# Kyo-suke-S/Depth_image_captioning_pub

Hardware: AMD Instinct MI355X
Metric: images/sec (train, depth-soft, 224x224, seq-len 20) (higher is better)
Workload: dtype f32; 1 GPU; depth-soft train step, synthetic RGB-D 224x224, batch 64/GPU, seq-len 20, V=10000, ResNet-152 (random init, batch-stat BN) + depth CNN + soft-attention LSTM; global_batch=64, batch_per_gpu=64, seq_len=20, vocab=10000, parallelism=dp1, resnet_conv_mode=f16x2, cross_step_resnet_overlap=True, resnet_forwards_in_flight=3, annotation_cells=49, ranks=1, collective=none (single rank)

## Files before the change

depth_image_captioning_pub_amd/csrc/api.hip:

```cpp
#include "dic.h"
#include "conv.h"
#include "nn_kernels.h"

#include <cstdio>

using namespace dic;

namespace dic { void resnet_fuse_bn_operand(int mask); void resnet_fuse_bn_halo(int on); void resnet_fuse_res_bn(int on); void depth_encoder_l1_sparse(int on); void bn_finalize_two_level_rows(int rows); void resnet_debug_fused_tail_bn(int on); void conv1_depth_debug_blocks(int n);
                void depth_encoder_f16x2(int on); }
#ifdef DIC_EXPERIMENTS
namespace dic { void decoder_debug_persistent(int on); void decoder_persist_debug_buffer(unsigned long long* p); void decoder_persist_debug_placement(int p);
                void resnet_debug_skip_bn_apply(int on); }
#endif

extern "C" {

int dic_version(void) { return DIC_ABI_VERSION; }
size_t dic_struct_bytes(int which) {
  switch (which) {
    case 0: return sizeof(dic_conv_bn_layer);
    case 1: return sizeof(dic_decoder_weights);
    case 2: return sizeof(dic_decoder_grads);
    case 3: return sizeof(dic_depth_encoder_weights);
    case 4: return sizeof(dic_depth_encoder_grads);
    case 5: return sizeof(dic_depth_bn_state);
    case 6: return sizeof(dic_nic_weights);
    case 7: return sizeof(dic_nic_grads);
    default: return 0;
  }
}
const char* dic_last_error(void) { return last_error(); }

int dic_gemm_f32(int M, int N, int K, const float* A, long long lda, int a_colk, const float* B, long long ldb,
                 int b_colk, float* C, long long ldc, const float* bias, int act, int accumulate, int splitk,
                 float* workspace, size_t workspace_bytes, int force_tile, void* stream) {
  GemmParams p{};
  p.M = M; p.N = N; p.K = K;
  p.A = a_colk ? op_colk(A, lda) : op_rowk(A, lda);
  p.B = b_colk ? op_colk(B, ldb) : op_rowk(B, ldb);
  p.ep = ep_store(C, ldc, bias, act);
  p.ep.accumulate = accumulate;
  p.splitk = splitk; p.ws = workspace;
  p.ablate = force_tile / 1000;
  force_tile %= 1000;
  DIC_REQUIRE(force_tile == 0 || force_tile == 64 || force_tile == 128, "force_tile must be 0, 64 or 128");
  if (splitk > 1)
    DIC_REQUIRE(workspace_bytes >= gemm_splitk_ws_bytes(M, N, splitk), "dic_gemm_f32: workspace too small");
  return gemm_launch(p, (hipStream_t)stream, force_tile);
}

int dic_conv2d_fwd(const float* x, int B, int H, int W, int C, int in_nchw, const float* w_ohwi, const float* bias,
                   int CO, int KH, int KW, int stride, int pad, float* y_nhwc, float* bn_partial, int* mtiles_out,
                   int force_tile, float* tail_ws, void* stream) {
  ConvDesc d{B, H, W, C, CO, KH, KW, stride, pad, in_nchw};
  return conv_fwd(x, d, w_ohwi, bias, y_nhwc, bn_partial, mtiles_out, (hipStream_t)stream, force_tile, tail_ws);
}

int dic_debug_force_staged_gemm(int on) {
  if (gemm_bf3_force_tile(on) == 0) return 0;
  if (on >= 100 && on <= 104) { dic::resnet_fuse_bn_operand(on == 104 ? -1 : on - 100); return 0; }
  if (on == 98 || on == 99) { dic::resnet_fuse_res_bn(on - 98); return 0; }
  if (on == 108 || on == 109) { dic::resnet_fuse_bn_halo(on - 108); return 0; }
  if (on == 182 || on == 183) { dic::bn_finalize_two_level_rows(on == 182 ? 512 : 1024); return 0; }
  if (on == 180 || on == 181) { dic::depth_encoder_l1_sparse(on - 180); return 0; }
  if (on == 116 || on == 117) { dic::depth_encoder_f16x2(on - 116); return 0; }
#ifdef DIC_EXPERIMENTS
  if (on == 140 || on == 141) { dic::decoder_debug_persistent(on - 140); return 0; }
  if (on == 142 || on == 143) { dic::decoder_persist_debug_placement(on - 142); return 0; }
  if (on >= 130 && on <= 134) { dic::conv1_depth_debug_blocks(256 * (on - 130)); return 0; }
  if (on >= 150 && on <= 153) { dic::resnet_debug_fused_tail_bn(on - 150); return 0; }
  if (on >= 124 && on <= 127) { dic::resnet_debug_skip_bn_apply(on == 125 ? 3 : on == 126 ? 2 : on == 127 ? 1 : 0); return 0; }
  if (on >= 0 && on <= 13) { gemm_force_v1(on); return 0; }
#endif
  DIC_REQUIRE(false, "debug switch: unknown code %d", on);
  return 0;
}
#ifdef DIC_EXPERIMENTS
int dic_debug_decoder_stamps(unsigned long long* dev_buf) { dic::decoder_persist_debug_buffer(dev_buf); return 0; }
#endif
int dic_debug_conv1_wgrad(const float* x, int B, int H, int W, const float* dy, float* dw, float* dbias, float* ws, float* cs_ws,
                          void* stream) {
  ConvDesc d{B, H, W, 1, 128, 7, 7, 3, 0, 0};
  return conv1_depth_wgrad(x, d, dy, dw, dbias, ws, cs_ws, (hipStream_t)stream);
}
int dic_debug_conv1_fwd(const float* x, int B, int H, int W, const float* w, const float* bias, float* y, float* partial,
                        void* stream) {
  ConvDesc d{B, H, W, 1, 128, 7, 7, 3, 0, 0};
  int rows = 0;
  return conv1_depth_fwd(x, d, w, bias, y, partial, &rows, (hipStream_t)stream);
}
int dic_debug_conv_bf3(const uint16_t* const x_planes[3], int B, int H, int W, int C, const uint16_t* const w_planes[3], int CO,
                       int k, int stride, int pad, float* y, float* bn_partial, int* mtiles_out, float* tail_ws, void* stream) {
  ConvDesc d{B, H, W, C, CO, k, k, stride, pad, 0};
  return conv_fwd_bf3(x_planes, d, w_planes, y, bn_partial, mtiles_out, tail_ws, (hipStream_t)stream, nullptr, nullptr, nullptr);
}
int dic_debug_bf3_plan(int route, int fmt, int B, int H, int W, int C, int CO, int k, int stride, int pad, int flags, int splitk,
                       int tail_ws_slabs, char* name, int name_bytes, int* out) {
  DIC_REQUIRE(name && name_bytes > 0 && out, "debug_bf3_plan: bad arguments");
  const char* kernel = nullptr;
  DIC_TRY(bf3_plan_route(route, fmt, ConvDesc{B, H, W, C, CO, k, k, stride, pad, 0}, flags, splitk, tail_ws_slabs, &kernel, out));
  snprintf(name, name_bytes, "%s", kernel);
  return DIC_OK;
}
int dic_debug_conv_fmt(const uint16_t* const x_planes[3], int B, int H, int W, int C, const uint16_t* const w_planes[3], int CO,
                       int k, int stride, int pad, float* y, float* bn_partial, int* mtiles_out, float* tail_ws, int fmt, float out_scale,
                       void* stream) {
  ConvDesc d{B, H, W, C, CO, k, k, stride, pad, 0};
  return conv_fwd_bf3(x_planes, d, w_planes, y, bn_partial, mtiles_out, tail_ws, (hipStream_t)stream, nullptr, nullptr, nullptr, 0, 1024, fmt,
                      out_scale);
}
int dic_debug_conv1x1_bn_fmt(const float* raw, const float* scale, const float* shift, const float* res, int relu, float* act_out, int M,
                             int C, const uint16_t* const w_planes[3], int CO, float* y, float* bn_partial, int* mtiles_out, float* tail_ws,
                             int tail_ws_slabs, int fmt, float out_scale, void* stream) {
  return conv1x1_fwd_bf3_bn(raw, scale, shift, res, relu, act_out, M, C, w_planes, CO, y, bn_partial, mtiles_out, tail_ws, tail_ws_slabs,
                            (hipStream_t)stream, nullptr, nullptr, fmt, out_scale);
}
int dic_debug_conv3x3_bn(const float* raw, const float* scale, const float* shift, int relu, int B, int H, int W, int C,
                         const uint16_t* const w_planes[3], int CO, float* y, float* bn_partial, int* mtiles_out, float* tail_ws,
                         int tail_ws_slabs, float out_scale, uint32_t* status, void* stream) {
  ConvDesc d{B, H, W, C, CO, 3, 3, 1, 1, 0};
  return conv3x3_fwd_bf3_bn(raw, scale, shift, relu, d, w_planes, y, bn_partial, mtiles_out, tail_ws, tail_ws_slabs, (hipStream_t)stream,
                            nullptr, nullptr, 1, out_scale, status);
}
#ifdef DIC_EXPERIMENTS
int dic_debug_conv1x1_astat(const float* raw, const float* scale, const float* shift, int relu, int M, int C, const uint16_t* const w_planes[3],
                            int CO, float* y, float* bn_partial, int* mtiles_out, float out_scale, uint32_t* status, void* stream) {
  return conv1x1_astat_bn(raw, scale, shift, relu, M, C, w_planes, CO, y, bn_partial, mtiles_out, (hipStream_t)stream, out_scale, status);
}
#endif
int dic_conv_persistent_grid(int max_workgroups) {
  DIC_REQUIRE(gemm_bf3_set_persist_grid(max_workgroups) == 0, "dic_conv_persistent_grid: 1 <= max_workgroups <= 1024");
  return DIC_OK;
}
int dic_debug_conv1x1_bn(const float* raw, const float* scale, const float* shift, const float* res, int relu, float* act_out, int M,
                         int C, const uint16_t* const w_planes[3], int CO, float* y, float* bn_partial, int* mtiles_out, float* tail_ws,
                         int tail_ws_slabs, void* stream) {
  return conv1x1_fwd_bf3_bn(raw, scale, shift, res, relu, act_out, M, C, w_planes, CO, y, bn_partial, mtiles_out, tail_ws, tail_ws_slabs,
                            (hipStream_t)stream, nullptr, nullptr);
}
static int bn_buf(const float* scale, const float* shift, const float* mean, const float* invstd, BnBuf* out, const char* who) {
  DIC_REQUIRE(scale && shift && mean && invstd, "%s: a BatchNorm buffer (scale, shift, mean, invstd) is NULL", who);
  *out = BnBuf{const_cast<float*>(scale), const_cast<float*>(shift), const_cast<float*>(mean), const_cast<float*>(invstd)};
  return DIC_OK;
}
static int bn_buf_opt(const float* scale, const float* shift, const float* mean, const float* invstd, BnBuf* out, bool* have, const char* who) {
  *have = scale || shift || mean || invstd;
  *out = BnBuf{};
  return *have ? bn_buf(scale, shift, mean, invstd, out, who) : DIC_OK;
}
static int plane_list(uint16_t* const planes[3], const char* who) {
  DIC_REQUIRE(!planes || (planes[0] && planes[1]), "%s: planes[0] / planes[1] is NULL", who);
  return DIC_OK;
}
int dic_debug_bn_backward_ws_floats(int C) {
  DIC_REQUIRE(C > 0 && C % 64 == 0, "dic_debug_bn_backward_ws_floats: C=%d must be a positive multiple of 64", C);
  const size_t n = bn_backward_ws_floats(C);
  DIC_REQUIRE(n < ((size_t)1 << 31), "dic_debug_bn_backward_ws_floats: C=%d is out of range", C);
  return (int)n;
}
int dic_debug_bn_finalize(const float* partial, int mtiles, long long count, int C, const float* gamma, const float* beta,
                          float* running_mean, float* running_var, float* scale, float* shift, float* mean, float* invstd, double* red,
                          size_t red_doubles, uint32_t* status, void* stream) {
  BnBuf bn;
  DIC_TRY(bn_buf(scale, shift, mean, invstd, &bn, "dic_debug_bn_finalize"));
  DIC_REQUIRE(partial && gamma && beta, "dic_debug_bn_finalize: partial / gamma / beta is NULL");
  DIC_REQUIRE(mtiles >= 1 && count >= 1 && C >= 1, "dic_debug_bn_finalize: mtiles=%d count=%lld C=%d must be positive", mtiles, count, C);
  DIC_REQUIRE(!running_mean == !running_var, "dic_debug_bn_finalize: running_mean and running_var go together");
  DIC_REQUIRE(!red || red_doubles >= bn_finalize_ws_doubles(mtiles, C), "dic_debug_bn_finalize: red holds %zu doubles, %zu needed", red_doubles,
              bn_finalize_ws_doubles(mtiles, C));
  return bn_finalize_train(partial, mtiles, count, C, gamma, beta, running_mean, running_var, bn, red, (hipStream_t)stream, status);
}
int dic_debug_bn_finalize_eval(int C, const float* gamma, const float* beta, const float* running_mean, const float* running_var,
                               float* scale, float* shift, float* mean, float* invstd, void* stream) {
  BnBuf bn;
  DIC_TRY(bn_buf(scale, shift, mean, invstd, &bn, "dic_debug_bn_finalize_eval"));
  DIC_REQUIRE(gamma && beta && running_mean && running_var, "dic_debug_bn_finalize_eval: gamma / beta / running statistics NULL");
  DIC_REQUIRE(C >= 1, "dic_debug_bn_finalize_eval: C=%d must be positive", C);
  return bn_finalize_eval(C, gamma, beta, running_mean, running_var, bn, (hipStream_t)stream);
}
int dic_debug_bn_apply(const float* x, const float* residual, const uint16_t* const residual_planes[3], float* y, uint16_t* const planes[3],
                       long long rows, int C, const float* scale, const float* shift, const float* mean, const float* invstd, int relu,
                       const float* res_scale, const float* res_shift, const float* res_mean, const float* res_invstd, uint32_t* status,
                       void* stream) {
  BnBuf bn, rbn;
  bool have_rbn;
  DIC_TRY(bn_buf(scale, shift, mean, invstd, &bn, "dic_debug_bn_apply"));
  DIC_TRY(bn_buf_opt(res_scale, res_shift, res_mean, res_invstd, &rbn, &have_rbn, "dic_debug_bn_apply (residual)"));
  DIC_TRY(plane_list(planes, "dic_debug_bn_apply"));
  DIC_REQUIRE(x, "dic_debug_bn_apply: x is NULL");
  DIC_REQUIRE(rows >= 1 && C >= 1, "dic_debug_bn_apply: rows=%lld C=%d must be positive", rows, C);
  DIC_REQUIRE(!residual_planes || (residual_planes[0] && residual_planes[1] && residual_planes[2]), "dic_debug_bn_apply: a residual plane is NULL");
  if (!planes) {
    DIC_REQUIRE(y, "dic_debug_bn_apply: no output (y and planes NULL)");
    DIC_REQUIRE(!residual_planes && !have_rbn, "dic_debug_bn_apply: a plane residual or a residual BatchNorm needs plane output");
    DIC_REQUIRE(C % 4 == 0, "dic_debug_bn_apply: C=%d %% 4", C);
    return bn_apply(x, residual, y, rows, C, bn, relu, (hipStream_t)stream);
  }
  DIC_REQUIRE(C % 32 == 0, "dic_debug_bn_apply: C=%d %% 32 (plane output)", C);
  return bn_apply_planes(x, residual, residual_planes, y, planes, rows, C, bn, relu, (hipStream_t)stream, have_rbn ? &rbn : nullptr, status);
}
static int pool_geometry(const char* who, int B, int H, int W, int C, int k, int s, int p) {
  DIC_REQUIRE(B >= 1 && H >= 1 && W >= 1 && C >= 1, "%s: B=%d H=%d W=%d C=%d must be positive", who, B, H, W, C);
  DIC_REQUIRE(C % 4 == 0, "%s: C=%d %% 4", who, C);
  DIC_REQUIRE(k >= 1 && k <= 15 && s >= 1 && p >= 0 && 2 * p <= k, "%s: k=%d (1..15) s=%d p=%d (at most k / 2)", who, k, s, p);
  DIC_REQUIRE(H + 2 * p >= k && W + 2 * p >= k, "%s: the %dx%d window does not fit the padded %dx%d map", who, k, k, H + 2 * p, W + 2 * p);
  return DIC_OK;
}
int dic_debug_bn_relu_maxpool(const float* x, int B, int H, int W, int C, const float* scale, const float* shift, const float* mean,
                              const float* invstd, int relu, int k, int s, int p, float* y, unsigned char* idx, uint16_t* const planes[3],
                              uint32_t* status, float* xsel, void* stream) {
  BnBuf bn;
  bool have_bn;
  DIC_TRY(bn_buf_opt(scale, shift, mean, invstd, &bn, &have_bn, "dic_debug_bn_relu_maxpool"));
  DIC_TRY(plane_list(planes, "dic_debug_bn_relu_maxpool"));
  DIC_TRY(pool_geometry("dic_debug_bn_relu_maxpool", B, H, W, C, k, s, p));
  DIC_REQUIRE(x && (y || planes), "dic_debug_bn_relu_maxpool: x is NULL or there is no output");
  DIC_REQUIRE(!planes || C % 32 == 0, "dic_debug_bn_relu_maxpool: C=%d %% 32 (plane output)", C);
  return bn_relu_maxpool(x, B, H, W, C, have_bn ? &bn : nullptr, relu, k, s, p, y, idx, (hipStream_t)stream, planes, status, xsel);
}
int dic_debug_adaptive_avgpool(const float* x, int B, int H, int W, int C, const float* scale, const float* shift, const float* mean,
                               const float* invstd, int relu, int out, float* y, void* stream) {
  BnBuf bn;
  bool have_bn;
  DIC_TRY(bn_buf_opt(scale, shift, mean, invstd, &bn, &have_bn, "dic_debug_adaptive_avgpool"));
  DIC_REQUIRE(x && y, "dic_debug_adaptive_avgpool: x / y is NULL");
  DIC_REQUIRE(B >= 1 && H >= 1 && W >= 1 && C >= 1 && out >= 1, "dic_debug_adaptive_avgpool: B=%d H=%d W=%d C=%d out=%d must be positive", B, H, W, C, out);
  DIC_REQUIRE(C % 4 == 0, "dic_debug_adaptive_avgpool: C=%d %% 4", C);
  return adaptive_avgpool(x, B, H, W, C, have_bn ? &bn : nullptr, relu, out, y, (hipStream_t)stream);
}
int dic_debug_adaptive_avgpool_bwd(const float* dy, int B, int H, int W, int C, int out, float* dx, void* stream) {
  DIC_REQUIRE(dy && dx, "dic_debug_adaptive_avgpool_bwd: dy / dx is NULL");
  DIC_REQUIRE(B >= 1 && H >= 1 && W >= 1 && C >= 1 && out >= 1, "dic_debug_adaptive_avgpool_bwd: B=%d H=%d W=%d C=%d out=%d must be positive", B, H, W, C, out);
  DIC_REQUIRE(C % 4 == 0, "dic_debug_adaptive_avgpool_bwd: C=%d %% 4", C);
  return adaptive_avgpool_bwd(dy, B, H, W, C, out, dx, (hipStream_t)stream);
}
int dic_debug_maxpool_relu_bwd(const float* dpool, const unsigned char* idx, const float* x, int B, int H, int W, int C, int k,
                               const float* scale, const float* shift, const float* mean, const float* invstd, float* dy, void* stream) {
  BnBuf bn;
  DIC_TRY(bn_buf(scale, shift, mean, invstd, &bn, "dic_debug_maxpool_relu_bwd"));
  DIC_TRY(pool_geometry("dic_debug_maxpool_relu_bwd", B, H, W, C, k, k, 0));
  DIC_REQUIRE(dpool && idx && x && dy, "dic_debug_maxpool_relu_bwd: dpool / idx / x / dy is NULL");
  return maxpool_relu_bwd(dpool, idx, x, B, H, W, C, k, bn, dy, (hipStream_t)stream);
}
int dic_debug_relu_mask_bwd(float* dy, const float* x, long long rows, int C, const float* scale, const float* shift, const float* mean,
                            const float* invstd, void* stream) {
  BnBuf bn;
  DIC_TRY(bn_buf(scale, shift, mean, invstd, &bn, "dic_debug_relu_mask_bwd"));
  DIC_REQUIRE(dy && x, "dic_debug_relu_mask_bwd: dy / x is NULL");
  DIC_REQUIRE(rows >= 1 && C >= 1 && C % 4 == 0, "dic_debug_relu_mask_bwd: rows=%lld, C=%d %% 4", rows, C);
  return relu_mask_bwd(dy, x, rows, C, bn, (hipStream_t)stream);
}
static int f16_scale(const uint16_t* const planes[3], uint32_t* bound, float* slot, F16Scale* out, const char* who) {
  *out = F16Scale{bound, slot};
  DIC_REQUIRE(!(planes && !planes[2]) || (bound && slot), "%s: f16x2 planes need the scale's bound word and slot", who);
  return DIC_OK;
}
int dic_debug_bn_backward(float* dy_dx, const float* x, long long rows, int C, const float* gamma, const float* scale, const float* shift,
                          const float* mean, const float* invstd, float* dgamma, float* dbeta, float* ws, size_t ws_floats,
                          uint16_t* const dx_planes[3], uint32_t* f16_bound, float* f16_slot, void* stream) {
  BnBuf bn;
  F16Scale fs;
  DIC_TRY(bn_buf(scale, shift, mean, invstd, &bn, "dic_debug_bn_backward"));
  DIC_TRY(plane_list(dx_planes, "dic_debug_bn_backward"));
  DIC_TRY(f16_scale(dx_planes, f16_bound, f16_slot, &fs, "dic_debug_bn_backward"));
  DIC_REQUIRE(dy_dx && x && gamma && dgamma && dbeta && ws, "dic_debug_bn_backward: dy_dx / x / gamma / dgamma / dbeta / ws is NULL");
  DIC_REQUIRE(rows >= 1 && C >= 1 && C % 64 == 0, "dic_debug_bn_backward: rows=%lld, C=%d %% 64", rows, C);
  DIC_REQUIRE(ws_floats >= bn_backward_ws_floats(C), "dic_debug_bn_backward: ws holds %zu floats, %zu needed", ws_floats, bn_backward_ws_floats(C));
  return bn_backward(dy_dx, x, rows, C, gamma, bn, dgamma, dbeta, ws, (hipStream_t)stream, dx_planes, &fs);
}
int dic_debug_bn_pool_backward(const float* dpool, const unsigned char* idx, const float* x, int B, int H, int W, int C, int k,
                               const float* gamma, const float* scale, const float* shift, const float* mean, const float* invstd,
                               float* dgamma, float* dbeta, float* ws, size_t ws_floats, float* dy, uint16_t* const dy_planes[3],
                               uint32_t* f16_bound, float* f16_slot, void* stream) {
  BnBuf bn;
  F16Scale fs;
  DIC_TRY(bn_buf(scale, shift, mean, invstd, &bn, "dic_debug_bn_pool_backward"));
  DIC_TRY(plane_list(dy_planes, "dic_debug_bn_pool_backward"));
  DIC_TRY(f16_scale(dy_planes, f16_bound, f16_slot, &fs, "dic_debug_bn_pool_backward"));
  DIC_TRY(pool_geometry("dic_debug_bn_pool_backward", B, H, W, C, k, k, 0));
  DIC_REQUIRE(dpool && idx && x && gamma && dgamma && dbeta && ws && dy, "dic_debug_bn_pool_backward: dpool / idx / x / gamma / dgamma / dbeta / ws / dy is NULL");
  DIC_REQUIRE(C % 64 == 0 && 256 % (C / 4) == 0, "dic_debug_bn_pool_backward: C=%d %% 64, with C / 4 dividing 256", C);
  DIC_REQUIRE(ws_floats >= bn_backward_ws_floats(C), "dic_debug_bn_pool_backward: ws holds %zu floats, %zu needed", ws_floats, bn_backward_ws_floats(C));
  return bn_pool_backward(dpool, idx, x, B, H, W, C, k, gamma, bn, dgamma, dbeta, ws, dy, (hipStream_t)stream, dy_planes, &fs);
}
int dic_debug_colsum_rows(const float* X, long long ld, long long rows, int C, float* out, float* ws, size_t ws_floats, void* stream) {
  DIC_REQUIRE(X && out && ws, "dic_debug_colsum_rows: X / out / ws is NULL");
  DIC_REQUIRE(rows >= 1 && C >= 1 && ld >= C, "dic_debug_colsum_rows: rows=%lld C=%d ld=%lld (at least C)", rows, C, ld);
  DIC_REQUIRE(ws_floats >= (size_t)256 * C, "dic_debug_colsum_rows: ws holds %zu floats, %zu needed", ws_floats, (size_t)256 * C);
  return colsum_rows(X, ld, rows, C, out, ws, (hipStream_t)stream);
}
int dic_debug_f16_scale_reset(uint32_t* bounds, int n, void* stream) {
  DIC_REQUIRE(bounds && n >= 1 && n <= 64, "dic_debug_f16_scale_reset: bounds is NULL or n=%d is outside 1..64", n);
  return f16_scale_reset(bounds, n, (hipStream_t)stream);
}
int dic_debug_f16_scale_from_absmax(const float* x, long long n, uint32_t* bound, float* slot, void* stream) {
  DIC_REQUIRE(x && bound && slot, "dic_debug_f16_scale_from_absmax: x / bound / slot is NULL");
  DIC_REQUIRE(n >= 4 && n % 4 == 0, "dic_debug_f16_scale_from_absmax: n=%lld %% 4", n);
  return f16_scale_from_absmax(x, n, F16Scale{bound, slot}, (hipStream_t)stream);
}
int dic_debug_f16_scale_finish(uint32_t* bound, float* slot, void* stream) {
  DIC_REQUIRE(bound && slot, "dic_debug_f16_scale_finish: bound / slot is NULL");
  return f16_scale_finish(F16Scale{bound, slot}, (hipStream_t)stream);
}
static int conv_geometry(const char* who, int B, int H, int W, int C, int CO, int k, int stride, int pad) {
  DIC_REQUIRE(B >= 1 && H >= 1 && W >= 1 && C >= 1 && CO >= 1, "%s: B=%d H=%d W=%d C=%d CO=%d must be positive", who, B, H, W, C, CO);
  DIC_REQUIRE(k >= 1 && k <= 7 && stride >= 1 && pad >= 0 && pad < k, "%s: k=%d (1..7) stride=%d pad=%d (below k)", who, k, stride, pad);
  DIC_REQUIRE(H + 2 * pad >= k && W + 2 * pad >= k, "%s: the %dx%d filter does not fit the padded %dx%d map", who, k, k, H + 2 * pad, W + 2 * pad);
  const ConvDesc d{B, H, W, C, CO, k, k, stride, pad, 0};
  DIC_REQUIRE((long long)B * d.OH() * d.OW() <= 0x7fffffffll - 32 && (long long)B * H * W <= 0x7fffffffll, "%s: more than 2^31 pixels", who);
  return DIC_OK;
}
static int plane_triple(const uint16_t* const planes[3], int fmt, const char* who, const char* what) {
  DIC_REQUIRE(planes && planes[0] && planes[1] && (fmt || planes[2]), "%s: %s: a plane pointer is NULL", who, what);
  return DIC_OK;
}
int dic_debug_conv_wgrad_sizes(int B, int H, int W, int C, int CO, int k, int stride, int pad, int splitk, size_t* dyT_elems, size_t* pT_elems,
                               size_t* ws_floats) {
  DIC_TRY(conv_geometry("dic_debug_conv_wgrad_sizes", B, H, W, C, CO, k, stride, pad));
  DIC_REQUIRE(C % 32 == 0 && CO % 32 == 0, "dic_debug_conv_wgrad_sizes: C=%d and CO=%d %% 32", C, CO);
  DIC_REQUIRE(splitk >= 1 && splitk <= 16, "dic_debug_conv_wgrad_sizes: splitk=%d is outside 1..16", splitk);
  DIC_REQUIRE(dyT_elems && pT_elems && ws_floats, "dic_debug_conv_wgrad_sizes: an output pointer is NULL");
  const ConvDesc d{B, H, W, C, CO, k, k, stride, pad, 0};
  *dyT_elems = conv_wgrad_bf3_plane_elems(d, 0); *pT_elems = conv_wgrad_bf3_plane_elems(d, 1); *ws_floats = conv_wgrad_bf3_ws_floats(d, splitk);
  return DIC_OK;
}
int dic_debug_conv_wgrad(const float* x, int B, int H, int W, int C, int CO, int k, int stride, int pad, const float* dy, float* dw_ohwi,
                         int splitk, uint16_t* const dyT[3], size_t dyT_elems, uint16_t* const pT[3], size_t pT_elems, float* ws,
                         size_t ws_floats, int fmt, const float* dy_slot, void* stream) {
  const char* who = "dic_debug_conv_wgrad";
  DIC_TRY(conv_geometry(who, B, H, W, C, CO, k, stride, pad));
  DIC_REQUIRE(x && dy && dw_ohwi && ws, "%s: x / dy / dw_ohwi / ws is NULL", who);
  DIC_REQUIRE(fmt == 0 || fmt == 1, "%s: fmt=%d is neither 0 (bf16x3) nor 1 (f16x2)", who, fmt);
  DIC_REQUIRE(C % 32 == 0 && CO % 32 == 0, "%s: C=%d and CO=%d %% 32", who, C, CO);
  DIC_REQUIRE(splitk >= 1 && splitk <= 16, "%s: splitk=%d is outside 1..16", who, splitk);
  DIC_TRY(plane_triple(dyT, fmt, who, "dyT"));
  DIC_TRY(plane_triple(pT, fmt, who, "pT"));
  DIC_REQUIRE(fmt == 0 || dy_slot, "%s: the f16x2 format needs the gradient's scale slot", who);
  const ConvDesc d{B, H, W, C, CO, k, k, stride, pad, 0};
  DIC_REQUIRE(dyT_elems >= conv_wgrad_bf3_plane_elems(d, 0), "%s: dyT planes hold %zu elements, %zu needed", who, dyT_elems, conv_wgrad_bf3_plane_elems(d, 0));
  DIC_REQUIRE(pT_elems >= conv_wgrad_bf3_plane_elems(d, 1), "%s: pT planes hold %zu elements, %zu needed", who, pT_elems, conv_wgrad_bf3_plane_elems(d, 1));
  DIC_REQUIRE(ws_floats >= conv_wgrad_bf3_ws_floats(d, splitk), "%s: ws holds %zu floats, %zu needed", who, ws_floats, conv_wgrad_bf3_ws_floats(d, splitk));
  return conv_wgrad_bf3(x, d, dy, dw_ohwi, splitk, dyT, pT, ws, (hipStream_t)stream, fmt, dy_slot);
}
int dic_debug_conv_dgrad_s1(const uint16_t* const dy_planes[3], int B, int H, int W, int C, int CO, int k, int pad,
                            const uint16_t* const wflip_planes[3], float* dx, float* tail_ws, int tail_ws_slabs, int fmt, const float* alpha_dev0,
                            const float* alpha_dev1, void* stream) {
  const char* who = "dic_debug_conv_dgrad_s1";
  DIC_TRY(conv_geometry(who, B, H, W, C, CO, k, 1, pad));
  DIC_REQUIRE(fmt == 0 || fmt == 1, "%s: fmt=%d is neither 0 (bf16x3) nor 1 (f16x2)", who, fmt);
  DIC_REQUIRE(C % 32 == 0 && CO % 32 == 0, "%s: C=%d and CO=%d %% 32", who, C, CO);
  DIC_REQUIRE(k * k <= 32, "%s: k=%d: at most 32 taps", who, k);
  DIC_TRY(plane_triple(dy_planes, fmt, who, "dy_planes"));
  DIC_TRY(plane_triple(wflip_planes, fmt, who, "wflip_planes"));
  DIC_REQUIRE(dx, "%s: dx is NULL", who);
  DIC_REQUIRE(!tail_ws == (tail_ws_slabs == 0) && tail_ws_slabs >= 0 && tail_ws_slabs <= 1024, "%s: tail_ws and tail_ws_slabs=%d (0..1024) go together", who, tail_ws_slabs);
  DIC_REQUIRE(fmt == 1 || (!alpha_dev0 && !alpha_dev1), "%s: device-resident factors belong to the f16x2 format", who);
  const ConvDesc d{B, H, W, C, CO, k, k, 1, pad, 0};
  return conv_dgrad_s1_bf3(dy_planes, d, wflip_planes, dx, (hipStream_t)stream, tail_ws, tail_ws ? tail_ws_slabs : 256, fmt, alpha_dev0, alpha_dev1);
}
int dic_debug_depth_prepare_weights(const float* w2_oihw, const float* w3_oihw, uint16_t* const w2_pl[3], uint16_t* const w2f_pl[3],
                                    uint16_t* const w3_pl[3], uint16_t* const w3f_pl[3], size_t w2_plane_elems, size_t w3_plane_elems,
                                    const float* slots, void* stream) {
  const char* who = "dic_debug_depth_prepare_weights";
  const int fmt = slots ? 1 : 0;
  DIC_REQUIRE(w2_oihw && w3_oihw, "%s: w2 / w3 is NULL", who);
  DIC_TRY(plane_triple(w2_pl, fmt, who, "w2_pl"));
  DIC_TRY(plane_triple(w2f_pl, fmt, who, "w2f_pl"));
  DIC_TRY(plane_triple(w3_pl, fmt, who, "w3_pl"));
  DIC_TRY(plane_triple(w3f_pl, fmt, who, "w3f_pl"));
  DIC_REQUIRE(w2_plane_elems >= (size_t)512 * 1152 && w3_plane_elems >= (size_t)2048 * 512, "%s: planes hold %zu / %zu elements, %zu / %zu needed", who,
              w2_plane_elems, w3_plane_elems, (size_t)512 * 1152, (size_t)2048 * 512);
  return depth_prepare_weights(w2_oihw, w3_oihw, w2_pl, w2f_pl, w3_pl, w3f_pl, slots, (hipStream_t)stream);
}
int dic_debug_conv_wgrad_f32(const float* x, int B, int H, int W, int C, int in_nchw, int CO, int k, int stride, int pad, const float* dy, float* dw_ohwi,
                             int splitk, float* ws, size_t ws_floats, void* stream) {
  const char* who = "dic_debug_conv_wgrad_f32";
  DIC_TRY(conv_geometry(who, B, H, W, C, CO, k, stride, pad));
  DIC_REQUIRE(x && dy && dw_ohwi, "%s: x / dy / dw_ohwi is NULL", who);
  DIC_REQUIRE(splitk >= 1 && splitk <= 1024, "%s: splitk=%d is outside 1..1024", who, splitk);
  DIC_REQUIRE(in_nchw == 0 || in_nchw == 1, "%s: in_nchw=%d is neither 0 nor 1", who, in_nchw);
  const size_t need = gemm_splitk_ws_bytes(CO, k * k * C, splitk) / sizeof(float);
  DIC_REQUIRE(splitk == 1 || (ws && ws_floats >= need), "%s: ws holds %zu floats, %zu needed", who, ws ? ws_floats : (size_t)0, need);
  const ConvDesc d{B, H, W, C, CO, k, k, stride, pad, in_nchw};
  return conv_wgrad(x, d, dy, dw_ohwi, splitk, ws, (hipStream_t)stream);
}
static const ConvDesc layer1_desc(int B, int H, int W) { return ConvDesc{B, H, W, 1, 128, 7, 7, 3, 0, 0}; }
int dic_debug_depth_layer1_sparse_ws_floats(int B, int H, int W) {
  DIC_REQUIRE(B >= 1 && H >= 7 && W >= 7 && (long long)B * H * W <= 0x7fffffffll, "dic_debug_depth_layer1_sparse_ws_floats: B=%d H=%d W=%d", B, H, W);
  const size_t n = depth_layer1_sparse_ws_floats(layer1_desc(B, H, W));
  DIC_REQUIRE(n < ((size_t)1 << 31), "dic_debug_depth_layer1_sparse_ws_floats: B=%d H=%d W=%d is out of range", B, H, W);
  return (int)n;
}
constexpr size_t kLayer1ColsumFloats = (size_t)64 * 128 * 49;
int dic_debug_depth_layer1_bwd_sparse(const float* depth, int B, int H, int W, const float* dpool, const unsigned char* idx, const float* xsel,
                                      const float* conv_w, const float* conv_b, const float* gamma, const float* scale, const float* shift,
                                      const float* mean, const float* invstd, float* dgamma, float* dbeta, float* dW, float* db, float* bn_ws,
                                      size_t bn_ws_floats, float* ws, size_t ws_floats, float* cs_ws, size_t cs_ws_floats, void* stream) {
  const char* who = "dic_debug_depth_layer1_bwd_sparse";
  BnBuf bn;
  DIC_TRY(bn_buf(scale, shift, mean, invstd, &bn, who));
  DIC_REQUIRE(depth && dpool && idx && xsel && conv_w && conv_b && gamma, "%s: depth / dpool / idx / xsel / conv_w / conv_b / gamma is NULL", who);
  DIC_REQUIRE(dgamma && dbeta && dW && db && bn_ws && ws && cs_ws, "%s: dgamma / dbeta / dW / db / bn_ws / ws / cs_ws is NULL", who);
  DIC_REQUIRE(B >= 1 && H >= 7 && W >= 7 && (long long)B * H * W <= 0x7fffffffll, "%s: B=%d H=%d W=%d", who, B, H, W);
  const ConvDesc d = layer1_desc(B, H, W);
  if (!depth_layer1_sparse_supported(d)) return 1;
  DIC_REQUIRE(bn_ws_floats >= bn_backward_ws_floats(128), "%s: bn_ws holds %zu floats, %zu needed", who, bn_ws_floats, bn_backward_ws_floats(128));
  DIC_REQUIRE(ws_floats >= depth_layer1_sparse_ws_floats(d), "%s: ws holds %zu floats, %zu needed", who, ws_floats, depth_layer1_sparse_ws_floats(d));
  DIC_REQUIRE(cs_ws_floats >= kLayer1ColsumFloats, "%s: cs_ws holds %zu floats, %zu needed", who, cs_ws_floats, kLayer1ColsumFloats);
  return depth_layer1_backward_sparse(depth, d, dpool, idx, xsel, conv_w, conv_b, gamma, bn, dgamma, dbeta, dW, db, bn_ws, ws, cs_ws, (hipStream_t)stream);
}
int dic_debug_conv1_fwd_checked(const float* x, int B, int H, int W, const float* w, const float* bias, float* y, float* partial,
                                size_t partial_floats, int* partial_rows, void* stream) {
  const char* who = "dic_debug_conv1_fwd_checked";
  DIC_REQUIRE(x && w && bias && y, "%s: x / w / bias / y is NULL", who);
  DIC_REQUIRE(B >= 1 && H >= 7 && W >= 7 && (long long)B * H * W <= 0x7fffffffll, "%s: B=%d H=%d W=%d", who, B, H, W);
  const ConvDesc d = layer1_desc(B, H, W);
  if (!conv1_depth_supported(d)) return 1;
  DIC_REQUIRE(!partial || partial_floats >= (size_t)conv1_depth_fwd_blocks(d) * 2 * 128, "%s: partial holds %zu floats, %zu needed", who, partial_floats,
              (size_t)conv1_depth_fwd_blocks(d) * 2 * 128);
  return conv1_depth_fwd(x, d, w, bias, y, partial, partial_rows, (hipStream_t)stream);
}
int dic_debug_conv1_wgrad_checked(const float* x, int B, int H, int W, const float* dy, float* dw, float* dbias, float* ws, size_t ws_floats,
// ... 23 lines not shown
```

depth_image_captioning_pub_amd/csrc/conv.h:

```cpp
#pragma once
#include "gemm.h"

namespace dic {

struct ConvDesc {
  int B, H, W, C;
  int CO, KH, KW, stride, pad;
  int in_nchw;
  int OH() const { return (H + 2 * pad - KH) / stride + 1; }
  int OW() const { return (W + 2 * pad - KW) / stride + 1; }
  int M() const { return B * OH() * OW(); }
  int K() const { return KH * KW * C; }
  ConvGeom geom() const { return ConvGeom{H, W, C, OH(), OW(), KH, KW, stride, pad, in_nchw}; }
};

int conv_fwd(const float* x, const ConvDesc& d, const float* w_ohwi, const float* bias, float* y,
             float* bn_partial, int* mtiles_out, hipStream_t st, int force_tile = 0, float* tail_ws = nullptr);
int conv_mtiles(const ConvDesc& d, int force_tile = 0);

int conv_fwd_bf3(const unsigned short* const x_planes[3], const ConvDesc& d, const unsigned short* const w_planes[3],
                 float* y, float* bn_partial, int* mtiles_out, float* tail_ws, hipStream_t st,
                 const float* bias = nullptr, const BnFuseArgs* bn_fuse = nullptr, int* bn_fused = nullptr,
                 int act = 0 , int tail_ws_slabs = 256 ,
                 int fmt = 0 ,
                 float out_scale = 1.0f ,
                 const float* alpha_dev0 = nullptr, const float* alpha_dev1 = nullptr );
int conv1x1_fwd_bf3_bn(const float* raw, const float* scale, const float* shift, const float* res, int relu, float* act_out,
                       int M, int C, const unsigned short* const w_planes[3], int CO, float* y, float* bn_partial,
                       int* mtiles_out, float* tail_ws, int tail_ws_slabs, hipStream_t st, const BnFuseArgs* bn_fuse = nullptr,
                       int* bn_fused = nullptr, int fmt = 0, float out_scale = 1.0f,
                       unsigned* status = nullptr ,
                       const float* res_scale = nullptr, const float* res_shift = nullptr );
bool conv1x1_bf3_bn_eligible(const float* raw, int M, int C, int CO, float* tail_ws, int tail_ws_slabs, int fmt = 0);
int bf3_plan_route(int route, int fmt, const ConvDesc& d, int flags, int splitk, int tail_ws_slabs, const char** kernel, int out[6]);
int conv3x3_fwd_bf3_bn(const float* raw, const float* scale, const float* shift, int relu, const ConvDesc& d,
                       const unsigned short* const w_planes[3], float* y, float* bn_partial, int* mtiles_out, float* tail_ws,
                       int tail_ws_slabs, hipStream_t st, const BnFuseArgs* bn_fuse, int* bn_fused, int fmt, float out_scale, unsigned* status);
#ifdef DIC_EXPERIMENTS
bool conv1x1_astat_eligible(int M, int C, int CO);
int conv1x1_astat_bn(const float* raw, const float* scale, const float* shift, int relu, int M, int C, const unsigned short* const w_planes[3],
                     int CO, float* y, float* bn_partial, int* mtiles_out, hipStream_t st, float out_scale, unsigned* status = nullptr);
#endif
constexpr int kResnetTailSlabs = 1024;
size_t conv_wgrad_bf3_plane_elems(const ConvDesc& d, int which);
size_t conv_wgrad_bf3_ws_floats(const ConvDesc& d, int splitk);
int conv_wgrad_bf3(const float* x, const ConvDesc& d, const float* dy, float* dw_ohwi, int splitk,
                   unsigned short* const dyT[3], unsigned short* const pT[3], float* ws, hipStream_t st,
                   int fmt = 0, const float* dy_slot = nullptr );
size_t conv_stem_bf3_plane_elems(int B, int H, int W);
int conv_stem_pack_weights(const float* w_oihw, int CO, float* scratch_f32, unsigned short* const w_planes[3], hipStream_t st,
                           float f16_scale = 0.f );
int conv_stem_bf3(const float* imgs_nchw, int B, int H, int W, int CO, unsigned short* const x_planes[3],
                  const unsigned short* const w_planes[3], float* y, float* bn_partial, int* mtiles_out, hipStream_t st,
                  int fmt = 0, float out_scale = 1.0f, unsigned* status = nullptr );
int conv_dgrad_s1_bf3(const unsigned short* const dy_planes[3], const ConvDesc& d,
                      const unsigned short* const wflip_planes[3], float* dx, hipStream_t st, float* tail_ws = nullptr,
                      int tail_ws_slabs = 256, int fmt = 0, const float* alpha_dev0 = nullptr, const float* alpha_dev1 = nullptr);
int split_bf16x3(const float* x, long long n, unsigned short* hi, unsigned short* mid, unsigned short* lo, hipStream_t st);
int split_bf16x3_paired(const float* x, long long rows, int K, unsigned short* hi, unsigned short* mid,
                        unsigned short* lo, hipStream_t st);
int split_f16x2_paired(const float* x, long long rows, int K, float scale, unsigned short* h1, unsigned short* h2, hipStream_t st,
                       unsigned* status = nullptr );

int conv1_depth_fwd(const float* x, const ConvDesc& d, const float* w, const float* bias, float* y, float* bn_partial,
                    int* partial_rows, hipStream_t st);
int conv1_depth_fwd_blocks(const ConvDesc& d);
bool conv1_depth_supported(const ConvDesc& d);
size_t conv1_depth_wgrad_ws_floats(const ConvDesc& d);
struct BnBuf;
bool depth_layer1_sparse_supported(const ConvDesc& d);
size_t depth_layer1_sparse_ws_floats(const ConvDesc& d);
int conv1_depth_wgrad(const float* x, const ConvDesc& d, const float* dy, float* dw, float* dbias, float* ws, float* cs_ws,
                      hipStream_t st);
int depth_layer1_backward_sparse(const float* depth, const ConvDesc& d, const float* dpool, const unsigned char* idx, const float* xsel,
                                 const float* conv_w, const float* conv_b, const float* gamma, BnBuf bn, float* dgamma, float* dbeta,
                                 float* dW, float* db, float* bn_ws, float* ws, float* cs_ws, hipStream_t st);
int depth_prepare_weights(const float* w2, const float* w3, unsigned short* const w2_pl[3], unsigned short* const w2f_pl[3],
                          unsigned short* const w3_pl[3], unsigned short* const w3f_pl[3], const float* slots, hipStream_t st);
int conv_wgrad(const float* x, const ConvDesc& d, const float* dy, float* dw_ohwi, int splitk, float* ws,
               hipStream_t st);
int conv_dgrad_s1(const float* dy, const ConvDesc& d, const float* w_flip, float* dx, hipStream_t st);
int conv_flip_weights(const float* w_ohwi, const ConvDesc& d, float* w_flip, hipStream_t st);

}
```

depth_image_captioning_pub_amd/csrc/encoders.hip:

```cpp
#include "dic.h"
#include "conv.h"
#include "nn_kernels.h"
#include <algorithm>
#include <vector>

namespace dic {

struct DepthGeom {
  int B, H, W;
  int H1, W1, P1h, P1w, H2, W2, P2h, P2w;
  ConvDesc c1, c2, c3;
  long long M1, M2, M3;
};

static DepthGeom depth_geom(int B, int H, int W) {
  DepthGeom g{};
  g.B = B; g.H = H; g.W = W;
  g.c1 = ConvDesc{B, H, W, 1, 128, 7, 7, 3, 0, 1};
  g.H1 = g.c1.OH(); g.W1 = g.c1.OW();
  g.P1h = g.H1 / 3; g.P1w = g.W1 / 3;
  g.c2 = ConvDesc{B, g.P1h, g.P1w, 128, 512, 3, 3, 1, 0, 0};
  g.H2 = g.c2.OH(); g.W2 = g.c2.OW();
  g.P2h = g.H2 / 3; g.P2w = g.W2 / 3;
  g.c3 = ConvDesc{B, g.P2h, g.P2w, 512, 2048, 1, 1, 1, 0, 0};
  g.M1 = (long long)B * g.H1 * g.W1; g.M2 = (long long)B * g.H2 * g.W2; g.M3 = (long long)B * g.P2h * g.P2w;
  return g;
}

static int g_l1_sparse = 1;
void depth_encoder_l1_sparse(int on) { g_l1_sparse = on; }
static int g_depth_f16x2 = 1;
void depth_encoder_f16x2(int on) { g_depth_f16x2 = on; }
constexpr int kWg1Split = 128;
constexpr int kWg2Split = 4;
constexpr int kWg2SplitBf3 = 5;
constexpr int kWg3SplitBf3 = 3;

struct DepthWs {
  unsigned* status;
  unsigned* bounds;
  float* slots;
  float *x1, *y1p, *x2, *y2p, *x3, *partial;
  float* x1sel;
  double* red;
  unsigned char *idx1, *idx2;
  BnBuf bn1, bn2, bn3;
  float *dy1, *dy1p, *dy2, *dy2p, *dy3, *dw2o, *wg_ws, *bn_ws, *cs_ws;
  unsigned short *y1p_pl[3], *w2_pl[3], *dy2_pl[3], *w2f_pl[3];
  unsigned short *y2p_pl[3], *w3_pl[3], *dy3_pl[3], *w3f_pl[3];
  float* tail;
  unsigned short *wg_dyT[3], *wg_pT[3];
  float* wg_bf3_ws;
  size_t bytes;
};

static BnBuf take_bn(Carver& c, int C) {
  BnBuf b;
  b.scale = c.take<float>(C); b.shift = c.take<float>(C); b.mean = c.take<float>(C); b.invstd = c.take<float>(C);
  return b;
}

static DepthWs depth_carve(void* p, size_t bytes, const DepthGeom& g, bool* ov) {
  Carver c(p, bytes);
  DepthWs w{};
  const long long B = g.B;
  w.status = c.take<unsigned>(64);
  w.bounds = c.take<unsigned>(64);
  w.slots = c.take<float>(64);
  w.x1 = c.take<float>((size_t)g.M1 * 128);
  w.y1p = c.take<float>((size_t)B * g.P1h * g.P1w * 128);
  w.idx1 = c.take<unsigned char>((size_t)B * g.P1h * g.P1w * 128);
  w.x1sel = c.take<float>((size_t)B * g.P1h * g.P1w * 128);
  w.x2 = c.take<float>((size_t)g.M2 * 512);
  w.y2p = c.take<float>((size_t)B * g.P2h * g.P2w * 512);
  w.idx2 = c.take<unsigned char>((size_t)B * g.P2h * g.P2w * 512);
  w.x3 = c.take<float>((size_t)g.M3 * 2048);
  const long long rows1 = std::max<long long>(g.M1 / 64 + 2, 1024 + 2);
  size_t part = (size_t)rows1 * 2 * 128;
  part = std::max(part, (size_t)(g.M2 / 64 + 2) * 2 * 512);
  part = std::max(part, (size_t)(g.M3 / 64 + 2) * 2 * 2048);
  w.partial = c.take<float>(part);
  w.red = c.take<double>(std::max(std::max(bn_finalize_ws_doubles((int)rows1, 128), bn_finalize_ws_doubles(g.M2 / 64 + 2, 512)),
                                   bn_finalize_ws_doubles(g.M3 / 64 + 2, 2048)));
  w.bn1 = take_bn(c, 128); w.bn2 = take_bn(c, 512); w.bn3 = take_bn(c, 2048);
  w.dy1 = c.take<float>(std::max((size_t)g.M1 * 128, depth_layer1_sparse_supported(g.c1) ? depth_layer1_sparse_ws_floats(g.c1) : (size_t)0));
  w.dy1p = c.take<float>((size_t)B * g.P1h * g.P1w * 128);
  w.dy2 = c.take<float>((size_t)g.M2 * 512);
  w.dy2p = c.take<float>((size_t)B * g.P2h * g.P2w * 512);
  w.dy3 = c.take<float>((size_t)g.M3 * 2048);
  w.dw2o = c.take<float>((size_t)512 * 1152);
  w.wg_ws = c.take<float>(std::max(std::max((size_t)kWg1Split * 128 * 49, (size_t)kWg2Split * 512 * 1152),
                                   conv1_depth_wgrad_ws_floats(g.c1)));
  w.bn_ws = c.take<float>(bn_backward_ws_floats(2048));
  w.cs_ws = c.take<float>((size_t)256 * 2048);
  for (int i = 0; i < 3; ++i) {
    w.y1p_pl[i] = c.take<unsigned short>((size_t)(B * g.P1h * g.P1w + 1) * 128);
    w.w2_pl[i] = c.take<unsigned short>((size_t)512 * 1152);
    w.dy2_pl[i] = c.take<unsigned short>((size_t)(g.M2 + 1) * 512);
    w.w2f_pl[i] = c.take<unsigned short>((size_t)128 * 4608);
    w.y2p_pl[i] = c.take<unsigned short>((size_t)(g.M3 + 1) * 512);
    w.w3_pl[i] = c.take<unsigned short>((size_t)2048 * 512);
    w.dy3_pl[i] = c.take<unsigned short>((size_t)(g.M3 + 1) * 2048);
    w.w3f_pl[i] = c.take<unsigned short>((size_t)512 * 2048);
    w.wg_dyT[i] = c.take<unsigned short>(std::max(conv_wgrad_bf3_plane_elems(g.c2, 0), conv_wgrad_bf3_plane_elems(g.c3, 0)));
    w.wg_pT[i] = c.take<unsigned short>(std::max(conv_wgrad_bf3_plane_elems(g.c2, 1), conv_wgrad_bf3_plane_elems(g.c3, 1)));
  }
  w.wg_bf3_ws = c.take<float>(std::max(conv_wgrad_bf3_ws_floats(g.c2, kWg2SplitBf3), conv_wgrad_bf3_ws_floats(g.c3, kWg3SplitBf3)));
  w.tail = c.take<float>(std::max((size_t)kResnetTailSlabs * 64 * 64, kGemmTailWsBytes / sizeof(float)));
  w.bytes = c.off;
  if (ov) *ov = c.overflow;
  return w;
}

struct RnConv {
  ConvDesc d;
  int layer;
};

struct RnPlan {
  std::vector<RnConv> convs;
  size_t max_act = 0, max_partial = 0, max_red = 0;
  int outH = 0, outW = 0;
  int B = 0, H = 0, W = 0;
};

static void rn_track(RnPlan& pl, const ConvDesc& d) {
  pl.max_act = std::max(pl.max_act, (size_t)d.M() * d.CO);
  pl.max_partial = std::max(pl.max_partial, (size_t)(d.M() / 32 + 4) * 2 * d.CO);
  pl.max_red = std::max(pl.max_red, bn_finalize_ws_doubles(d.M() / 32 + 4, d.CO));
}

static RnPlan resnet_plan(int B, int H, int W, const int* blocks) {
  RnPlan pl;
  pl.B = B; pl.H = H; pl.W = W;
  int li = 0;
  ConvDesc stem{B, H, W, 3, 64, 7, 7, 2, 3, 1};
  pl.convs.push_back({stem, li++});
  rn_track(pl, stem);
  int h = stem.OH(), w = stem.OW();
  h = (h + 2 - 3) / 2 + 1; w = (w + 2 - 3) / 2 + 1;
  int inpl = 64;
  const int planes_of[4] = {64, 128, 256, 512};
  for (int s = 0; s < 4; ++s) {
    const int planes = planes_of[s];
    for (int b = 0; b < blocks[s]; ++b) {
      const int stride = (s > 0 && b == 0) ? 2 : 1;
      ConvDesc c1{B, h, w, inpl, planes, 1, 1, 1, 0, 0};
      ConvDesc c2{B, h, w, planes, planes, 3, 3, stride, 1, 0};
      const int oh = c2.OH(), ow = c2.OW();
      ConvDesc c3{B, oh, ow, planes, planes * 4, 1, 1, 1, 0, 0};
      pl.convs.push_back({c1, li++}); rn_track(pl, c1);
      pl.convs.push_back({c2, li++}); rn_track(pl, c2);
      pl.convs.push_back({c3, li++}); rn_track(pl, c3);
      if (b == 0) {
        ConvDesc ds{B, h, w, inpl, planes * 4, 1, 1, stride, 0, 0};
        pl.convs.push_back({ds, li++}); rn_track(pl, ds);
      }
      h = oh; w = ow; inpl = planes * 4;
    }
  }
  pl.outH = h; pl.outW = w;
  return pl;
}

struct RnWs {
  unsigned* status;
  float* act[6];
  unsigned short* planes[3][3];
  unsigned short* stem_planes[3];
  float* partial;
  float* tail;
  double* red;
  BnBuf bn;
  BnBuf bn2, bn3;
  BnBuf bn_ds;
  size_t bytes;
};

static RnWs rn_carve(void* p, size_t bytes, const RnPlan& pl, int mode, bool* ov) {
  Carver c(p, bytes);
  RnWs w{};
  w.status = c.take<unsigned>(64);
  for (int i = 0; i < (mode >= 1 ? 6 : 4); ++i) w.act[i] = c.take<float>(pl.max_act);
  if (mode >= 1)
    for (int i = 0; i < 3; ++i)
// ... 219 lines not shown
__global__ void __launch_bounds__(256) depth_prepare_weights_kernel(const float* __restrict__ w2, const float* __restrict__ w3,
                                                                    DepthWeightPlanes pl, const float* __restrict__ slots) {
  constexpr int O2 = 512, I2 = 128, O3 = 2048, I3 = 512;
  constexpr long long n2 = (long long)O2 * I2 * 9, n3 = (long long)O3 * I3;
  constexpr long long q2 = n2 / 4, q3 = n3 / 4;
  for (long long e = (long long)blockIdx.x * 256 + threadIdx.x; e < 2 * (q2 + q3); e += (long long)gridDim.x * 256) {
    int set; long long g = e;
    if (g < q2) set = 0; else if ((g -= q2) < q2) set = 1; else if ((g -= q2) < q3) set = 2; else { g -= q3; set = 3; }
    const int K = set == 0 ? 9 * I2 : set == 1 ? 9 * O2 : set == 2 ? I3 : O3;
    const int kb = K / 32;
    const long long idx = g * 4;
    const long long line = idx >> 6;
    const int within = (int)(idx & 63);
    const int row = (int)(line / kb) * 2 + (within >> 5);
    const int k0 = (int)(line % kb) * 32 + (within & 31);
    float v[4];
#pragma unroll
    for (int u = 0; u < 4; ++u) {
      const int k = k0 + u;
      if (set == 0) {
        const int tap = k / I2, i = k - tap * I2;
        v[u] = w2[((long long)row * I2 + i) * 9 + tap];
      } else if (set == 1) {
        const int ftap = k / O2, o = k - ftap * O2;
        v[u] = w2[((long long)o * I2 + row) * 9 + (8 - ftap)];
      } else if (set == 2) {
        v[u] = w3[(long long)row * I3 + k];
      } else {
        v[u] = w3[(long long)k * I3 + row];
      }
    }
    unsigned short h[4], m[4], l[4];
    if (slots) {
      const float fs = slots[set < 2 ? 0 : 2];
#pragma unroll
      for (int u = 0; u < 4; ++u) split2_f16(v[u], fs, h[u], m[u]);
    } else {
#pragma unroll
      for (int u = 0; u < 4; ++u) split3_bf16(v[u], h[u], m[u], l[u]);
    }
    unsigned short* const* pp = set == 0 ? pl.w2 : set == 1 ? pl.w2f : set == 2 ? pl.w3 : pl.w3f;
    *reinterpret_cast<uint2*>(pp[0] + idx) = make_uint2((unsigned)h[0] | ((unsigned)h[1] << 16), (unsigned)h[2] | ((unsigned)h[3] << 16));
    *reinterpret_cast<uint2*>(pp[1] + idx) = make_uint2((unsigned)m[0] | ((unsigned)m[1] << 16), (unsigned)m[2] | ((unsigned)m[3] << 16));
    if (!slots) *reinterpret_cast<uint2*>(pp[2] + idx) = make_uint2((unsigned)l[0] | ((unsigned)l[1] << 16), (unsigned)l[2] | ((unsigned)l[3] << 16));
  }
}

int depth_prepare_weights(const float* w2, const float* w3, unsigned short* const w2_pl[3], unsigned short* const w2f_pl[3],
                          unsigned short* const w3_pl[3], unsigned short* const w3f_pl[3], const float* slots, hipStream_t st) {
  DepthWeightPlanes pl;
  for (int i = 0; i < 3; ++i) { pl.w2[i] = w2_pl[i]; pl.w2f[i] = w2f_pl[i]; pl.w3[i] = w3_pl[i]; pl.w3f[i] = w3f_pl[i]; }
  hipLaunchKernelGGL(depth_prepare_weights_kernel, dim3(2048), dim3(256), 0, st, w2, w3, pl, slots);
  DIC_LAUNCH_CHECK();
  return DIC_OK;
}

}

using namespace dic;

extern "C" {

int dic_oihw_to_ohwi(const float* src, float* dst, int O, int I, int KH, int KW, void* stream) {
  DIC_REQUIRE(src && dst && src != dst, "oihw_to_ohwi: bad pointers");
  return oihw_to_ohwi(src, dst, O, I, KH, KW, (hipStream_t)stream);
}

size_t dic_depth_encoder_workspace_bytes(int B, int H, int W) {
  bool ov;
  return depth_carve(nullptr, 0, depth_geom(B, H, W), &ov).bytes;
}

static int depth_encoder_fwd_impl(const dic_depth_encoder_weights* w, const dic_depth_bn_state* s, const float* depth, int B,
                                  int H, int W, int train, float* features, void* workspace, size_t workspace_bytes,
                                  void* stream, int pool_out) {
  hipStream_t st = (hipStream_t)stream;
  DIC_REQUIRE(w && s && depth && features && workspace, "depth_encoder_fwd: null pointer");
  DIC_REQUIRE(B > 0 && H >= 43 && W >= 43, "depth_encoder_fwd: input too small (%dx%d)", H, W);
  const DepthGeom g = depth_geom(B, H, W);
  DIC_REQUIRE(g.P2h >= 1 && g.P2w >= 1, "depth_encoder_fwd: input too small");
  bool ov = false;
  DepthWs ws = depth_carve(workspace, workspace_bytes, g, &ov);
  DIC_REQUIRE(!ov, "depth_encoder_fwd: workspace too small (%zu < %zu)", workspace_bytes, ws.bytes);
  int mt = 0;
  const int fmt = g_depth_f16x2;
  DIC_TRY(clear_status(ws.status, st));
  const F16Scale s_w2{ws.bounds + 0, ws.slots + 0}, s_w3{ws.bounds + 1, ws.slots + 2};
  if (fmt) {
    DIC_TRY(f16_scale_reset(ws.bounds, 2, st));
    DIC_TRY(f16_scale_from_absmax(w->conv2_w, 512ll * 128 * 9, s_w2, st));
    DIC_TRY(f16_scale_from_absmax(w->conv3_w, 2048ll * 512, s_w3, st));
  }
  DIC_TRY(depth_prepare_weights(w->conv2_w, w->conv3_w, ws.w2_pl, ws.w2f_pl, ws.w3_pl, ws.w3f_pl, fmt ? (const float*)ws.slots : nullptr, st));
  unsigned short* const y1p_out[3] = {ws.y1p_pl[0], ws.y1p_pl[1], fmt ? nullptr : ws.y1p_pl[2]};
  unsigned short* const y2p_out[3] = {ws.y2p_pl[0], ws.y2p_pl[1], fmt ? nullptr : ws.y2p_pl[2]};
  if (conv1_depth_supported(g.c1))
    DIC_TRY(conv1_depth_fwd(depth, g.c1, w->conv1_w, w->conv1_b, ws.x1, train ? ws.partial : nullptr, &mt, st));
  else
    DIC_TRY(conv_fwd(depth, g.c1, w->conv1_w, w->conv1_b, ws.x1, train ? ws.partial : nullptr, &mt, st));
  if (train) DIC_TRY(bn_finalize_train(ws.partial, mt, g.M1, 128, w->bn1_w, w->bn1_b, s->rm1, s->rv1, ws.bn1, ws.red, st));
  else DIC_TRY(bn_finalize_eval(128, w->bn1_w, w->bn1_b, s->rm1, s->rv1, ws.bn1, st));
  DIC_TRY(bn_relu_maxpool(ws.x1, B, g.H1, g.W1, 128, &ws.bn1, 1, 3, 3, 0, ws.y1p, ws.idx1, st, y1p_out, ws.status, ws.x1sel));
  {
    const unsigned short* xp[3] = {ws.y1p_pl[0], ws.y1p_pl[1], fmt ? nullptr : ws.y1p_pl[2]};
    const unsigned short* wp[3] = {ws.w2_pl[0], ws.w2_pl[1], fmt ? nullptr : ws.w2_pl[2]};
    DIC_TRY(conv_fwd_bf3(xp, g.c2, wp, ws.x2, train ? ws.partial : nullptr, &mt, ws.tail, st, w->conv2_b, nullptr, nullptr,
                         ACT_NONE, kResnetTailSlabs, fmt, 1.0f / kF16ActScale, fmt ? s_w2.slot + 1 : nullptr));
  }
  if (train) DIC_TRY(bn_finalize_train(ws.partial, mt, g.M2, 512, w->bn2_w, w->bn2_b, s->rm2, s->rv2, ws.bn2, ws.red, st));
  else DIC_TRY(bn_finalize_eval(512, w->bn2_w, w->bn2_b, s->rm2, s->rv2, ws.bn2, st));
  DIC_TRY(bn_relu_maxpool(ws.x2, B, g.H2, g.W2, 512, &ws.bn2, 1, 3, 3, 0, ws.y2p, ws.idx2, st, y2p_out, ws.status));
  {
    const unsigned short* xp[3] = {ws.y2p_pl[0], ws.y2p_pl[1], fmt ? nullptr : ws.y2p_pl[2]};
    const unsigned short* wp[3] = {ws.w3_pl[0], ws.w3_pl[1], fmt ? nullptr : ws.w3_pl[2]};
    DIC_TRY(conv_fwd_bf3(xp, g.c3, wp, ws.x3, train ? ws.partial : nullptr, &mt, ws.tail, st, w->conv3_b, nullptr, nullptr,
                         ACT_NONE, kResnetTailSlabs, fmt, 1.0f / kF16ActScale, fmt ? s_w3.slot + 1 : nullptr));
  }
  if (train) DIC_TRY(bn_finalize_train(ws.partial, mt, g.M3, 2048, w->bn3_w, w->bn3_b, s->rm3, s->rv3, ws.bn3, ws.red, st));
  else DIC_TRY(bn_finalize_eval(2048, w->bn3_w, w->bn3_b, s->rm3, s->rv3, ws.bn3, st));
  DIC_REQUIRE(pool_out != 0 || g.P2h == g.P2w, "depth_encoder_fwd_map: the feature map must be square");
  DIC_TRY(adaptive_avgpool(ws.x3, B, g.P2h, g.P2w, 2048, &ws.bn3, 1, pool_out ? pool_out : g.P2h, features, st));
  if (fmt)
    DIC_TRY(poison_if_raised(features, (long long)B * (pool_out ? pool_out * pool_out : g.P2h * g.P2w) * 2048, ws.status, st));
  return DIC_OK;
}

int dic_depth_encoder_fwd(const dic_depth_encoder_weights* w, const dic_depth_bn_state* s, const float* depth, int B,
                          int H, int W, int train, float* features, void* workspace, size_t workspace_bytes,
                          void* stream) {
  return depth_encoder_fwd_impl(w, s, depth, B, H, W, train, features, workspace, workspace_bytes, stream, 14);
}

int dic_depth_encoder_fwd_map(const dic_depth_encoder_weights* w, const dic_depth_bn_state* s, const float* depth, int B,
                              int H, int W, int train, float* feature_map, void* workspace, size_t workspace_bytes,
                              void* stream) {
  return depth_encoder_fwd_impl(w, s, depth, B, H, W, train, feature_map, workspace, workspace_bytes, stream, 0);
}

static int depth_encoder_bwd_impl(const dic_depth_encoder_weights* w, const float* depth, const float* d_features, int B, int H,
                                  int W, const dic_depth_encoder_grads* gr, void* workspace, size_t workspace_bytes,
                                  void* stream, int pool_out) {
  hipStream_t st = (hipStream_t)stream;
  DIC_REQUIRE(w && depth && d_features && gr && workspace, "depth_encoder_bwd: null pointer");
  const DepthGeom g = depth_geom(B, H, W);
  bool ov = false;
  DepthWs ws = depth_carve(workspace, workspace_bytes, g, &ov);
  DIC_REQUIRE(!ov, "depth_encoder_bwd: workspace too small");
  const int fmt = g_depth_f16x2;
  F16Scale s_dy3{ws.bounds + 2, ws.slots + 4}, s_dy2{ws.bounds + 3, ws.slots + 6};
  const float *inv_w2 = ws.slots + 1, *inv_w3 = ws.slots + 3;
  if (fmt) DIC_TRY(f16_scale_reset(ws.bounds + 2, 2, st));
  unsigned short* const dy3_out[3] = {ws.dy3_pl[0], ws.dy3_pl[1], fmt ? nullptr : ws.dy3_pl[2]};
  unsigned short* const dy2_out[3] = {ws.dy2_pl[0], ws.dy2_pl[1], fmt ? nullptr : ws.dy2_pl[2]};
  DIC_TRY(adaptive_avgpool_bwd(d_features, B, g.P2h, g.P2w, 2048, pool_out ? pool_out : g.P2h, ws.dy3, st));
  DIC_TRY(relu_mask_bwd(ws.dy3, ws.x3, g.M3, 2048, ws.bn3, st));
  DIC_TRY(bn_backward(ws.dy3, ws.x3, g.M3, 2048, w->bn3_w, ws.bn3, gr->bn3_w, gr->bn3_b, ws.bn_ws, st, dy3_out, fmt ? &s_dy3 : nullptr));
  DIC_TRY(conv_wgrad_bf3(ws.y2p, g.c3, ws.dy3, gr->conv3_w, kWg3SplitBf3, ws.wg_dyT, ws.wg_pT, ws.wg_bf3_ws, st, fmt, s_dy3.slot));
  DIC_TRY(colsum_rows(ws.dy3, 2048, g.M3, 2048, gr->conv3_b, ws.cs_ws, st));
  {
    const unsigned short* dp[3] = {ws.dy3_pl[0], ws.dy3_pl[1], fmt ? nullptr : ws.dy3_pl[2]};
    const unsigned short* wp[3] = {ws.w3f_pl[0], ws.w3f_pl[1], fmt ? nullptr : ws.w3f_pl[2]};
    DIC_TRY(conv_dgrad_s1_bf3(dp, g.c3, wp, ws.dy2p, st, ws.tail, kResnetTailSlabs, fmt, fmt ? s_dy3.slot + 1 : nullptr, fmt ? inv_w3 : nullptr));
  }
  DIC_TRY(bn_pool_backward(ws.dy2p, ws.idx2, ws.x2, B, g.H2, g.W2, 512, 3, w->bn2_w, ws.bn2, gr->bn2_w, gr->bn2_b,
                           ws.bn_ws, ws.dy2, st, dy2_out, fmt ? &s_dy2 : nullptr));
  DIC_TRY(conv_wgrad_bf3(ws.y1p, g.c2, ws.dy2, ws.dw2o, kWg2SplitBf3, ws.wg_dyT, ws.wg_pT, ws.wg_bf3_ws, st, fmt, s_dy2.slot));
  DIC_TRY(ohwi_to_oihw(ws.dw2o, gr->conv2_w, 512, 128, 3, 3, st));
  DIC_TRY(colsum_rows(ws.dy2, 512, g.M2, 512, gr->conv2_b, ws.cs_ws, st));
  {
    const unsigned short* dp[3] = {ws.dy2_pl[0], ws.dy2_pl[1], fmt ? nullptr : ws.dy2_pl[2]};
    const unsigned short* wp[3] = {ws.w2f_pl[0], ws.w2f_pl[1], fmt ? nullptr : ws.w2f_pl[2]};
    DIC_TRY(conv_dgrad_s1_bf3(dp, g.c2, wp, ws.dy1p, st, ws.tail, kResnetTailSlabs, fmt, fmt ? s_dy2.slot + 1 : nullptr, fmt ? inv_w2 : nullptr));
  }
  if (g_l1_sparse && depth_layer1_sparse_supported(g.c1))
    return depth_layer1_backward_sparse(depth, g.c1, ws.dy1p, ws.idx1, ws.x1sel, w->conv1_w, w->conv1_b, w->bn1_w, ws.bn1, gr->bn1_w, gr->bn1_b,
                                        gr->conv1_w, gr->conv1_b, ws.bn_ws, ws.dy1, ws.cs_ws, st);
  DIC_TRY(bn_pool_backward(ws.dy1p, ws.idx1, ws.x1, B, g.H1, g.W1, 128, 3, w->bn1_w, ws.bn1, gr->bn1_w, gr->bn1_b,
                           ws.bn_ws, ws.dy1, st));
  if (conv1_depth_supported(g.c1)) {
    DIC_TRY(conv1_depth_wgrad(depth, g.c1, ws.dy1, gr->conv1_w, gr->conv1_b, ws.wg_ws, ws.cs_ws, st));
  } else {
    DIC_TRY(conv_wgrad(depth, g.c1, ws.dy1, gr->conv1_w, kWg1Split, ws.wg_ws, st));
    DIC_TRY(colsum_rows(ws.dy1, 128, g.M1, 128, gr->conv1_b, ws.cs_ws, st));
  }
  return DIC_OK;
}

int dic_depth_encoder_bwd(const dic_depth_encoder_weights* w, const float* depth, const float* d_features, int B, int H,
                          int W, const dic_depth_encoder_grads* gr, void* workspace, size_t workspace_bytes,
                          void* stream) {
  return depth_encoder_bwd_impl(w, depth, d_features, B, H, W, gr, workspace, workspace_bytes, stream, 14);
}

int dic_depth_encoder_bwd_map(const dic_depth_encoder_weights* w, const float* depth, const float* d_feature_map, int B,
                              int H, int W, const dic_depth_encoder_grads* gr, void* workspace, size_t workspace_bytes,
                              void* stream) {
  return depth_encoder_bwd_impl(w, depth, d_feature_map, B, H, W, gr, workspace, workspace_bytes, stream, 0);
}

int dic_depth_encoder_inspect(const void* workspace, size_t workspace_bytes, int B, int H, int W, int which, void* out,
                              long long* n_out, void* stream) {
  DIC_REQUIRE(workspace && B > 0 && which >= 1 && which <= 5, "depth_encoder_inspect: bad arguments");
  const DepthGeom g = depth_geom(B, H, W);
  bool ov = false;
  DepthWs ws = depth_carve(const_cast<void*>(workspace), workspace_bytes, g, &ov);
  DIC_REQUIRE(!ov, "depth_encoder_inspect: workspace too small");
  const long long n = which <= 2 ? (long long)B * g.P1h * g.P1w * 128
                      : which <= 4 ? (long long)B * g.P2h * g.P2w * 512 : g.M3 * 2048;
  if (n_out) *n_out = n;
  if (!out) return DIC_OK;
  if (which == 5) return relu_mask_export(ws.x3, g.M3, 2048, ws.bn3, (unsigned char*)out, (hipStream_t)stream);
  const void* src = which == 1 ? (const void*)ws.y1p : which == 2 ? (const void*)ws.idx1 : which == 3 ? (const void*)ws.y2p
                                                                                                      : (const void*)ws.idx2;
  const size_t bytes = (size_t)n * ((which & 1) ? sizeof(float) : 1);
  DIC_CHECK_HIP(hipMemcpyAsync(out, src, bytes, hipMemcpyDeviceToDevice, (hipStream_t)stream));
  return DIC_OK;
}

int dic_resnet_pack_stem_weights(const float* w_oihw, float* scratch_f32, uint16_t* w_hi, uint16_t* w_mid, uint16_t* w_lo,
                                 void* stream) {
  DIC_REQUIRE(w_oihw && scratch_f32 && w_hi && w_mid && w_lo, "resnet_pack_stem_weights: null pointer");
  unsigned short* wp[3] = {w_hi, w_mid, w_lo};
  return conv_stem_pack_weights(w_oihw, 64, scratch_f32, wp, (hipStream_t)stream);
}

int dic_resnet_pack_stem_weights_f16x2(const float* w_oihw, float* scratch_f32, uint16_t* w_h1, uint16_t* w_h2, float w_scale, void* stream) {
  DIC_REQUIRE(w_oihw && scratch_f32 && w_h1 && w_h2 && w_scale > 0.f, "resnet_pack_stem_weights_f16x2: null pointer / scale");
  unsigned short* wp[3] = {w_h1, w_h2, nullptr};
  return conv_stem_pack_weights(w_oihw, 64, scratch_f32, wp, (hipStream_t)stream, w_scale);
}

int dic_resnet_num_layers(const int* blocks) {
  int n = 1;
  for (int s = 0; s < 4; ++s) n += 3 * blocks[s] + 1;
  return n;
}

size_t dic_resnet_workspace_bytes(int B, int H, int W, const int* blocks, int mode) {
  bool ov;
  return rn_carve(nullptr, 0, resnet_plan(B, H, W, blocks), mode, &ov).bytes;
}

static int resnet_fwd_impl(const dic_conv_bn_layer* layers, int n_layers, const int* blocks, const float* imgs_nchw, int B,
                           int H, int W, int train_bn, int mode, float* features, void* workspace, size_t workspace_bytes,
                           void* stream, int pool_out) {
  hipStream_t st = (hipStream_t)stream;
  DIC_REQUIRE(layers && blocks && imgs_nchw && features && workspace, "resnet_fwd: null pointer");
  DIC_REQUIRE(n_layers == dic_resnet_num_layers(blocks), "resnet_fwd: expected %d conv+bn layers, got %d",
              dic_resnet_num_layers(blocks), n_layers);
  DIC_REQUIRE(B > 0 && H >= 32 && W >= 32, "resnet_fwd: bad input size");
  const RnPlan pl = resnet_plan(B, H, W, blocks);
  bool ov = false;
  DIC_REQUIRE(mode >= 0 && mode <= 2, "resnet_fwd: mode must be 0 (exact-fp32 MFMA), 1 (bf16x3 split MFMA) or 2 (f16x2 split MFMA)");
  RnWs ws = rn_carve(workspace, workspace_bytes, pl, mode, &ov);
  DIC_REQUIRE(!ov, "resnet_fwd: workspace too small (%zu < %zu)", workspace_bytes, ws.bytes);
  DIC_TRY(clear_status(ws.status, st));
  if (mode >= 1) {
    for (int i = 1; i < n_layers; ++i) {
      DIC_REQUIRE(layers[i].w_hi && layers[i].w_mid, "resnet_fwd: split-operand modes need split weights");
      if (mode == 1) DIC_REQUIRE(layers[i].w_lo, "resnet_fwd: bf16x3 mode needs three weight planes");
      else DIC_REQUIRE(layers[i].w_scale > 0.f, "resnet_fwd: f16x2 mode needs the scale of the weight planes (layer %d)", i);
    }
    return resnet_fwd_bf3(layers, blocks, imgs_nchw, B, train_bn, features, pl, ws, st, pool_out, mode == 2);
  }

  size_t ci = 0;
  float *X = ws.act[0], *A = ws.act[1], *Bf = ws.act[2], *Cf = ws.act[3];
  {
    const RnConv& c = pl.convs[ci++];
    DIC_TRY(conv_bn(imgs_nchw, c.d, layers[c.layer], A, ws.partial, ws.bn, ws.red, ws.tail, train_bn, st));
    DIC_TRY(bn_relu_maxpool(A, B, c.d.OH(), c.d.OW(), 64, &ws.bn, 1, 3, 2, 1, X, nullptr, st));
  }
  for (int s = 0; s < 4; ++s)
    for (int b = 0; b < blocks[s]; ++b) {
      const RnConv& c1 = pl.convs[ci++];
      const RnConv& c2 = pl.convs[ci++];
      const RnConv& c3 = pl.convs[ci++];
      DIC_TRY(conv_bn(X, c1.d, layers[c1.layer], A, ws.partial, ws.bn, ws.red, ws.tail, train_bn, st));
      DIC_TRY(bn_apply(A, nullptr, A, c1.d.M(), c1.d.CO, ws.bn, 1, st));
      DIC_TRY(conv_bn(A, c2.d, layers[c2.layer], Bf, ws.partial, ws.bn, ws.red, ws.tail, train_bn, st));
      DIC_TRY(bn_apply(Bf, nullptr, Bf, c2.d.M(), c2.d.CO, ws.bn, 1, st));
      const float* identity = X;
      if (b == 0) {
        const RnConv& ds = pl.convs[ci++];
        DIC_TRY(conv_bn(X, ds.d, layers[ds.layer], Cf, ws.partial, ws.bn, ws.red, ws.tail, train_bn, st));
        DIC_TRY(bn_apply(Cf, nullptr, Cf, ds.d.M(), ds.d.CO, ws.bn, 0, st));
        identity = Cf;
      }
      DIC_TRY(conv_bn(Bf, c3.d, layers[c3.layer], A, ws.partial, ws.bn, ws.red, ws.tail, train_bn, st));
      DIC_TRY(bn_apply(A, identity, Bf, c3.d.M(), c3.d.CO, ws.bn, 1, st));
      std::swap(X, Bf);
    }
  if (pool_out == 0) {
    DIC_CHECK_HIP(hipMemcpyAsync(features, X, sizeof(float) * (size_t)B * pl.outH * pl.outW * 2048, hipMemcpyDeviceToDevice, st));
    return DIC_OK;
  }
  DIC_TRY(adaptive_avgpool(X, B, pl.outH, pl.outW, 2048, nullptr, 0, pool_out, features, st));
  return DIC_OK;
}

int dic_resnet_fwd(const dic_conv_bn_layer* layers, int n_layers, const int* blocks, const float* imgs_nchw, int B,
                   int H, int W, int train_bn, int mode, float* features, void* workspace, size_t workspace_bytes,
                   void* stream) {
  return resnet_fwd_impl(layers, n_layers, blocks, imgs_nchw, B, H, W, train_bn, mode, features, workspace,
                         workspace_bytes, stream, 14);
}

int dic_resnet_fwd_map(const dic_conv_bn_layer* layers, int n_layers, const int* blocks, const float* imgs_nchw, int B,
                       int H, int W, int train_bn, int mode, float* feature_map, void* workspace, size_t workspace_bytes,
                       void* stream) {
  return resnet_fwd_impl(layers, n_layers, blocks, imgs_nchw, B, H, W, train_bn, mode, feature_map, workspace,
                         workspace_bytes, stream, 0);
}

}
```

depth_image_captioning_pub_amd/csrc/gemm_bf3.hip:

```cpp
#include "conv.h"
#include "gemm_epilogue.h"
#include <algorithm>
#include <cmath>
#include <type_traits>
#include <cstdlib>

namespace dic {

typedef __bf16 bf16x8 __attribute__((ext_vector_type(8)));
typedef _Float16 f16x8 __attribute__((ext_vector_type(8)));
typedef unsigned int u32x4 __attribute__((ext_vector_type(4)));
template <int FMT> struct Bf3Fmt { static constexpr int NPL = FMT == 1 ? 2 : 3; };
constexpr int BK3 = 32;
#ifndef DIC_WS_A_AUX
#define DIC_WS_A_AUX 0
#endif

__device__ __attribute__((aligned(256))) const unsigned short g_zero_line16[128] = {0};

__global__ void __launch_bounds__(256) split_bf16x3_kernel(const float* __restrict__ x, long long n,
                                                            unsigned short* __restrict__ hi,
                                                            unsigned short* __restrict__ mid,
                                                            unsigned short* __restrict__ lo) {
  const long long stride = (long long)gridDim.x * 256;
// ... 2002 lines not shown
}

static Bf3Params conv1x1_bn_bf3_params(const float* raw, const float* scale, const float* shift, const float* res, int relu, float* act_out,
                                       int M, int C, const unsigned short* const w_planes[3], int CO, float* y, float* bn_partial, int fmt,
                                       float out_scale, unsigned* status, const float* res_scale, const float* res_shift) {
  Bf3Params p{};
  p.M = M; p.N = CO; p.K = C;
  for (int i = 0; i < 3; ++i) { p.A.p[i] = nullptr; p.B.p[i] = w_planes[i]; }
  p.A.kind = OPK_ROWK; p.A.ld = C; p.A.paired = 1;
  p.B.kind = OPK_ROWK; p.B.ld = C; p.B.paired = 1;
  p.a_raw = raw; p.a_scale = scale; p.a_shift = shift; p.a_res = res; p.a_out = act_out; p.a_ld = C; p.a_relu = relu;
  p.a_res_scale = res_scale; p.a_res_shift = res_shift; p.status = status;
  p.ep = ep_store(y, CO, nullptr, ACT_NONE);
  p.ep.stats = bn_partial; p.fmt = fmt;
  if (fmt == 1) p.ep.alpha = out_scale;
  return p;
}
static bool conv1x1_bn_bf3_shape_ok(int M, int C) { return C % 32 == 0 && C <= kBnTabMax && (long long)M * C * 4 < (1ll << 32); }

bool conv1x1_bf3_bn_eligible(const float* raw, int M, int C, int CO, float* tail_ws, int tail_ws_slabs, int fmt) {
  const unsigned short* const none[3] = {};
  Bf3Plan pl;
  return conv1x1_bn_bf3_shape_ok(M, C) && plan_bf3(conv1x1_bn_bf3_params(raw, nullptr, nullptr, nullptr, 1, nullptr, M, C, none, CO, nullptr,
                                                                        nullptr, fmt, 1.0f, nullptr, nullptr, nullptr), Bf3Work{tail_ws, tail_ws_slabs}, &pl) == DIC_OK;
}

int conv1x1_fwd_bf3_bn(const float* raw, const float* scale, const float* shift, const float* res, int relu, float* act_out,
                       int M, int C, const unsigned short* const w_planes[3], int CO, float* y, float* bn_partial,
                       int* mtiles_out, float* tail_ws, int tail_ws_slabs, hipStream_t st, const BnFuseArgs* bn_fuse, int* bn_fused, int fmt,
                       float out_scale, unsigned* status, const float* res_scale, const float* res_shift) {
  DIC_REQUIRE(!res_scale || (fmt == 1 && res && res_shift), "conv1x1_fwd_bf3_bn: a BatchNorm on the residual needs the f16x2 format, the residual and both tables");
  DIC_REQUIRE(raw && scale && shift && y && C % 32 == 0 && C <= kBnTabMax, "conv1x1_fwd_bf3_bn: C %% 32 == 0, C <= 2048");
  if (!conv1x1_bn_bf3_shape_ok(M, C)) {
    set_last_error("conv1x1 with on-the-fly BatchNorm operand: input of %d x %d floats exceeds 4 GiB (32-bit offsets); nothing was launched", M, C);
    return 1;
  }
  return launch_bf3(conv1x1_bn_bf3_params(raw, scale, shift, res, relu, act_out, M, C, w_planes, CO, y, bn_partial, fmt, out_scale, status,
                                          res_scale, res_shift),
                    Bf3Work{tail_ws, tail_ws_slabs}, st, bn_fuse, bn_fused, mtiles_out);
}

static bool conv3x3_bn_bf3_shape_ok(const ConvDesc& d, int fmt) {
  return fmt == 1 && !d.in_nchw && d.KH == 3 && d.KW == 3 && d.stride == 1 && d.pad == 1 && d.C % 32 == 0 && d.C <= kHaloBnTab &&
         (long long)d.B * d.H * d.W * d.C * 4 < (1ll << 32);
}
static Bf3Params conv3x3_bn_bf3_params(const float* raw, const float* scale, const float* shift, int relu, const ConvDesc& d,
                                       const unsigned short* const w_planes[3], float* y, float* bn_partial, float out_scale, unsigned* status) {
  Bf3Params p{};
  p.M = d.M(); p.N = d.CO; p.K = d.K();
  for (int i = 0; i < 3; ++i) { p.A.p[i] = nullptr; p.B.p[i] = w_planes[i]; }
  p.A.kind = OPK_IM2COL; p.A.ld = d.C; p.A.g = d.geom(); p.A.paired = 1;
  p.B.kind = OPK_ROWK; p.B.ld = d.K(); p.B.paired = 1;
  p.a_raw = raw; p.a_scale = scale; p.a_shift = shift; p.a_ld = d.C; p.a_relu = relu; p.status = status;
  p.ep = ep_store(y, d.CO, nullptr, ACT_NONE);
  p.ep.stats = bn_partial; p.fmt = 1; p.ep.alpha = out_scale;
  return p;
}
int conv3x3_fwd_bf3_bn(const float* raw, const float* scale, const float* shift, int relu, const ConvDesc& d,
                       const unsigned short* const w_planes[3], float* y, float* bn_partial, int* mtiles_out, float* tail_ws,
                       int tail_ws_slabs, hipStream_t st, const BnFuseArgs* bn_fuse, int* bn_fused, int fmt, float out_scale, unsigned* status) {
  if (!conv3x3_bn_bf3_shape_ok(d, fmt)) return 1;
  DIC_REQUIRE(raw && scale && shift && y, "conv3x3_fwd_bf3_bn: null pointer");
  return launch_bf3(conv3x3_bn_bf3_params(raw, scale, shift, relu, d, w_planes, y, bn_partial, out_scale, status),
                    Bf3Work{tail_ws, tail_ws_slabs}, st, bn_fuse, bn_fused, mtiles_out);
}

template <bool IM2COL>
__global__ void __launch_bounds__(256) transpose_split_kernel(const float* __restrict__ x, long long ld, int M, int Kpad,
                                                               int ncols, ConvGeom g, unsigned short* __restrict__ hi,
                                                               unsigned short* __restrict__ mid,
                                                               unsigned short* __restrict__ lo, float f16_scale,
                                                               const float* __restrict__ f16_slot) {
  __shared__ float tile[32][33];
  const int m0 = blockIdx.x * 32;
  const int tid = threadIdx.x;
  int c0, tap = 0;
  if constexpr (IM2COL) {
    const int cb = g.C / 32;
    tap = blockIdx.y / cb;
    c0 = (blockIdx.y - tap * cb) * 32;
  } else {
    c0 = blockIdx.y * 32;
  }
  {
    const int mrow = tid >> 3, c4 = (tid & 7) * 4;
    const int m = m0 + mrow;
    float4 v = make_float4(0.f, 0.f, 0.f, 0.f);
    if (m < M) {
      if constexpr (IM2COL) {
        const int ohw = g.OH * g.OW;
        const int img = m / ohw, rem = m - img * ohw;
        const int oh = rem / g.OW, ow = rem - oh * g.OW;
        const int kh = tap / g.KW, kw = tap - kh * g.KW;
        const int ih = oh * g.stride - g.pad + kh, iw = ow * g.stride - g.pad + kw;
        if ((unsigned)ih < (unsigned)g.H && (unsigned)iw < (unsigned)g.W)
          v = *reinterpret_cast<const float4*>(x + (((long long)img * g.H + ih) * g.W + iw) * g.C + c0 + c4);
      } else {
        if (c0 + c4 < ncols) v = *reinterpret_cast<const float4*>(x + (long long)m * ld + c0 + c4);
      }
    }
    tile[mrow][c4] = v.x; tile[mrow][c4 + 1] = v.y; tile[mrow][c4 + 2] = v.z; tile[mrow][c4 + 3] = v.w;
  }
  __syncthreads();
  {
    const int quad = tid & 7, parity = (tid >> 3) & 1, q = tid >> 4;
    const int c = 2 * q + parity;
    const long long row = (IM2COL ? (long long)tap * g.C : 0) + c0 + c;
    unsigned short h[4], mm[4], l[4];
    if (!lo) {
      const float fs = f16_slot ? f16_slot[0] : f16_scale;
#pragma unroll
      for (int j = 0; j < 4; ++j) split2_f16(tile[quad * 4 + j][c], fs, h[j], mm[j]);
    } else {
#pragma unroll
      for (int j = 0; j < 4; ++j) split3_bf16(tile[quad * 4 + j][c], h[j], mm[j], l[j]);
    }
    const long long off = plane_offset(row, m0 + quad * 4, Kpad / 32, 1);
    *reinterpret_cast<uint2*>(hi + off) = make_uint2((unsigned)h[0] | ((unsigned)h[1] << 16), (unsigned)h[2] | ((unsigned)h[3] << 16));
    *reinterpret_cast<uint2*>(mid + off) = make_uint2((unsigned)mm[0] | ((unsigned)mm[1] << 16), (unsigned)mm[2] | ((unsigned)mm[3] << 16));
    if (lo) *reinterpret_cast<uint2*>(lo + off) = make_uint2((unsigned)l[0] | ((unsigned)l[1] << 16), (unsigned)l[2] | ((unsigned)l[3] << 16));
  }
}

size_t conv_wgrad_bf3_plane_elems(const ConvDesc& d, int which) {
  const size_t kpad = ((size_t)d.M() + 31) / 32 * 32;
  const size_t rows = which == 0 ? (size_t)d.CO : (size_t)d.K();
  return ((rows + 1) & ~(size_t)1) * kpad;
}
static bool wgrad_persist_shape(const ConvDesc& d) {
  const long long t22 = (long long)ceil_div(d.CO, 128) * ceil_div(d.K(), 128);
  return d.K() % 128 == 0 && t22 >= 32 && t22 < g_bf3_remainder_grid && (d.M() + 31) / 32 >= 64;
}
size_t conv_wgrad_bf3_ws_floats(const ConvDesc& d, int splitk) {
  size_t n = (size_t)ceil_div(d.CO, 64) * ceil_div(d.K(), 64) * splitk * 64 * 64;
  if (wgrad_persist_shape(d)) n = std::max(n, (size_t)4 * g_bf3_remainder_grid * 64 * 64);
  return n;
}

static Bf3Params conv_wgrad_bf3_params(const ConvDesc& d, unsigned short* const dyT[3], unsigned short* const pT[3], float* dw_ohwi, int fmt,
                                       const float* dy_slot, int splitk, float* ws, Bf3Work* w) {
  const int Kpad = (d.M() + 31) / 32 * 32;
  Bf3Params p{};
  p.M = d.CO; p.N = d.K(); p.K = Kpad;
  for (int i = 0; i < 3; ++i) { p.A.p[i] = dyT[i]; p.B.p[i] = pT[i]; }
  if (fmt) p.A.p[2] = p.B.p[2] = nullptr;
  p.A.kind = p.B.kind = OPK_ROWK; p.A.ld = p.B.ld = Kpad; p.A.paired = p.B.paired = 1;
  p.ep = ep_store(dw_ohwi, d.K(), nullptr, ACT_NONE);
  if (fmt) { p.fmt = 1; p.ep.alpha = 1.0f / kF16ActScale; p.ep.alpha_dev[0] = dy_slot + 1; }
  *w = g_bf3_wgrad_persist && wgrad_persist_shape(d) ? Bf3Work{ws, 4 * g_bf3_remainder_grid} : Bf3Work{nullptr, 256, splitk, ws};
  return p;
}

int conv_wgrad_bf3(const float* x, const ConvDesc& d, const float* dy, float* dw_ohwi, int splitk,
                   unsigned short* const dyT[3], unsigned short* const pT[3], float* ws, hipStream_t st, int fmt, const float* dy_slot) {
  DIC_REQUIRE(!d.in_nchw && d.C % 32 == 0 && d.CO % 32 == 0, "conv_wgrad_bf3: NHWC input, C and CO %% 32");
  DIC_REQUIRE(fmt == 0 || dy_slot, "conv_wgrad_bf3: the f16x2 format needs the scale slot of the gradient");
  const int M = d.M(), Kpad = (M + 31) / 32 * 32;
  const ConvGeom g = d.geom();
  hipLaunchKernelGGL((transpose_split_kernel<false>), dim3(Kpad / 32, d.CO / 32), dim3(256), 0, st, dy, (long long)d.CO, M,
                     Kpad, d.CO, g, dyT[0], dyT[1], fmt ? nullptr : dyT[2], 1.0f, fmt ? dy_slot : nullptr);
  hipLaunchKernelGGL((transpose_split_kernel<true>), dim3(Kpad / 32, d.KH * d.KW * (d.C / 32)), dim3(256), 0, st, x,
                     (long long)d.C, M, Kpad, d.C, g, pT[0], pT[1], fmt ? nullptr : pT[2], kF16ActScale, (const float*)nullptr);
  DIC_LAUNCH_CHECK();
  Bf3Work w; const Bf3Params p = conv_wgrad_bf3_params(d, dyT, pT, dw_ohwi, fmt, dy_slot, splitk, ws, &w);
  return launch_bf3(p, w, st);
}

__global__ void __launch_bounds__(256) stem_pack_image_kernel(const float* __restrict__ img, int B, int H, int W, int Hp,
                                                               int Wp, unsigned short* __restrict__ hi,
                                                               unsigned short* __restrict__ mid,
                                                               unsigned short* __restrict__ lo, unsigned* __restrict__ status) {
  const long long total = (long long)B * Hp * Wp;
  const long long stride = (long long)gridDim.x * 256;
  for (long long i = (long long)blockIdx.x * 256 + threadIdx.x; i < total; i += stride) {
    const int pw = (int)(i % Wp);
    const long long r = i / Wp;
    const int ph = (int)(r % Hp);
    const long long b = r / Hp;
    const int h = ph - 3, w = pw - 3;
    unsigned short a[4] = {0, 0, 0, 0}, m[4] = {0, 0, 0, 0}, l[4] = {0, 0, 0, 0};
    if ((unsigned)h < (unsigned)H && (unsigned)w < (unsigned)W) {
#pragma unroll
      for (int c = 0; c < 3; ++c) {
        const float v = img[((b * 3 + c) * H + h) * W + w];
        if (lo) split3_bf16(v, a[c], m[c], l[c]);
        else {
          if (f16x2_out_of_range(v, kF16ActScale)) f16x2_raise(status, 16u);
          split2_f16(v, kF16ActScale, a[c], m[c]);
        }
      }
    }
    reinterpret_cast<uint2*>(hi)[i] = make_uint2((unsigned)a[0] | ((unsigned)a[1] << 16), (unsigned)a[2] | ((unsigned)a[3] << 16));
    reinterpret_cast<uint2*>(mid)[i] = make_uint2((unsigned)m[0] | ((unsigned)m[1] << 16), (unsigned)m[2] | ((unsigned)m[3] << 16));
    if (lo) reinterpret_cast<uint2*>(lo)[i] = make_uint2((unsigned)l[0] | ((unsigned)l[1] << 16), (unsigned)l[2] | ((unsigned)l[3] << 16));
  }
}

__global__ void __launch_bounds__(256) stem_pack_weights_kernel(const float* __restrict__ w, int CO, float* __restrict__ out) {
  const int i = blockIdx.x * 256 + threadIdx.x;
  if (i >= CO * 224) return;
  const int c = i & 3, kw = (i >> 2) & 7, kh = (i >> 5) % 7, co = i / 224;
  out[i] = (c < 3 && kw < 7) ? w[((co * 3 + c) * 7 + kh) * 7 + kw] : 0.f;
}

size_t conv_stem_bf3_plane_elems(int B, int H, int W) { return (size_t)B * (H + 6) * (W + 8) * 4 + 64; }

int conv_stem_pack_weights(const float* w_oihw, int CO, float* scratch_f32, unsigned short* const w_planes[3], hipStream_t st, float f16_scale) {
  hipLaunchKernelGGL(stem_pack_weights_kernel, dim3(ceil_div(CO * 224, 256)), dim3(256), 0, st, w_oihw, CO, scratch_f32);
  DIC_LAUNCH_CHECK();
  if (f16_scale > 0.f) return split_f16x2_paired(scratch_f32, CO, 224, f16_scale, w_planes[0], w_planes[1], st, nullptr);
  return split_bf16x3_paired(scratch_f32, CO, 224, w_planes[0], w_planes[1], w_planes[2], st);
}

static Bf3Params conv_stem_bf3_params(int B, int H, int W, int CO, unsigned short* const x_planes[3], const unsigned short* const w_planes[3],
                                      float* y, float* bn_partial, int fmt, float out_scale) {
  const int Hp = H + 6, Wp = W + 8, OH = H / 2, OW = W / 2;
  Bf3Params p{};
  p.M = B * OH * OW; p.N = CO; p.K = 224;
  for (int i = 0; i < 3; ++i) { p.A.p[i] = x_planes[i]; p.B.p[i] = w_planes[i]; }
  p.A.kind = OPK_IM2COL; p.A.ld = 4; p.A.paired = 0;
  p.A.g = ConvGeom{Hp, Wp, 4, OH, OW, 7, 1, 2, 0, 2};
  p.B.kind = OPK_ROWK; p.B.ld = 224; p.B.paired = 1;
  p.ep = ep_store(y, CO, nullptr, ACT_NONE); p.ep.stats = bn_partial;
  if (fmt) { p.A.p[2] = p.B.p[2] = nullptr; p.fmt = 1; p.ep.alpha = out_scale; }
  return p;
}

int conv_stem_bf3(const float* imgs_nchw, int B, int H, int W, int CO, unsigned short* const x_planes[3],
                  const unsigned short* const w_planes[3], float* y, float* bn_partial, int* mtiles_out, hipStream_t st, int fmt,
                  float out_scale, unsigned* status) {
  DIC_REQUIRE(H % 2 == 0 && W % 2 == 0, "conv_stem_bf3: even image sizes");
  const int Hp = H + 6, Wp = W + 8;
  const long long px = (long long)B * Hp * Wp;
  hipLaunchKernelGGL(stem_pack_image_kernel, dim3((unsigned)std::min<long long>((px + 255) / 256, 16384)), dim3(256), 0, st,
                     imgs_nchw, B, H, W, Hp, Wp, x_planes[0], x_planes[1], fmt ? nullptr : x_planes[2], status);
  DIC_LAUNCH_CHECK();
  return launch_bf3(conv_stem_bf3_params(B, H, W, CO, x_planes, w_planes, y, bn_partial, fmt, out_scale), Bf3Work{}, st, nullptr, nullptr,
                    mtiles_out);
}
int conv_dgrad_s1_bf3(const unsigned short* const dy_planes[3], const ConvDesc& d,
                      const unsigned short* const wflip_planes[3], float* dx, hipStream_t st, float* tail_ws, int tail_ws_slabs,
                      int fmt, const float* alpha_dev0, const float* alpha_dev1) {
  DIC_REQUIRE(d.stride == 1 && d.CO % 32 == 0, "conv_dgrad_s1_bf3: stride 1, CO %% 32");
  const ConvDesc dd{d.B, d.OH(), d.OW(), d.CO, d.C, d.KH, d.KW, 1, d.KH - 1 - d.pad, 0};
  return conv_fwd_bf3(dy_planes, dd, wflip_planes, dx, nullptr, nullptr, tail_ws, st, nullptr, nullptr, nullptr, ACT_NONE,
                      tail_ws_slabs, fmt, 1.0f, alpha_dev0, alpha_dev1);
}

int bf3_plan_route(int route, int fmt, const ConvDesc& d, int flags, int splitk, int tail_ws_slabs, const char** kernel, int out[6]) {
  static float t[1];
  unsigned short* const u = reinterpret_cast<unsigned short*>(t), * const pl3[3] = {u, u, fmt ? nullptr : u};
  float* const stats = (flags & 16) ? nullptr : t, * const rbn = (flags & 4) ? t : nullptr;
  Bf3Params p{};
  Bf3Work w{(route == 4 || (route == 0 && (flags & 32))) ? nullptr : t, tail_ws_slabs};
  if (route == 0) p = conv_fwd_bf3_params(pl3, d, pl3, t, stats, (flags & 8) ? t : nullptr, ACT_NONE, fmt, 1.0f);
  else if (route == 1 && conv1x1_bn_bf3_shape_ok(d.M(), d.C))
    p = conv1x1_bn_bf3_params(t, t, t, (flags & 1) ? t : nullptr, 1, (flags & 2) ? t : nullptr, d.M(), d.C, pl3, d.CO, t, stats, fmt, 1.0f, nullptr, rbn, rbn);
  else if (route == 2 && conv3x3_bn_bf3_shape_ok(d, fmt)) p = conv3x3_bn_bf3_params(t, t, t, 1, d, pl3, t, stats, 1.0f, nullptr);
  else if (route == 3) p = conv_wgrad_bf3_params(d, pl3, pl3, t, fmt, t, splitk, t, &w);
  else if (route == 4) p = conv_stem_bf3_params(d.B, d.H, d.W, d.CO, pl3, pl3, t, stats, fmt, 1.0f);
  else { DIC_REQUIRE(route == 1 || route == 2, "bf3_plan_route: unknown route %d", route); return 1; }
  Bf3Plan pl;
  DIC_TRY(plan_bf3(p, w, &pl));
  const int fused = pl.fixup == BF3_FIX_TAIL64 && gemm_tail_fixup_bn_eligible(pl.fix, pl.fixup_n);
  *kernel = kBf3Kernels[pl.kernel].name;
  out[0] = pl.grid; out[1] = kBf3Kernels[pl.kernel].block; out[2] = pl.fixup + fused; out[3] = pl.fixup_n; out[4] = pl.rows; out[5] = pl.key;
  return DIC_OK;
}

int split_bf16x3_paired(const float* x, long long rows, int K, unsigned short* hi, unsigned short* mid,
                        unsigned short* lo, hipStream_t st) {
  DIC_REQUIRE(K % 32 == 0 && rows > 0, "split_bf16x3_paired: K %% 32");
  const long long n4 = ((rows + 1) >> 1) * (K / 2);
  const int blocks = (int)std::min<long long>((n4 + 255) / 256, 8192);
  hipLaunchKernelGGL(split_bf16x3_paired_kernel, dim3(blocks), dim3(256), 0, st, x, rows, K, hi, mid, lo);
  DIC_LAUNCH_CHECK();
  return DIC_OK;
}

int split_f16x2_paired(const float* x, long long rows, int K, float scale, unsigned short* h1, unsigned short* h2, hipStream_t st,
                       unsigned* status) {
  DIC_REQUIRE(K % 32 == 0 && rows > 0 && scale > 0.f, "split_f16x2_paired: K %% 32, scale > 0");
  const long long n4 = ((rows + 1) >> 1) * (K / 2);
  const int blocks = (int)std::min<long long>((n4 + 255) / 256, 8192);
  hipLaunchKernelGGL(split_f16x2_paired_kernel, dim3(blocks), dim3(256), 0, st, x, rows, K, scale, h1, h2, status);
  DIC_LAUNCH_CHECK();
  return DIC_OK;
}

int split_bf16x3(const float* x, long long n, unsigned short* hi, unsigned short* mid, unsigned short* lo, hipStream_t st) {
  const int blocks = (int)std::min<long long>((n + 255) / 256, 8192);
  hipLaunchKernelGGL(split_bf16x3_kernel, dim3(blocks), dim3(256), 0, st, x, n, hi, mid, lo);
  DIC_LAUNCH_CHECK();
  return DIC_OK;
}

}

using namespace dic;

extern "C" {

int dic_split_bf16x3(const float* x, long long n, uint16_t* hi, uint16_t* mid, uint16_t* lo, void* stream) {
  DIC_REQUIRE(x && hi && mid && lo && n > 0, "split_bf16x3: bad arguments");
  return split_bf16x3(x, n, hi, mid, lo, (hipStream_t)stream);
}

int dic_split_bf16x3_paired(const float* x, long long rows, int K, uint16_t* hi, uint16_t* mid, uint16_t* lo,
                            void* stream) {
  DIC_REQUIRE(x && hi && mid && lo && rows > 0 && K > 0, "split_bf16x3_paired: bad arguments");
  return split_bf16x3_paired(x, rows, K, hi, mid, lo, (hipStream_t)stream);
}

// ... 110 lines not shown
```

depth_image_captioning_pub_amd/csrc/nn_kernels.h:

```cpp
#pragma once
#include "common.h"

namespace dic {

constexpr float kBnEps = 1e-5f;
constexpr float kBnMomentum = 0.1f;

struct BnBuf {
  float *scale, *shift, *mean, *invstd;
};

struct F16Scale {
  unsigned* bound;
  float* slot;
};
int f16_scale_reset(unsigned* bounds, int n, hipStream_t st);
int f16_scale_from_absmax(const float* x, long long n, F16Scale s, hipStream_t st);
int f16_scale_finish(F16Scale s, hipStream_t st);

void bn_finalize_two_level_rows(int rows);
size_t bn_finalize_ws_doubles(long long max_mtiles, int C);
int bn_finalize_train(const float* partial, int mtiles, long long count, int C, const float* gamma,
                      const float* beta, float* running_mean, float* running_var, BnBuf out, double* red,
                      hipStream_t st, unsigned* status = nullptr)   ;
int bn_finalize_eval(int C, const float* gamma, const float* beta, const float* running_mean,
                     const float* running_var, BnBuf out, hipStream_t st);
int bn_apply(const float* x, const float* residual, float* y, long long rows, int C, BnBuf bn, int relu,
             hipStream_t st);
int bn_apply_planes(const float* x, const float* residual, const unsigned short* const residual_planes[3], float* y,
                    unsigned short* const planes[3], long long rows, int C, BnBuf bn, int relu, hipStream_t st,
                    const BnBuf* residual_bn = nullptr   ,
                    unsigned* status = nullptr)          ;
int bn_relu_maxpool(const float* x, int B, int H, int W, int C, const BnBuf* bn, int relu, int k, int s, int p,
                    float* y, unsigned char* idx, hipStream_t st,
                    unsigned short* const planes[3] = nullptr   ,
                    unsigned* status = nullptr                  ,
                    float* xsel = nullptr                        );
int poison_if_raised(float* y, long long n, const unsigned* status, hipStream_t st);
int clear_status(unsigned* status, hipStream_t st);
int adaptive_avgpool(const float* x, int B, int H, int W, int C, const BnBuf* bn, int relu, int out, float* y,
                     hipStream_t st);
int adaptive_avgpool_bwd(const float* dy, int B, int H, int W, int C, int out, float* dx, hipStream_t st);

int maxpool_relu_bwd(const float* dpool, const unsigned char* idx, const float* x, int B, int H, int W, int C,
                     int k, BnBuf bn, float* dy, hipStream_t st);
int relu_mask_bwd(float* dy, const float* x, long long rows, int C, BnBuf bn, hipStream_t st);
int bn_backward(float* dy_dx, const float* x, long long rows, int C, const float* gamma, BnBuf bn, float* dgamma,
                float* dbeta, float* ws, hipStream_t st,
                unsigned short* const dx_planes[3] = nullptr   ,
                F16Scale* f16 = nullptr)                        ;
int bn_pool_backward(const float* dpool, const unsigned char* idx, const float* x, int B, int H, int W, int C, int k,
                     const float* gamma, BnBuf bn, float* dgamma, float* dbeta, float* ws, float* dy, hipStream_t st,
                     unsigned short* const dy_planes[3] = nullptr   ,
                     F16Scale* f16 = nullptr)                        ;
void bn_backward_ws_layout(float* ws, int C, float** part, float** k2, float** k3);
int bn_backward_finalize(const float* part, int chunks, int C, double rows, float* dgamma, float* dbeta, float* k2, float* k3, hipStream_t st);
size_t bn_backward_ws_floats(int C);
int relu_mask_export(const float* x, long long rows, int C, BnBuf bn, unsigned char* out, hipStream_t st);
int colsum_rows(const float* X, long long ld, long long rows, int C, float* out, float* ws, hipStream_t st);
int oihw_to_ohwi(const float* src, float* dst, int O, int I, int KH, int KW, hipStream_t st);
int ohwi_to_oihw(const float* src, float* dst, int O, int I, int KH, int KW, hipStream_t st);

}
```

depth_image_captioning_pub_amd/csrc/nn_kernels.hip:

```cpp
#include "nn_kernels.h"
#include "gemm.h"
#include <algorithm>

namespace dic {

static inline int ew_blocks(long long n_items) { return (int)std::min<long long>((n_items + 255) / 256, 8192); }

struct FastDiv { unsigned m, s; };
static inline FastDiv make_fastdiv(unsigned d) {
  unsigned s = 0;
  while ((1u << s) < d) ++s;
  return FastDiv{(unsigned)((((unsigned long long)1 << 32) * (((unsigned long long)1 << s) - d)) / d + 1), s};
}
__device__ __forceinline__ unsigned fast_div(unsigned x, FastDiv f) { return (__umulhi(x, f.m) + x) >> f.s; }

__global__ void __launch_bounds__(1024) bn_finalize_train_kernel(const float* __restrict__ partial, int mtiles,
                                                                  double count, int C, const float* __restrict__ gamma,
                                                                  const float* __restrict__ beta,
                                                                  float* __restrict__ rmean, float* __restrict__ rvar,
                                                                  BnBuf out, unsigned* __restrict__ status) {
  __shared__ double s1[32][33], s2[32][33];
  const int cl = threadIdx.x & 31, g = threadIdx.x >> 5;
  const int c = blockIdx.x * 32 + cl;
  double a = 0.0, b = 0.0;
// ... 263 lines not shown
  DIC_REQUIRE(C % 32 == 0, "bn_apply_planes: C %% 32");
  DIC_REQUIRE(planes[2] || !residual_planes, "bn_apply_planes: f16x2 planes (planes[2] == NULL) are not exact - the residual must be fp32");
  const long long n4 = ((rows + 1) >> 1) * (C / 4);
  const unsigned short* r0 = residual_planes ? residual_planes[0] : nullptr;
  const unsigned short* r1 = residual_planes ? residual_planes[1] : nullptr;
  const unsigned short* r2 = residual_planes ? residual_planes[2] : nullptr;
  hipLaunchKernelGGL(bn_apply_planes_kernel, dim3(ew_blocks(n4)), dim3(256), 0, st, x, residual, r0, r1, r2, y, planes[0],
                     planes[1], planes[2], rows, C, bn, relu, residual_bn ? residual_bn->scale : nullptr,
                     residual_bn ? residual_bn->shift : nullptr, status);
  DIC_LAUNCH_CHECK();
  return DIC_OK;
}

__global__ void __launch_bounds__(256) bn_relu_maxpool_kernel(const float* __restrict__ x, int B, int H, int W, int C4,
                                                               BnBuf bn, int has_bn, int relu, int k, int s, int p,
                                                               int PH, int PW, float* __restrict__ y,
                                                               unsigned char* __restrict__ idx,
                                                               unsigned short* __restrict__ hi,
                                                               unsigned short* __restrict__ mid,
                                                               unsigned short* __restrict__ lo, unsigned* __restrict__ status,
                                                               FastDiv dC4, FastDiv dPW, FastDiv dPH, float* __restrict__ xsel) {
  const unsigned total = (unsigned)B * PH * PW * C4;
  const unsigned stride = gridDim.x * 256u;
  for (unsigned i = blockIdx.x * 256u + threadIdx.x; i < total; i += stride) {
    const unsigned row = fast_div(i, dC4);
    const int c4 = (int)(i - row * (unsigned)C4);
    const unsigned r1 = fast_div(row, dPW);
    const int pw = (int)(row - r1 * (unsigned)PW);
    const int b = (int)fast_div(r1, dPH);
    const int ph = (int)(r1 - (unsigned)b * (unsigned)PH);
    float4 sc = make_float4(1.f, 1.f, 1.f, 1.f), sh = make_float4(0.f, 0.f, 0.f, 0.f);
    if (has_bn) {
      sc = *reinterpret_cast<const float4*>(bn.scale + c4 * 4);
      sh = *reinterpret_cast<const float4*>(bn.shift + c4 * 4);
    }
    float4 best = make_float4(-INFINITY, -INFINITY, -INFINITY, -INFINITY);
    float4 braw = make_float4(0.f, 0.f, 0.f, 0.f);
    uchar4 bi = make_uchar4(0, 0, 0, 0);
    for (int kh = 0; kh < k; ++kh) {
      const int h = ph * s - p + kh;
      if ((unsigned)h >= (unsigned)H) continue;
      for (int kw = 0; kw < k; ++kw) {
        const int w = pw * s - p + kw;
        if ((unsigned)w >= (unsigned)W) continue;
        float4 v = reinterpret_cast<const float4*>(x)[(((long long)b * H + h) * W + w) * C4 + c4];
        const float4 raw = v;
        v.x = v.x * sc.x + sh.x; v.y = v.y * sc.y + sh.y; v.z = v.z * sc.z + sh.z; v.w = v.w * sc.w + sh.w;
        if (relu) { v.x = fmaxf(v.x, 0.f); v.y = fmaxf(v.y, 0.f); v.z = fmaxf(v.z, 0.f); v.w = fmaxf(v.w, 0.f); }
        const unsigned char id = (unsigned char)(kh * k + kw);
        if (v.x > best.x) { best.x = v.x; bi.x = id; braw.x = raw.x; }
        if (v.y > best.y) { best.y = v.y; bi.y = id; braw.y = raw.y; }
        if (v.z > best.z) { best.z = v.z; bi.z = id; braw.z = raw.z; }
        if (v.w > best.w) { best.w = v.w; bi.w = id; braw.w = raw.w; }
      }
    }
    if (y) reinterpret_cast<float4*>(y)[i] = best;
    if (idx) reinterpret_cast<uchar4*>(idx)[i] = bi;
    if (xsel) reinterpret_cast<float4*>(xsel)[i] = braw;
    if (hi) {
      const long long off = plane_offset((long long)row, c4 * 4, C4 / 8, 1);
      unsigned short h[4], m[4], l[4];
      if (!lo) {
        if (f16x2_out_of_range(best.x, kF16ActScale) | f16x2_out_of_range(best.y, kF16ActScale) | f16x2_out_of_range(best.z, kF16ActScale) |
            f16x2_out_of_range(best.w, kF16ActScale)) f16x2_raise(status, 2u);
        split2_f16(best.x, kF16ActScale, h[0], m[0]); split2_f16(best.y, kF16ActScale, h[1], m[1]);
        split2_f16(best.z, kF16ActScale, h[2], m[2]); split2_f16(best.w, kF16ActScale, h[3], m[3]);
      } else {
        split3_bf16(best.x, h[0], m[0], l[0]); split3_bf16(best.y, h[1], m[1], l[1]);
        split3_bf16(best.z, h[2], m[2], l[2]); split3_bf16(best.w, h[3], m[3], l[3]);
      }
      *reinterpret_cast<uint2*>(hi + off) = make_uint2((unsigned)h[0] | ((unsigned)h[1] << 16), (unsigned)h[2] | ((unsigned)h[3] << 16));
      *reinterpret_cast<uint2*>(mid + off) = make_uint2((unsigned)m[0] | ((unsigned)m[1] << 16), (unsigned)m[2] | ((unsigned)m[3] << 16));
      if (lo) *reinterpret_cast<uint2*>(lo + off) = make_uint2((unsigned)l[0] | ((unsigned)l[1] << 16), (unsigned)l[2] | ((unsigned)l[3] << 16));
    }
  }
}

int bn_relu_maxpool(const float* x, int B, int H, int W, int C, const BnBuf* bn, int relu, int k, int s, int p,
                    float* y, unsigned char* idx, hipStream_t st, unsigned short* const planes[3], unsigned* status, float* xsel) {
  DIC_REQUIRE(C % 4 == 0, "maxpool: C %% 4");
  DIC_REQUIRE(y || planes, "maxpool: no output");
  DIC_REQUIRE(!planes || C % 32 == 0, "maxpool: plane output needs C %% 32");
  const int PH = (H + 2 * p - k) / s + 1, PW = (W + 2 * p - k) / s + 1;
  const long long total = (long long)B * PH * PW * (C / 4);
  DIC_REQUIRE(total < (1ll << 31) - (1ll << 22), "maxpool: more than 2^31 output elements");
  BnBuf z{};
  hipLaunchKernelGGL(bn_relu_maxpool_kernel, dim3(ew_blocks(total)), dim3(256), 0, st, x, B, H, W, C / 4, bn ? *bn : z,
                     bn ? 1 : 0, relu, k, s, p, PH, PW, y, idx, planes ? planes[0] : nullptr, planes ? planes[1] : nullptr,
                     planes ? planes[2] : nullptr, status, make_fastdiv((unsigned)(C / 4)), make_fastdiv((unsigned)PW), make_fastdiv((unsigned)PH), xsel);
  DIC_LAUNCH_CHECK();
  return DIC_OK;
}

__global__ void __launch_bounds__(256) poison_if_raised_kernel(float* __restrict__ y, long long n, const unsigned* __restrict__ status) {
  if (*status == 0u) return;
  const float nan = __uint_as_float(0x7fc00000u);
  for (long long i = (long long)blockIdx.x * 256 + threadIdx.x; i < n; i += (long long)gridDim.x * 256) y[i] = nan;
}
__global__ void clear_status_kernel(unsigned* __restrict__ status) { status[threadIdx.x] = 0u; }
int clear_status(unsigned* status, hipStream_t st) {
  hipLaunchKernelGGL(clear_status_kernel, dim3(1), dim3(64), 0, st, status);
  DIC_LAUNCH_CHECK();
  return DIC_OK;
}
int poison_if_raised(float* y, long long n, const unsigned* status, hipStream_t st) {
  hipLaunchKernelGGL(poison_if_raised_kernel, dim3(64), dim3(256), 0, st, y, n, status);
  DIC_LAUNCH_CHECK();
  return DIC_OK;
}

__global__ void __launch_bounds__(256) adaptive_avgpool_kernel(const float* __restrict__ x, int B, int H, int W, int C4,
                                                                BnBuf bn, int has_bn, int relu, int OUT,
                                                                float* __restrict__ y) {
  const long long total = (long long)B * OUT * OUT * C4;
  const long long stride = (long long)gridDim.x * 256;
  for (long long i = (long long)blockIdx.x * 256 + threadIdx.x; i < total; i += stride) {
    const int c4 = (int)(i % C4);
    long long r = i / C4;
    const int oj = (int)(r % OUT); r /= OUT;
    const int oi = (int)(r % OUT);
    const int b = (int)(r / OUT);
    const int h0 = (oi * H) / OUT, h1 = ((oi + 1) * H + OUT - 1) / OUT;
    const int w0 = (oj * W) / OUT, w1 = ((oj + 1) * W + OUT - 1) / OUT;
    float4 sc = make_float4(1.f, 1.f, 1.f, 1.f), sh = make_float4(0.f, 0.f, 0.f, 0.f);
    if (has_bn) {
      sc = *reinterpret_cast<const float4*>(bn.scale + c4 * 4);
      sh = *reinterpret_cast<const float4*>(bn.shift + c4 * 4);
    }
    float4 acc = make_float4(0.f, 0.f, 0.f, 0.f);
    for (int h = h0; h < h1; ++h)
      for (int w = w0; w < w1; ++w) {
        float4 v = reinterpret_cast<const float4*>(x)[(((long long)b * H + h) * W + w) * C4 + c4];
        v.x = v.x * sc.x + sh.x; v.y = v.y * sc.y + sh.y; v.z = v.z * sc.z + sh.z; v.w = v.w * sc.w + sh.w;
        if (relu) { v.x = fmaxf(v.x, 0.f); v.y = fmaxf(v.y, 0.f); v.z = fmaxf(v.z, 0.f); v.w = fmaxf(v.w, 0.f); }
        acc.x += v.x; acc.y += v.y; acc.z += v.z; acc.w += v.w;
      }
    const float n = (float)((h1 - h0) * (w1 - w0));
    acc.x /= n; acc.y /= n; acc.z /= n; acc.w /= n;
    reinterpret_cast<float4*>(y)[i] = acc;
  }
}

int adaptive_avgpool(const float* x, int B, int H, int W, int C, const BnBuf* bn, int relu, int out, float* y,
                     hipStream_t st) {
  DIC_REQUIRE(C % 4 == 0, "avgpool: C %% 4");
  const long long total = (long long)B * out * out * (C / 4);
  BnBuf z{};
  hipLaunchKernelGGL(adaptive_avgpool_kernel, dim3(ew_blocks(total)), dim3(256), 0, st, x, B, H, W, C / 4,
                     bn ? *bn : z, bn ? 1 : 0, relu, out, y);
  DIC_LAUNCH_CHECK();
  return DIC_OK;
}

__global__ void __launch_bounds__(256) adaptive_avgpool_bwd_kernel(const float* __restrict__ dy, int B, int H, int W,
                                                                    int C4, int OUT, float* __restrict__ dx) {
  const long long total = (long long)B * H * W * C4;
  const long long stride = (long long)gridDim.x * 256;
  for (long long i = (long long)blockIdx.x * 256 + threadIdx.x; i < total; i += stride) {
    const int c4 = (int)(i % C4);
    long long r = i / C4;
    const int w = (int)(r % W); r /= W;
    const int h = (int)(r % H);
    const int b = (int)(r / H);
    float4 acc = make_float4(0.f, 0.f, 0.f, 0.f);
    const int oi_lo = max(0, (h * OUT) / H - 1), oi_hi = min(OUT - 1, ((h + 1) * OUT + H - 1) / H + 1);
    const int oj_lo = max(0, (w * OUT) / W - 1), oj_hi = min(OUT - 1, ((w + 1) * OUT + W - 1) / W + 1);
    for (int oi = oi_lo; oi <= oi_hi; ++oi) {
      const int h0 = (oi * H) / OUT, h1 = ((oi + 1) * H + OUT - 1) / OUT;
      if (h < h0 || h >= h1) continue;
      for (int oj = oj_lo; oj <= oj_hi; ++oj) {
        const int w0 = (oj * W) / OUT, w1 = ((oj + 1) * W + OUT - 1) / OUT;
        if (w < w0 || w >= w1) continue;
        const float inv = 1.0f / (float)((h1 - h0) * (w1 - w0));
        const float4 g = reinterpret_cast<const float4*>(dy)[(((long long)b * OUT + oi) * OUT + oj) * C4 + c4];
        acc.x += g.x * inv; acc.y += g.y * inv; acc.z += g.z * inv; acc.w += g.w * inv;
      }
    }
    reinterpret_cast<float4*>(dx)[i] = acc;
  }
}

int adaptive_avgpool_bwd(const float* dy, int B, int H, int W, int C, int out, float* dx, hipStream_t st) {
  const long long total = (long long)B * H * W * (C / 4);
  hipLaunchKernelGGL(adaptive_avgpool_bwd_kernel, dim3(ew_blocks(total)), dim3(256), 0, st, dy, B, H, W, C / 4, out, dx);
  DIC_LAUNCH_CHECK();
  return DIC_OK;
}

__global__ void __launch_bounds__(256) maxpool_relu_bwd_kernel(const float* __restrict__ dpool,
                                                                const unsigned char* __restrict__ idx,
                                                                const float* __restrict__ x, int B, int H, int W, int C4,
                                                                int k, int PH, int PW, BnBuf bn, float* __restrict__ dy) {
  const long long total = (long long)B * H * W * C4;
  const long long stride = (long long)gridDim.x * 256;
  for (long long i = (long long)blockIdx.x * 256 + threadIdx.x; i < total; i += stride) {
    const int c4 = (int)(i % C4);
    long long r = i / C4;
    const int w = (int)(r % W); r /= W;
    const int h = (int)(r % H);
    const int b = (int)(r / H);
    const int ph = h / k, pw = w / k;
    float4 g = make_float4(0.f, 0.f, 0.f, 0.f);
    if (ph < PH && pw < PW) {
      const long long po = (((long long)b * PH + ph) * PW + pw) * C4 + c4;
      const float4 d = reinterpret_cast<const float4*>(dpool)[po];
      const uchar4 id = reinterpret_cast<const uchar4*>(idx)[po];
      const unsigned char me = (unsigned char)((h - ph * k) * k + (w - pw * k));
      const float4 v = reinterpret_cast<const float4*>(x)[i];
      const float4 sc = *reinterpret_cast<const float4*>(bn.scale + c4 * 4);
      const float4 sh = *reinterpret_cast<const float4*>(bn.shift + c4 * 4);
      g.x = (id.x == me && v.x * sc.x + sh.x > 0.f) ? d.x : 0.f;
      g.y = (id.y == me && v.y * sc.y + sh.y > 0.f) ? d.y : 0.f;
      g.z = (id.z == me && v.z * sc.z + sh.z > 0.f) ? d.z : 0.f;
      g.w = (id.w == me && v.w * sc.w + sh.w > 0.f) ? d.w : 0.f;
    }
    reinterpret_cast<float4*>(dy)[i] = g;
  }
}

int maxpool_relu_bwd(const float* dpool, const unsigned char* idx, const float* x, int B, int H, int W, int C, int k,
                     BnBuf bn, float* dy, hipStream_t st) {
  const long long total = (long long)B * H * W * (C / 4);
  hipLaunchKernelGGL(maxpool_relu_bwd_kernel, dim3(ew_blocks(total)), dim3(256), 0, st, dpool, idx, x, B, H, W, C / 4,
                     k, H / k, W / k, bn, dy);
  DIC_LAUNCH_CHECK();
  return DIC_OK;
}

__device__ __forceinline__ bool relu_passes(float v, float sc, float sh) { return fmaf(v, sc, sh) > 0.f; }

__global__ void __launch_bounds__(256) relu_mask_bwd_kernel(float* __restrict__ dy, const float* __restrict__ x,
                                                             long long n4, int C4, BnBuf bn) {
  const long long stride = (long long)gridDim.x * 256;
  for (long long i = (long long)blockIdx.x * 256 + threadIdx.x; i < n4; i += stride) {
    const int c = (int)(i % C4) * 4;
    const float4 v = reinterpret_cast<const float4*>(x)[i];
    const float4 sc = *reinterpret_cast<const float4*>(bn.scale + c);
    const float4 sh = *reinterpret_cast<const float4*>(bn.shift + c);
    float4 g = reinterpret_cast<float4*>(dy)[i];
    if (!relu_passes(v.x, sc.x, sh.x)) g.x = 0.f;
    if (!relu_passes(v.y, sc.y, sh.y)) g.y = 0.f;
    if (!relu_passes(v.z, sc.z, sh.z)) g.z = 0.f;
    if (!relu_passes(v.w, sc.w, sh.w)) g.w = 0.f;
    reinterpret_cast<float4*>(dy)[i] = g;
  }
}

__global__ void __launch_bounds__(256) relu_mask_export_kernel(const float* __restrict__ x, long long n, int C, BnBuf bn,
                                                                unsigned char* __restrict__ out) {
  const long long stride = (long long)gridDim.x * 256;
  for (long long i = (long long)blockIdx.x * 256 + threadIdx.x; i < n; i += stride) {
    const int c = (int)(i % C);
    out[i] = relu_passes(x[i], bn.scale[c], bn.shift[c]) ? 1 : 0;
  }
}

int relu_mask_export(const float* x, long long rows, int C, BnBuf bn, unsigned char* out, hipStream_t st) {
  hipLaunchKernelGGL(relu_mask_export_kernel, dim3(ew_blocks(rows * C)), dim3(256), 0, st, x, rows * C, C, bn, out);
  DIC_LAUNCH_CHECK();
  return DIC_OK;
}

int relu_mask_bwd(float* dy, const float* x, long long rows, int C, BnBuf bn, hipStream_t st) {
  const long long n4 = rows * C / 4;
  hipLaunchKernelGGL(relu_mask_bwd_kernel, dim3(ew_blocks(n4)), dim3(256), 0, st, dy, x, n4, C / 4, bn);
  DIC_LAUNCH_CHECK();
  return DIC_OK;
}

__global__ void __launch_bounds__(64) f16_scale_reset_kernel(unsigned* __restrict__ bounds, int n) {
  if ((int)threadIdx.x < n) bounds[threadIdx.x] = 0u;
}
__global__ void __launch_bounds__(256) absmax_kernel(const float* __restrict__ x, long long n4, unsigned* __restrict__ bound) {
  __shared__ float sm[4];
  float m = 0.f;
  for (long long i = (long long)blockIdx.x * 256 + threadIdx.x; i < n4; i += (long long)gridDim.x * 256) {
    const float4 v = reinterpret_cast<const float4*>(x)[i];
    m = fmaxf(fmaxf(m, fmaxf(fabsf(v.x), fabsf(v.y))), fmaxf(fabsf(v.z), fabsf(v.w)));
    if (v.x != v.x || v.y != v.y || v.z != v.z || v.w != v.w) m = __uint_as_float(0x7f800000u);
  }
  m = wave_max(m);
  if ((threadIdx.x & 63) == 0) sm[threadIdx.x >> 6] = m;
  __syncthreads();
  if (threadIdx.x == 0) atomicMax(bound, __float_as_uint(fmaxf(fmaxf(sm[0], sm[1]), fmaxf(sm[2], sm[3]))));
}
__global__ void __launch_bounds__(64) f16_scale_finish_kernel(const unsigned* __restrict__ bound, float* __restrict__ slot) {
  if (threadIdx.x != 0) return;
  const int e = min(60, max(-60, (int)((*bound >> 23) & 0xffu) - 127));
  slot[0] = __uint_as_float((unsigned)(13 - e + 127) << 23);
  slot[1] = __uint_as_float((unsigned)(e - 13 + 127) << 23);
}
int f16_scale_reset(unsigned* bounds, int n, hipStream_t st) {
  DIC_REQUIRE(n <= 64, "f16_scale_reset: at most 64 words");
  hipLaunchKernelGGL(f16_scale_reset_kernel, dim3(1), dim3(64), 0, st, bounds, n);
  DIC_LAUNCH_CHECK();
  return DIC_OK;
}
int f16_scale_finish(F16Scale sl, hipStream_t st) {
  hipLaunchKernelGGL(f16_scale_finish_kernel, dim3(1), dim3(64), 0, st, (const unsigned*)sl.bound, sl.slot);
  DIC_LAUNCH_CHECK();
  return DIC_OK;
}
int f16_scale_from_absmax(const float* x, long long n, F16Scale sl, hipStream_t st) {
  DIC_REQUIRE(n % 4 == 0, "f16_scale_from_absmax: n %% 4");
  hipLaunchKernelGGL(absmax_kernel, dim3((unsigned)std::min<long long>((n / 4 + 255) / 256, 128)), dim3(256), 0, st, x, n / 4, sl.bound);
  DIC_LAUNCH_CHECK();
  return f16_scale_finish(sl, st);
}

constexpr int kBnChunksMax = 512;
static inline int reduce_chunks(int C) { return std::min(kBnChunksMax, std::max(64, 1024 / std::max(1, C / 64))); }
__global__ void __launch_bounds__(256) bn_bwd_reduce_kernel(const float* __restrict__ dy, const float* __restrict__ x,
                                                             long long rows, int C, BnBuf bn, float* __restrict__ part,
                                                             float* __restrict__ gmaxp) {
  __shared__ float4 sa[16][16], sb[16][16];
  __shared__ float smax[4];
  float gm = 0.f;
  const int c4l = threadIdx.x & 15, rl = threadIdx.x >> 4;
  const int c = blockIdx.x * 64 + c4l * 4;
  const long long per = (rows + gridDim.y - 1) / gridDim.y;
  const long long r0 = (long long)blockIdx.y * per, r1 = min(rows, r0 + per);
  float4 a = make_float4(0.f, 0.f, 0.f, 0.f), b = a;
  if (c < C) {
    const float4 mu = *reinterpret_cast<const float4*>(bn.mean + c);
    const float4 is = *reinterpret_cast<const float4*>(bn.invstd + c);
    for (long long r = r0 + rl; r < r1; r += 64) {
      float4 g[4], v[4];
#pragma unroll
      for (int u = 0; u < 4; ++u) {
        const long long rr = r + 16 * u;
        const long long rc = min(rr, r1 - 1);
        g[u] = *reinterpret_cast<const float4*>(dy + rc * C + c);
        v[u] = *reinterpret_cast<const float4*>(x + rc * C + c);
        if (rr >= r1) g[u] = make_float4(0.f, 0.f, 0.f, 0.f);
      }
#pragma unroll
      for (int u = 0; u < 4; ++u) {
        a.x += g[u].x; a.y += g[u].y; a.z += g[u].z; a.w += g[u].w;
        b.x += g[u].x * (v[u].x - mu.x) * is.x; b.y += g[u].y * (v[u].y - mu.y) * is.y;
        b.z += g[u].z * (v[u].z - mu.z) * is.z; b.w += g[u].w * (v[u].w - mu.w) * is.w;
        gm = fmaxf(fmaxf(gm, fmaxf(fabsf(g[u].x), fabsf(g[u].y))), fmaxf(fabsf(g[u].z), fabsf(g[u].w)));
      }
    }
  }
  sa[rl][c4l] = a; sb[rl][c4l] = b;
  if (gmaxp) { gm = wave_max(gm); if ((threadIdx.x & 63) == 0) smax[threadIdx.x >> 6] = gm; }
  __syncthreads();
  if (gmaxp && threadIdx.x == 0) gmaxp[(long long)blockIdx.y * gridDim.x + blockIdx.x] = fmaxf(fmaxf(smax[0], smax[1]), fmaxf(smax[2], smax[3]));
  if (rl == 0 && c < C) {
#pragma unroll
    for (int i = 1; i < 16; ++i) {
      a.x += sa[i][c4l].x; a.y += sa[i][c4l].y; a.z += sa[i][c4l].z; a.w += sa[i][c4l].w;
      b.x += sb[i][c4l].x; b.y += sb[i][c4l].y; b.z += sb[i][c4l].z; b.w += sb[i][c4l].w;
    }
    *reinterpret_cast<float4*>(part + ((long long)blockIdx.y * 2 + 0) * C + c) = a;
    *reinterpret_cast<float4*>(part + ((long long)blockIdx.y * 2 + 1) * C + c) = b;
  }
}

__global__ void __launch_bounds__(256) bn_bwd_finalize_kernel(const float* __restrict__ part, int chunks, int C,
                                                               double rows, float* __restrict__ dgamma,
                                                               float* __restrict__ dbeta, float* __restrict__ k2,
                                                               float* __restrict__ k3, const float* __restrict__ gmaxp,
                                                               const float* __restrict__ gamma, const float* __restrict__ invstd,
                                                               unsigned* __restrict__ bound) {
  __shared__ double sa[8][32], sb[8][32];
  __shared__ float sg[8][32];
  const int cl = threadIdx.x & 31, g = threadIdx.x >> 5;
  const int c = blockIdx.x * 32 + cl;
  double a = 0.0, b = 0.0;
  float gm = 0.f;
  if (c < C) {
    const int cb = c >> 6, ncb = C >> 6;
    for (int t0 = g; t0 < chunks; t0 += 64) {
      float va[8], vb[8], vg[8];
#pragma unroll
      for (int u = 0; u < 8; ++u) {
        const int t = t0 + 8 * u, tc = min(t, chunks - 1);
        va[u] = part[((long long)tc * 2 + 0) * C + c];
        vb[u] = part[((long long)tc * 2 + 1) * C + c];
        vg[u] = bound ? gmaxp[(long long)tc * ncb + cb] : 0.f;
        if (t >= chunks) { va[u] = 0.f; vb[u] = 0.f; vg[u] = 0.f; }
      }
#pragma unroll
      for (int u = 0; u < 8; ++u) { a += (double)va[u]; b += (double)vb[u]; gm = fmaxf(gm, vg[u]); }
    }
  }
  sa[g][cl] = a; sb[g][cl] = b; sg[g][cl] = gm;
  __syncthreads();
  float bnd = 0.f;
  if (g == 0 && c < C) {
#pragma unroll
    for (int i = 1; i < 8; ++i) { a += sa[i][cl]; b += sb[i][cl]; gm = fmaxf(gm, sg[i][cl]); }
    dbeta[c] = (float)a;
    dgamma[c] = (float)b;
    k2[c] = (float)(a / rows);
    k3[c] = (float)(b / rows);
    if (bound) {
      bnd = fabsf(gamma[c] * invstd[c]) * (gm + fabsf((float)(a / rows)) + sqrtf((float)rows) * fabsf((float)(b / rows)));
      if (bnd != bnd) bnd = __uint_as_float(0x7f800000u);
    }
  }
  if (bound && threadIdx.x < 64) {
    bnd = wave_max(bnd);
    if (threadIdx.x == 0) atomicMax(bound, __float_as_uint(bnd));
  }
}

__global__ void __launch_bounds__(256) bn_bwd_apply_kernel(float* __restrict__ dy, const float* __restrict__ x,
                                                            long long n4, int C4, const float* __restrict__ gamma,
                                                            BnBuf bn, const float* __restrict__ k2,
                                                            const float* __restrict__ k3,
                                                            unsigned short* __restrict__ hi,
                                                            unsigned short* __restrict__ mid,
                                                            unsigned short* __restrict__ lo, const float* __restrict__ f16_slot) {
  const long long stride = (long long)gridDim.x * 256;
  const float fs = f16_slot ? f16_slot[0] : 1.f;
  for (long long i = (long long)blockIdx.x * 256 + threadIdx.x; i < n4; i += stride) {
    const int c = (int)(i % C4) * 4;
    const float4 g = reinterpret_cast<float4*>(dy)[i];
    const float4 v = reinterpret_cast<const float4*>(x)[i];
    const float4 mu = *reinterpret_cast<const float4*>(bn.mean + c);
    const float4 is = *reinterpret_cast<const float4*>(bn.invstd + c);
    const float4 ga = *reinterpret_cast<const float4*>(gamma + c);
    const float4 a2 = *reinterpret_cast<const float4*>(k2 + c);
    const float4 a3 = *reinterpret_cast<const float4*>(k3 + c);
    float4 o;
    o.x = ga.x * is.x * (g.x - a2.x - (v.x - mu.x) * is.x * a3.x);
    o.y = ga.y * is.y * (g.y - a2.y - (v.y - mu.y) * is.y * a3.y);
    o.z = ga.z * is.z * (g.z - a2.z - (v.z - mu.z) * is.z * a3.z);
    o.w = ga.w * is.w * (g.w - a2.w - (v.w - mu.w) * is.w * a3.w);
    reinterpret_cast<float4*>(dy)[i] = o;
    if (hi) {
      const long long off = plane_offset(i / C4, c, C4 / 8, 1);
      unsigned short h[4], m[4], l[4];
      if (!lo) {
        split2_f16(o.x, fs, h[0], m[0]); split2_f16(o.y, fs, h[1], m[1]); split2_f16(o.z, fs, h[2], m[2]); split2_f16(o.w, fs, h[3], m[3]);
      } else {
        split3_bf16(o.x, h[0], m[0], l[0]); split3_bf16(o.y, h[1], m[1], l[1]);
        split3_bf16(o.z, h[2], m[2], l[2]); split3_bf16(o.w, h[3], m[3], l[3]);
      }
      *reinterpret_cast<uint2*>(hi + off) = make_uint2((unsigned)h[0] | ((unsigned)h[1] << 16), (unsigned)h[2] | ((unsigned)h[3] << 16));
      *reinterpret_cast<uint2*>(mid + off) = make_uint2((unsigned)m[0] | ((unsigned)m[1] << 16), (unsigned)m[2] | ((unsigned)m[3] << 16));
      if (lo) *reinterpret_cast<uint2*>(lo + off) = make_uint2((unsigned)l[0] | ((unsigned)l[1] << 16), (unsigned)l[2] | ((unsigned)l[3] << 16));
    }
  }
}

size_t bn_backward_ws_floats(int C) { return (size_t)kBnChunksMax * 2 * C + 2 * (size_t)C + (size_t)kBnChunksMax * (C / 64 + 1); }

int bn_backward(float* dy_dx, const float* x, long long rows, int C, const float* gamma, BnBuf bn, float* dgamma,
                float* dbeta, float* ws, hipStream_t st, unsigned short* const dx_planes[3], F16Scale* f16) {
  DIC_REQUIRE(C % 64 == 0, "bn_backward: C %% 64");
  const bool f16x2 = dx_planes && !dx_planes[2];
  DIC_REQUIRE(!f16x2 || (f16 && f16->bound && f16->slot), "bn_backward: f16x2 planes need a scale slot");
  float* part = ws;
  float* k2 = ws + (size_t)kBnChunksMax * 2 * C;
  float* k3 = k2 + C;
  float* gmaxp = k3 + C;
  const int chunks = reduce_chunks(C);
  hipLaunchKernelGGL(bn_bwd_reduce_kernel, dim3(C / 64, chunks), dim3(256), 0, st, dy_dx, x, rows, C, bn, part, f16x2 ? gmaxp : nullptr);
  hipLaunchKernelGGL(bn_bwd_finalize_kernel, dim3(ceil_div(C, 32)), dim3(256), 0, st, part, chunks, C, (double)rows,
                     dgamma, dbeta, k2, k3, (const float*)gmaxp, gamma, (const float*)bn.invstd, f16x2 ? f16->bound : nullptr);
  if (f16x2) DIC_TRY(f16_scale_finish(*f16, st));
  const long long n4 = rows * C / 4;
  hipLaunchKernelGGL(bn_bwd_apply_kernel, dim3(ew_blocks(n4)), dim3(256), 0, st, dy_dx, x, n4, C / 4, gamma, bn, k2, k3,
                     dx_planes ? dx_planes[0] : nullptr, dx_planes ? dx_planes[1] : nullptr,
                     dx_planes ? dx_planes[2] : nullptr, f16x2 ? (const float*)f16->slot : nullptr);
  DIC_LAUNCH_CHECK();
  return DIC_OK;
}

void bn_backward_ws_layout(float* ws, int C, float** part, float** k2, float** k3) {
  *part = ws; *k2 = ws + (size_t)kBnChunksMax * 2 * C; *k3 = *k2 + C;
}
int bn_backward_finalize(const float* part, int chunks, int C, double rows, float* dgamma, float* dbeta, float* k2, float* k3, hipStream_t st) {
  DIC_REQUIRE(chunks >= 1 && chunks <= kBnChunksMax && C % 64 == 0, "bn_backward_finalize: chunks <= %d, C %% 64", kBnChunksMax);
  hipLaunchKernelGGL(bn_bwd_finalize_kernel, dim3(ceil_div(C, 32)), dim3(256), 0, st, part, chunks, C, rows, dgamma, dbeta, k2, k3,
                     (const float*)nullptr, (const float*)nullptr, (const float*)nullptr, (unsigned*)nullptr);
  DIC_LAUNCH_CHECK();
  return DIC_OK;
}

struct PoolGeom { int H, W, k, PH, PW; FastDiv dH, dW, dk; };

__device__ __forceinline__ float4 pool_relu_grad4(const float* __restrict__ dpool, const unsigned char* __restrict__ idx,
                                                  const float4 v, const float4 sc, const float4 sh, unsigned row,
                                                  int c4, int C4, PoolGeom pg) {
  const unsigned r2 = fast_div(row, pg.dW);
  const int w = (int)(row - r2 * (unsigned)pg.W);
  const unsigned b = fast_div(r2, pg.dH);
  const int h = (int)(r2 - b * (unsigned)pg.H);
  const int ph = (int)fast_div((unsigned)h, pg.dk), pw = (int)fast_div((unsigned)w, pg.dk);
  float4 g = make_float4(0.f, 0.f, 0.f, 0.f);
  if (ph < pg.PH && pw < pg.PW) {
    const long long po = (((long long)b * pg.PH + ph) * pg.PW + pw) * C4 + c4;
    const float4 d = reinterpret_cast<const float4*>(dpool)[po];
    const uchar4 id = reinterpret_cast<const uchar4*>(idx)[po];
    const unsigned char me = (unsigned char)((h - ph * pg.k) * pg.k + (w - pw * pg.k));
    g.x = (id.x == me && v.x * sc.x + sh.x > 0.f) ? d.x : 0.f;
    g.y = (id.y == me && v.y * sc.y + sh.y > 0.f) ? d.y : 0.f;
    g.z = (id.z == me && v.z * sc.z + sh.z > 0.f) ? d.z : 0.f;
    g.w = (id.w == me && v.w * sc.w + sh.w > 0.f) ? d.w : 0.f;
  }
  return g;
}

__global__ void __launch_bounds__(256) bn_pool_bwd_reduce_kernel(const float* __restrict__ dpool,
                                                                  const unsigned char* __restrict__ idx,
                                                                  const float* __restrict__ x, long long rows, int C,
                                                                  PoolGeom pg, BnBuf bn, float* __restrict__ part,
                                                                  float* __restrict__ gmaxp) {
  __shared__ float4 sa[16][16], sb[16][16];
  __shared__ float smax[4];
  float gm = 0.f;
  const int c4l = threadIdx.x & 15, rl = threadIdx.x >> 4;
  const int c = blockIdx.x * 64 + c4l * 4;
  const long long per = (rows + gridDim.y - 1) / gridDim.y;
  const long long r0 = (long long)blockIdx.y * per, r1 = min(rows, r0 + per);
  float4 a = make_float4(0.f, 0.f, 0.f, 0.f), b = a;
  if (c < C) {
    const float4 mu = *reinterpret_cast<const float4*>(bn.mean + c);
    const float4 is = *reinterpret_cast<const float4*>(bn.invstd + c);
    const float4 sc = *reinterpret_cast<const float4*>(bn.scale + c);
    const float4 sh = *reinterpret_cast<const float4*>(bn.shift + c);
    for (long long r = r0 + rl; r < r1; r += 128) {
      float4 v[8];
#pragma unroll
      for (int u = 0; u < 8; ++u) v[u] = *reinterpret_cast<const float4*>(x + min(r + 16 * u, r1 - 1) * C + c);
#pragma unroll
      for (int u = 0; u < 8; ++u) {
        const long long rr = r + 16 * u;
        if (rr < r1) {
          const float4 g = pool_relu_grad4(dpool, idx, v[u], sc, sh, (unsigned)rr, c >> 2, C >> 2, pg);
          a.x += g.x; a.y += g.y; a.z += g.z; a.w += g.w;
          b.x += g.x * (v[u].x - mu.x) * is.x; b.y += g.y * (v[u].y - mu.y) * is.y;
          b.z += g.z * (v[u].z - mu.z) * is.z; b.w += g.w * (v[u].w - mu.w) * is.w;
          gm = fmaxf(fmaxf(gm, fmaxf(fabsf(g.x), fabsf(g.y))), fmaxf(fabsf(g.z), fabsf(g.w)));
        }
      }
    }
  }
  sa[rl][c4l] = a; sb[rl][c4l] = b;
  if (gmaxp) { gm = wave_max(gm); if ((threadIdx.x & 63) == 0) smax[threadIdx.x >> 6] = gm; }
  __syncthreads();
  if (gmaxp && threadIdx.x == 0) gmaxp[(long long)blockIdx.y * gridDim.x + blockIdx.x] = fmaxf(fmaxf(smax[0], smax[1]), fmaxf(smax[2], smax[3]));
  if (rl == 0 && c < C) {
#pragma unroll
    for (int i = 1; i < 16; ++i) {
      a.x += sa[i][c4l].x; a.y += sa[i][c4l].y; a.z += sa[i][c4l].z; a.w += sa[i][c4l].w;
      b.x += sb[i][c4l].x; b.y += sb[i][c4l].y; b.z += sb[i][c4l].z; b.w += sb[i][c4l].w;
    }
    *reinterpret_cast<float4*>(part + ((long long)blockIdx.y * 2 + 0) * C + c) = a;
    *reinterpret_cast<float4*>(part + ((long long)blockIdx.y * 2 + 1) * C + c) = b;
  }
}

__global__ void __launch_bounds__(256) bn_pool_bwd_apply_kernel(const float* __restrict__ dpool,
                                                                 const unsigned char* __restrict__ idx,
                                                                 const float* __restrict__ x, float* __restrict__ dy,
                                                                 long long n4, int C4, PoolGeom pg,
                                                                 const float* __restrict__ gamma, BnBuf bn,
                                                                 const float* __restrict__ k2,
                                                                 const float* __restrict__ k3,
                                                                 unsigned short* __restrict__ hi,
                                                                 unsigned short* __restrict__ mid,
                                                                 unsigned short* __restrict__ lo, const float* __restrict__ f16_slot,
                                                                 FastDiv dC4) {
  const long long stride = (long long)gridDim.x * 256;
  const float fs = f16_slot ? f16_slot[0] : 1.f;
  const int c4 = (int)(threadIdx.x % (unsigned)C4), c = c4 * 4;
  const float4 sc = *reinterpret_cast<const float4*>(bn.scale + c);
  const float4 sh = *reinterpret_cast<const float4*>(bn.shift + c);
  const float4 mu = *reinterpret_cast<const float4*>(bn.mean + c);
  const float4 is = *reinterpret_cast<const float4*>(bn.invstd + c);
  const float4 ga = *reinterpret_cast<const float4*>(gamma + c);
  const float4 a2 = *reinterpret_cast<const float4*>(k2 + c);
  const float4 a3 = *reinterpret_cast<const float4*>(k3 + c);
  auto finish = [&](long long i, const float4 v) {
    const unsigned row = fast_div((unsigned)i, dC4);
    const float4 g = pool_relu_grad4(dpool, idx, v, sc, sh, row, c4, C4, pg);
    float4 o;
    o.x = ga.x * is.x * (g.x - a2.x - (v.x - mu.x) * is.x * a3.x);
    o.y = ga.y * is.y * (g.y - a2.y - (v.y - mu.y) * is.y * a3.y);
    o.z = ga.z * is.z * (g.z - a2.z - (v.z - mu.z) * is.z * a3.z);
    o.w = ga.w * is.w * (g.w - a2.w - (v.w - mu.w) * is.w * a3.w);
    reinterpret_cast<float4*>(dy)[i] = o;
    if (hi) {
      const long long off = plane_offset((long long)row, c, C4 / 8, 1);
      unsigned short h[4], m[4], l[4];
      if (!lo) {
        split2_f16(o.x, fs, h[0], m[0]); split2_f16(o.y, fs, h[1], m[1]); split2_f16(o.z, fs, h[2], m[2]); split2_f16(o.w, fs, h[3], m[3]);
      } else {
        split3_bf16(o.x, h[0], m[0], l[0]); split3_bf16(o.y, h[1], m[1], l[1]);
        split3_bf16(o.z, h[2], m[2], l[2]); split3_bf16(o.w, h[3], m[3], l[3]);
      }
      *reinterpret_cast<uint2*>(hi + off) = make_uint2((unsigned)h[0] | ((unsigned)h[1] << 16), (unsigned)h[2] | ((unsigned)h[3] << 16));
      *reinterpret_cast<uint2*>(mid + off) = make_uint2((unsigned)m[0] | ((unsigned)m[1] << 16), (unsigned)m[2] | ((unsigned)m[3] << 16));
      if (lo) *reinterpret_cast<uint2*>(lo + off) = make_uint2((unsigned)l[0] | ((unsigned)l[1] << 16), (unsigned)l[2] | ((unsigned)l[3] << 16));
    }
  };
  long long i = (long long)blockIdx.x * 256 + threadIdx.x;
  for (; i + stride < n4; i += 2 * stride) {
    const float4 v0 = reinterpret_cast<const float4*>(x)[i], v1 = reinterpret_cast<const float4*>(x)[i + stride];
    finish(i, v0);
    finish(i + stride, v1);
  }
  if (i < n4) finish(i, reinterpret_cast<const float4*>(x)[i]);
}

int bn_pool_backward(const float* dpool, const unsigned char* idx, const float* x, int B, int H, int W, int C, int k,
                     const float* gamma, BnBuf bn, float* dgamma, float* dbeta, float* ws, float* dy, hipStream_t st,
                     unsigned short* const dy_planes[3], F16Scale* f16) {
  DIC_REQUIRE(C % 64 == 0, "bn_pool_backward: C %% 64");
  const bool f16x2 = dy_planes && !dy_planes[2];
  DIC_REQUIRE(!f16x2 || (f16 && f16->bound && f16->slot), "bn_pool_backward: f16x2 planes need a scale slot");
  const long long rows = (long long)B * H * W;
  DIC_REQUIRE((long long)B * H * W * C / 4 < (1ll << 31) && 256 % (C / 4) == 0, "bn_pool_backward: index range / C <= 1024 with C / 4 dividing 256");
  const PoolGeom pg{H, W, k, H / k, W / k, make_fastdiv((unsigned)H), make_fastdiv((unsigned)W), make_fastdiv((unsigned)k)};
  float* part = ws;
  float* k2 = ws + (size_t)kBnChunksMax * 2 * C;
  float* k3 = k2 + C;
  float* gmaxp = k3 + C;
  const int chunks = reduce_chunks(C);
  hipLaunchKernelGGL(bn_pool_bwd_reduce_kernel, dim3(C / 64, chunks), dim3(256), 0, st, dpool, idx, x, rows, C, pg, bn,
                     part, f16x2 ? gmaxp : nullptr);
  hipLaunchKernelGGL(bn_bwd_finalize_kernel, dim3(ceil_div(C, 32)), dim3(256), 0, st, part, chunks, C, (double)rows,
                     dgamma, dbeta, k2, k3, (const float*)gmaxp, gamma, (const float*)bn.invstd, f16x2 ? f16->bound : nullptr);
  if (f16x2) DIC_TRY(f16_scale_finish(*f16, st));
  const long long n4 = rows * C / 4;
  hipLaunchKernelGGL(bn_pool_bwd_apply_kernel, dim3(ew_blocks(n4)), dim3(256), 0, st, dpool, idx, x, dy, n4, C / 4, pg,
                     gamma, bn, k2, k3, dy_planes ? dy_planes[0] : nullptr, dy_planes ? dy_planes[1] : nullptr,
                     dy_planes ? dy_planes[2] : nullptr, f16x2 ? (const float*)f16->slot : nullptr, make_fastdiv((unsigned)(C / 4)));
  DIC_LAUNCH_CHECK();
  return DIC_OK;
}

__global__ void __launch_bounds__(256) colsum_rows_v4_kernel(const float* __restrict__ X, long long ld, long long rows,
                                                              int C, float* __restrict__ out) {
  __shared__ float4 sa[16][16];
  const int c4l = threadIdx.x & 15, rl = threadIdx.x >> 4;
  const int c = blockIdx.x * 64 + c4l * 4;
  const long long per = (rows + gridDim.y - 1) / gridDim.y;
  const long long r0 = (long long)blockIdx.y * per, r1 = min(rows, r0 + per);
  float4 a = make_float4(0.f, 0.f, 0.f, 0.f);
  if (c < C)
    for (long long r = r0 + rl; r < r1; r += 128) {
      float4 g[8];
#pragma unroll
      for (int u = 0; u < 8; ++u) {
        const long long rr = r + 16 * u;
        g[u] = *reinterpret_cast<const float4*>(X + min(rr, r1 - 1) * ld + c);
        if (rr >= r1) g[u] = make_float4(0.f, 0.f, 0.f, 0.f);
      }
#pragma unroll
      for (int u = 0; u < 8; ++u) { a.x += g[u].x; a.y += g[u].y; a.z += g[u].z; a.w += g[u].w; }
    }
  sa[rl][c4l] = a;
  __syncthreads();
  if (rl == 0 && c < C) {
#pragma unroll
    for (int i = 1; i < 16; ++i) { a.x += sa[i][c4l].x; a.y += sa[i][c4l].y; a.z += sa[i][c4l].z; a.w += sa[i][c4l].w; }
    *reinterpret_cast<float4*>(out + (long long)blockIdx.y * C + c) = a;
  }
}

__global__ void __launch_bounds__(256) colsum_rows_kernel(const float* __restrict__ X, long long ld, long long rows,
                                                           int C, float* __restrict__ out, int chunks) {
  const int c = blockIdx.x * 256 + threadIdx.x;
  if (c >= C) return;
  const long long per = (rows + chunks - 1) / chunks;
  const long long r0 = (long long)blockIdx.y * per, r1 = min(rows, r0 + per);
  float s = 0.f;
#pragma unroll 8
  for (long long r = r0; r < r1; ++r) s += X[r * ld + c];
  out[(long long)blockIdx.y * C + c] = s;
}

int colsum_rows(const float* X, long long ld, long long rows, int C, float* out, float* ws, hipStream_t st) {
  const bool v4 = (C % 4 == 0) && (ld % 4 == 0) && ((reinterpret_cast<uintptr_t>(X) & 15) == 0) && rows >= 256;
  if (v4) {
    const int chunks = std::min(256, reduce_chunks(C));
    hipLaunchKernelGGL(colsum_rows_v4_kernel, dim3(ceil_div(C, 64), chunks), dim3(256), 0, st, X, ld, rows, C, ws);
    hipLaunchKernelGGL(colsum_rows_kernel, dim3(ceil_div(C, 256), 1), dim3(256), 0, st, ws, (long long)C,
                       (long long)chunks, C, out, 1);
    DIC_LAUNCH_CHECK();
    return DIC_OK;
  }
  const int chunks = (int)std::min<long long>(256, std::max<long long>(1, rows / 16));
  if (chunks > 1) {
    hipLaunchKernelGGL(colsum_rows_kernel, dim3(ceil_div(C, 256), chunks), dim3(256), 0, st, X, ld, rows, C, ws, chunks);
    hipLaunchKernelGGL(colsum_rows_kernel, dim3(ceil_div(C, 256), 1), dim3(256), 0, st, ws, (long long)C,
                       (long long)chunks, C, out, 1);
  } else {
    hipLaunchKernelGGL(colsum_rows_kernel, dim3(ceil_div(C, 256), 1), dim3(256), 0, st, X, ld, rows, C, out, 1);
  }
  DIC_LAUNCH_CHECK();
  return DIC_OK;
}

__global__ void __launch_bounds__(256) oihw_ohwi_kernel(const float* __restrict__ src, float* __restrict__ dst, int O,
                                                         int I, int KH, int KW, int to_ohwi) {
  const long long total = (long long)O * I * KH * KW;
  const long long stride = (long long)gridDim.x * 256;
  for (long long e = (long long)blockIdx.x * 256 + threadIdx.x; e < total; e += stride) {
    const int i = (int)(e % I);
    long long r = e / I;
    const int kw = (int)(r % KW); r /= KW;
    const int kh = (int)(r % KH);
    const int o = (int)(r / KH);
    const long long oihw = (((long long)o * I + i) * KH + kh) * KW + kw;
    if (to_ohwi) dst[e] = src[oihw];
    else dst[oihw] = src[e];
  }
}

int oihw_to_ohwi(const float* src, float* dst, int O, int I, int KH, int KW, hipStream_t st) {
  const long long total = (long long)O * I * KH * KW;
  hipLaunchKernelGGL(oihw_ohwi_kernel, dim3(ew_blocks(total)), dim3(256), 0, st, src, dst, O, I, KH, KW, 1);
  DIC_LAUNCH_CHECK();
  return DIC_OK;
}

int ohwi_to_oihw(const float* src, float* dst, int O, int I, int KH, int KW, hipStream_t st) {
  const long long total = (long long)O * I * KH * KW;
  hipLaunchKernelGGL(oihw_ohwi_kernel, dim3(ew_blocks(total)), dim3(256), 0, st, src, dst, O, I, KH, KW, 0);
  DIC_LAUNCH_CHECK();
  return DIC_OK;
}

}
```

include/dic.h:

```cpp
#ifndef DIC_H_
#define DIC_H_
#include <stddef.h>
#include <stdint.h>

#ifdef __cplusplus
extern "C" {
#endif

#define DIC_L 196
#define DIC_D 2048
#define DIC_A 128
#define DIC_E 128
#define DIC_H 128

#define DIC_ABI_VERSION 200
int dic_version(void);
const char* dic_last_error(void);
size_t dic_struct_bytes(int which);

int dic_gemm_f32(int M, int N, int K, const float* A, long long lda, int a_colk, const float* B, long long ldb,
                 int b_colk, float* C, long long ldc, const float* bias, int act, int accumulate, int splitk,
                 float* workspace, size_t workspace_bytes, int force_tile, void* stream);

int dic_conv2d_fwd(const float* x, int B, int H, int W, int C, int in_nchw, const float* w_ohwi, const float* bias,
// ... 138 lines not shown
                      float temp, const float* d_ctx, const float* d_alpha, float* g_enc_att_w, float* g_enc_att_b,
                      float* g_dec_att_w, float* g_dec_att_b, float* g_full_att_w, float* g_full_att_b, float* d_feats,
                      float* d_h, void* workspace, size_t workspace_bytes, void* stream);

int dic_caption_loss(const float* logits, const int64_t* targets, int n_packed, int V, const float* alphas, int B,
                     int Tmax, float lam, float ce_grad_scale, float reg_grad_scale, float* loss, float* dlogits,
                     float* dalphas, float* scratch, void* stream);
int dic_pack_targets(const int64_t* captions, int cap_stride, const int* dec_lengths, int B, int64_t* targets,
                     void* stream);

int dic_adamw_step(float* params, const float* grads, float* exp_avg, float* exp_avg_sq, long long n, int step,
                   float lr, float beta1, float beta2, float eps, float weight_decay, void* stream);
int dic_adamw_step_guarded(float* params, const float* grads, float* exp_avg, float* exp_avg_sq, long long n, int step,
                           float lr, float beta1, float beta2, float eps, float weight_decay, const uint32_t* skip_if_raised,
                           void* stream);

#define DIC_COMM_ID_BYTES 128
typedef struct dic_comm dic_comm;
int dic_comm_unique_id(void* id128);
int dic_comm_create(const void* id128, int nranks, int rank, dic_comm** out);
int dic_allreduce_grads(dic_comm* comm, float* flat_grad, long long count, void* stream);
int dic_comm_ranks(const dic_comm* comm, int* nranks, int* rank);
int dic_comm_destroy(dic_comm* comm);
int dic_comm_info(char* buf, size_t bytes);

int dic_dropout_mask(float* out, long long n, float p, uint64_t seed, uint64_t offset, void* stream);

typedef struct dic_depth_encoder_weights {
  const float *conv1_w, *conv1_b, *bn1_w, *bn1_b;
  const float *conv2_w, *conv2_b, *bn2_w, *bn2_b;
  const float *conv3_w, *conv3_b, *bn3_w, *bn3_b;
} dic_depth_encoder_weights;
typedef struct dic_depth_encoder_grads {
  float *conv1_w, *conv1_b, *bn1_w, *bn1_b, *conv2_w, *conv2_b, *bn2_w, *bn2_b, *conv3_w, *conv3_b, *bn3_w, *bn3_b;
} dic_depth_encoder_grads;
typedef struct dic_depth_bn_state {
  float *rm1, *rv1, *rm2, *rv2, *rm3, *rv3;
} dic_depth_bn_state;

size_t dic_depth_encoder_workspace_bytes(int B, int H, int W);
int dic_depth_encoder_fwd(const dic_depth_encoder_weights* w, const dic_depth_bn_state* s, const float* depth, int B,
                          int H, int W, int train, float* features, void* workspace, size_t workspace_bytes,
                          void* stream);
int dic_depth_encoder_bwd(const dic_depth_encoder_weights* w, const float* depth, const float* d_features, int B, int H,
                          int W, const dic_depth_encoder_grads* g, void* workspace, size_t workspace_bytes,
                          void* stream);
int dic_depth_encoder_fwd_map(const dic_depth_encoder_weights* w, const dic_depth_bn_state* s, const float* depth, int B,
                              int H, int W, int train, float* feature_map, void* workspace, size_t workspace_bytes,
                              void* stream);
int dic_depth_encoder_bwd_map(const dic_depth_encoder_weights* w, const float* depth, const float* d_feature_map, int B,
                              int H, int W, const dic_depth_encoder_grads* gr, void* workspace, size_t workspace_bytes,
                              void* stream);

int dic_depth_encoder_inspect(const void* workspace, size_t workspace_bytes, int B, int H, int W, int which, void* out,
                              long long* n_out, void* stream);
int dic_decoder_inspect(const void* workspace, size_t workspace_bytes, int B, int Tmax, int V, int n_packed, int cells, int which,
                        float* out, long long* n_out, void* stream);

typedef struct dic_conv_bn_layer {
  const float* w;
  const float *gamma, *beta;
  float *running_mean, *running_var;
  const uint16_t *w_hi, *w_mid, *w_lo;
  float w_scale;
} dic_conv_bn_layer;

int dic_oihw_to_ohwi(const float* src, float* dst, int O, int I, int KH, int KW, void* stream);
int dic_resnet_pack_stem_weights(const float* w_oihw, float* scratch_f32, uint16_t* w_hi, uint16_t* w_mid, uint16_t* w_lo,
                                 void* stream);
int dic_resnet_pack_stem_weights_f16x2(const float* w_oihw, float* scratch_f32, uint16_t* w_h1, uint16_t* w_h2, float w_scale, void* stream);
int dic_resnet_num_layers(const int* blocks);
size_t dic_resnet_workspace_bytes(int B, int H, int W, const int* blocks, int mode);
int dic_resnet_fwd(const dic_conv_bn_layer* layers, int n_layers, const int* blocks, const float* imgs_nchw, int B,
                   int H, int W, int train_bn, int mode, float* features, void* workspace, size_t workspace_bytes,
                   void* stream);
int dic_resnet_fwd_map(const dic_conv_bn_layer* layers, int n_layers, const int* blocks, const float* imgs_nchw, int B,
                       int H, int W, int train_bn, int mode, float* feature_map, void* workspace, size_t workspace_bytes,
                       void* stream);

int dic_split_bf16x3(const float* x, long long n, uint16_t* hi, uint16_t* mid, uint16_t* lo, void* stream);
int dic_split_bf16x3_paired(const float* x, long long rows, int K, uint16_t* hi, uint16_t* mid, uint16_t* lo,
                            void* stream);
int dic_split_f16x2_paired(const float* x, long long rows, int K, float scale, uint16_t* h1, uint16_t* h2, void* stream);
int dic_split_f16x2_paired_checked(const float* x, long long rows, int K, float scale, uint16_t* h1, uint16_t* h2, uint32_t* overflow,
                                   void* stream);
int dic_gemm_bf16x3_paired(int M, int N, int K, const uint16_t* a_hi, const uint16_t* a_mid, const uint16_t* a_lo,
                           const uint16_t* b_hi, const uint16_t* b_mid, const uint16_t* b_lo, float* C, long long ldc,
                           const float* bias, void* stream);
int dic_linear_bf16x3(int M, int N, int K, const uint16_t* const x_planes[3], const uint16_t* const w_planes[3], const float* bias,
                      int act, int accumulate, float* C, long long ldc, void* stream);
int dic_conv2d_bf16x3(const uint16_t* const x_planes[3], int B, int H, int W, int C, const uint16_t* const w_planes[3],
                      const float* bias, int CO, int KH, int KW, int stride, int pad, int act, float* y_nhwc, float* tail_ws,
                      void* stream);
int dic_linear_f16x2(int M, int N, int K, const uint16_t* const x_planes[2], const uint16_t* const w_planes[2], const float* bias,
                     int act, int accumulate, float* C, long long ldc, float out_scale, void* stream);
int dic_conv2d_f16x2(const uint16_t* const x_planes[2], int B, int H, int W, int Cin, const uint16_t* const w_planes[2],
                     const float* bias, int CO, int KH, int KW, int stride, int pad, int act, float* y_nhwc, float* tail_ws,
                     float out_scale, void* stream);
int dic_gemm_bf16x3(int M, int N, int K, const uint16_t* a_hi, const uint16_t* a_mid, const uint16_t* a_lo,
                    long long lda, const uint16_t* b_hi, const uint16_t* b_mid, const uint16_t* b_lo, long long ldb,
                    float* C, long long ldc, const float* bias, void* stream);

int dic_weight_standardize(const float* w, int O, int K, float eps, float* out, void* stream);
int dic_pad_nhwc(const float* x, int B, int H, int W, int C, int top, int left, int bottom, int right, float value,
                 float* out, void* stream);
int dic_maxpool_nhwc(const float* x, int B, int H, int W, int C, int k, int stride, float* out, void* stream);
size_t dic_groupnorm_workspace_bytes(int B, int groups);
int dic_groupnorm_nhwc(const float* x, int B, long long HW, int C, int groups, const float* gamma, const float* beta,
                       float eps, const float* residual, int relu, float* out, void* workspace, void* stream);
int dic_layernorm(const float* x, long long rows, int C, const float* gamma, const float* beta, float eps, float* out,
                  void* stream);
size_t dic_vit_attention_workspace_bytes(int B, int N, int heads);
int dic_vit_attention(const float* qkv, int B, int N, int heads, int head_dim, float* out, void* workspace,
                      size_t workspace_bytes, void* stream);
int dic_upsample2x_bilinear_nhwc(const float* x, int B, int H, int W, int C, float* out, void* stream);
int dic_add_act(const float* a, const float* b, long long n, long long period, int act, float* out, void* stream);
int dic_pointwise_dot(const float* x, long long rows, int C, const float* w, const float* bias, int relu, float* out,
                      void* stream);

int dic_normalize_images(const float* in, float* out, int B, int C, int H, int W, const float* mean3, const float* std3,
                         void* stream);
int dic_resize_bilinear(const float* in, int planes, int H, int W, int resize_short, int crop, float mul, float add,
                        float* out, void* stream);
int dic_depth_standardize(float* depth, int B, long long hw, void* stream);
int dic_bn_ema_update(float* running, const float* delta, long long n, float momentum, void* stream);
int dic_bn_ema_update_guarded(float* running, const float* delta, long long n, float momentum, const uint32_t* skip_if_raised,
                              void* stream);
int dic_gather_rows(const float* table, const int64_t* idx, int n, long long row_floats, float* out, void* stream);

int dic_debug_force_staged_gemm(int on);
int dic_debug_bn_finalize(const float* partial, int mtiles, long long count, int C, const float* gamma, const float* beta,
                          float* running_mean, float* running_var, float* scale, float* shift, float* mean, float* invstd, double* red,
                          size_t red_doubles, uint32_t* status, void* stream);
int dic_debug_bn_finalize_eval(int C, const float* gamma, const float* beta, const float* running_mean, const float* running_var,
                               float* scale, float* shift, float* mean, float* invstd, void* stream);
int dic_debug_bn_apply(const float* x, const float* residual, const uint16_t* const residual_planes[3], float* y, uint16_t* const planes[3],
                       long long rows, int C, const float* scale, const float* shift, const float* mean, const float* invstd, int relu,
                       const float* res_scale, const float* res_shift, const float* res_mean, const float* res_invstd, uint32_t* status,
                       void* stream);
int dic_debug_bn_relu_maxpool(const float* x, int B, int H, int W, int C, const float* scale, const float* shift, const float* mean,
                              const float* invstd, int relu, int k, int s, int p, float* y, unsigned char* idx, uint16_t* const planes[3],
                              uint32_t* status, float* xsel, void* stream);
int dic_debug_adaptive_avgpool(const float* x, int B, int H, int W, int C, const float* scale, const float* shift, const float* mean,
                               const float* invstd, int relu, int out, float* y, void* stream);
int dic_debug_adaptive_avgpool_bwd(const float* dy, int B, int H, int W, int C, int out, float* dx, void* stream);
int dic_debug_maxpool_relu_bwd(const float* dpool, const unsigned char* idx, const float* x, int B, int H, int W, int C, int k,
                               const float* scale, const float* shift, const float* mean, const float* invstd, float* dy, void* stream);
int dic_debug_relu_mask_bwd(float* dy, const float* x, long long rows, int C, const float* scale, const float* shift, const float* mean,
                            const float* invstd, void* stream);
int dic_debug_bn_backward_ws_floats(int C);
int dic_debug_bn_backward(float* dy_dx, const float* x, long long rows, int C, const float* gamma, const float* scale, const float* shift,
                          const float* mean, const float* invstd, float* dgamma, float* dbeta, float* ws, size_t ws_floats,
                          uint16_t* const dx_planes[3], uint32_t* f16_bound, float* f16_slot, void* stream);
int dic_debug_bn_pool_backward(const float* dpool, const unsigned char* idx, const float* x, int B, int H, int W, int C, int k,
                               const float* gamma, const float* scale, const float* shift, const float* mean, const float* invstd,
                               float* dgamma, float* dbeta, float* ws, size_t ws_floats, float* dy, uint16_t* const dy_planes[3],
                               uint32_t* f16_bound, float* f16_slot, void* stream);
int dic_debug_colsum_rows(const float* X, long long ld, long long rows, int C, float* out, float* ws, size_t ws_floats, void* stream);
int dic_debug_f16_scale_reset(uint32_t* bounds, int n, void* stream);
int dic_debug_f16_scale_from_absmax(const float* x, long long n, uint32_t* bound, float* slot, void* stream);
int dic_debug_f16_scale_finish(uint32_t* bound, float* slot, void* stream);
int dic_debug_conv_wgrad_sizes(int B, int H, int W, int C, int CO, int k, int stride, int pad, int splitk, size_t* dyT_elems, size_t* pT_elems,
                               size_t* ws_floats);
int dic_debug_conv_wgrad(const float* x, int B, int H, int W, int C, int CO, int k, int stride, int pad, const float* dy, float* dw_ohwi,
                         int splitk, uint16_t* const dyT[3], size_t dyT_elems, uint16_t* const pT[3], size_t pT_elems, float* ws,
                         size_t ws_floats, int fmt, const float* dy_slot, void* stream);
int dic_debug_conv_dgrad_s1(const uint16_t* const dy_planes[3], int B, int H, int W, int C, int CO, int k, int pad,
                            const uint16_t* const wflip_planes[3], float* dx, float* tail_ws, int tail_ws_slabs, int fmt, const float* alpha_dev0,
                            const float* alpha_dev1, void* stream);
int dic_debug_depth_prepare_weights(const float* w2_oihw, const float* w3_oihw, uint16_t* const w2_pl[3], uint16_t* const w2f_pl[3],
                                    uint16_t* const w3_pl[3], uint16_t* const w3f_pl[3], size_t w2_plane_elems, size_t w3_plane_elems,
                                    const float* slots, void* stream);
int dic_debug_conv_wgrad_f32(const float* x, int B, int H, int W, int C, int in_nchw, int CO, int k, int stride, int pad, const float* dy, float* dw_ohwi,
                             int splitk, float* ws, size_t ws_floats, void* stream);
int dic_debug_depth_layer1_sparse_ws_floats(int B, int H, int W);
int dic_debug_depth_layer1_bwd_sparse(const float* depth, int B, int H, int W, const float* dpool, const unsigned char* idx, const float* xsel,
                                      const float* conv_w, const float* conv_b, const float* gamma, const float* scale, const float* shift,
                                      const float* mean, const float* invstd, float* dgamma, float* dbeta, float* dW, float* db, float* bn_ws,
                                      size_t bn_ws_floats, float* ws, size_t ws_floats, float* cs_ws, size_t cs_ws_floats, void* stream);
int dic_debug_conv1_fwd_checked(const float* x, int B, int H, int W, const float* w, const float* bias, float* y, float* partial,
                                size_t partial_floats, int* partial_rows, void* stream);
int dic_debug_conv1_wgrad_checked(const float* x, int B, int H, int W, const float* dy, float* dw, float* dbias, float* ws, size_t ws_floats,
                                  float* cs_ws, size_t cs_ws_floats, void* stream);
int dic_conv_persistent_grid(int max_workgroups);
int dic_profile_begin(void);
int dic_profile_end(int max_entries, int* keys, double* total_ms, double* total_flops, long long* launches, int* n_out);
int dic_profile_end_bytes(int max_entries, int* keys, double* total_ms, double* total_flops, double* total_bytes, long long* launches,
                          int* n_out);

#ifdef __cplusplus
}
#endif
#endif
```

Before: 7456 images/s.

## Fuse depth-encoder head backward and emit transposed wgrad planes from BN apply

Replaces the depth encoder's separate avgpool-backward, ReLU-mask-backward and BN-backward passes with one bn_head_backward that recomputes the pooled gradient and mask inside the reduce and apply kernels. It also adds a tiled BN-apply kernel that writes the K-major split planes used by the following weight-gradient GEMM, so conv_wgrad_bf3 can skip its own dy transpose pass. Both are on by default and aim to cut full-tensor round trips through memory and kernel launches. The cost is recomputing the avgpool gradient in both passes and a more complex tiled kernel with LDS transposes.

```diff
diff --git a/depth_image_captioning_pub_amd/csrc/api.hip b/depth_image_captioning_pub_amd/csrc/api.hip
--- a/depth_image_captioning_pub_amd/csrc/api.hip
+++ b/depth_image_captioning_pub_amd/csrc/api.hip
@@ -7,7 +7,7 @@
 using namespace dic;
 
 namespace dic { void resnet_fuse_bn_operand(int mask); void resnet_fuse_bn_halo(int on); void resnet_fuse_res_bn(int on); void depth_encoder_l1_sparse(int on); void bn_finalize_two_level_rows(int rows); void resnet_debug_fused_tail_bn(int on); void conv1_depth_debug_blocks(int n);
-                void depth_encoder_f16x2(int on); }
+                void depth_encoder_f16x2(int on); void depth_encoder_head_fused(int on); void depth_encoder_dyT_fused(int on); }
 #ifdef DIC_EXPERIMENTS
 namespace dic { void decoder_debug_persistent(int on); void decoder_persist_debug_buffer(unsigned long long* p); void decoder_persist_debug_placement(int p);
                 void resnet_debug_skip_bn_apply(int on); }
@@ -64,6 +64,8 @@
   if (on == 182 || on == 183) { dic::bn_finalize_two_level_rows(on == 182 ? 512 : 1024); return 0; }
   if (on == 180 || on == 181) { dic::depth_encoder_l1_sparse(on - 180); return 0; }
   if (on == 116 || on == 117) { dic::depth_encoder_f16x2(on - 116); return 0; }
+  if (on == 188 || on == 189) { dic::depth_encoder_dyT_fused(on - 188); return 0; }
+  if (on == 186 || on == 187) { dic::depth_encoder_head_fused(on - 186); return 0; }
 #ifdef DIC_EXPERIMENTS
   if (on == 140 || on == 141) { dic::decoder_debug_persistent(on - 140); return 0; }
   if (on == 142 || on == 143) { dic::decoder_persist_debug_placement(on - 142); return 0; }
@@ -268,6 +270,20 @@
   DIC_REQUIRE(ws_floats >= bn_backward_ws_floats(C), "dic_debug_bn_backward: ws holds %zu floats, %zu needed", ws_floats, bn_backward_ws_floats(C));
   return bn_backward(dy_dx, x, rows, C, gamma, bn, dgamma, dbeta, ws, (hipStream_t)stream, dx_planes, &fs);
 }
+int dic_debug_bn_head_backward(const float* dpool, int B, int H, int W, int out, const float* x, int C, const float* gamma, const float* scale,
+                               const float* shift, const float* mean, const float* invstd, float* dgamma, float* dbeta, float* ws,
+                               size_t ws_floats, float* dx, uint16_t* const dx_planes[3], uint32_t* f16_bound, float* f16_slot, void* stream) {
+  BnBuf bn;
+  F16Scale fs{};
+  DIC_TRY(bn_buf(scale, shift, mean, invstd, &bn, "dic_debug_bn_head_backward"));
+  DIC_TRY(plane_list(dx_planes, "dic_debug_bn_head_backward"));
+  DIC_TRY(f16_scale(dx_planes, f16_bound, f16_slot, &fs, "dic_debug_bn_head_backward"));
+  DIC_REQUIRE(dpool && x && gamma && dgamma && dbeta && ws && dx, "dic_debug_bn_head_backward: dpool / x / gamma / dgamma / dbeta / ws / dx is NULL");
+  DIC_REQUIRE(B >= 1 && H >= 1 && W >= 1 && out >= 1 && C >= 1, "dic_debug_bn_head_backward: B=%d H=%d W=%d out=%d C=%d must be positive", B, H, W, out, C);
+  DIC_REQUIRE(C % 4 == 0 && (!dx_planes || C % 64 == 0), "dic_debug_bn_head_backward: C=%d %% 4 (%% 64 with planes)", C);
+  DIC_REQUIRE(ws_floats >= bn_backward_ws_floats(C), "dic_debug_bn_head_backward: ws holds %zu floats, %zu needed", ws_floats, bn_backward_ws_floats(C));
+  return bn_head_backward(dpool, B, H, W, out, x, C, gamma, bn, dgamma, dbeta, ws, dx, (hipStream_t)stream, dx_planes, &fs);
+}
 int dic_debug_bn_pool_backward(const float* dpool, const unsigned char* idx, const float* x, int B, int H, int W, int C, int k,
                                const float* gamma, const float* scale, const float* shift, const float* mean, const float* invstd,
                                float* dgamma, float* dbeta, float* ws, size_t ws_floats, float* dy, uint16_t* const dy_planes[3],
diff --git a/depth_image_captioning_pub_amd/csrc/conv.h b/depth_image_captioning_pub_amd/csrc/conv.h
--- a/depth_image_captioning_pub_amd/csrc/conv.h
+++ b/depth_image_captioning_pub_amd/csrc/conv.h
@@ -46,7 +46,8 @@
 size_t conv_wgrad_bf3_ws_floats(const ConvDesc& d, int splitk);
 int conv_wgrad_bf3(const float* x, const ConvDesc& d, const float* dy, float* dw_ohwi, int splitk,
                    unsigned short* const dyT[3], unsigned short* const pT[3], float* ws, hipStream_t st,
-                   int fmt = 0, const float* dy_slot = nullptr );
+                   int fmt = 0, const float* dy_slot = nullptr ,
+                   bool dyT_ready = false );
 size_t conv_stem_bf3_plane_elems(int B, int H, int W);
 int conv_stem_pack_weights(const float* w_oihw, int CO, float* scratch_f32, unsigned short* const w_planes[3], hipStream_t st,
                            float f16_scale = 0.f );
diff --git a/depth_image_captioning_pub_amd/csrc/encoders.hip b/depth_image_captioning_pub_amd/csrc/encoders.hip
--- a/depth_image_captioning_pub_amd/csrc/encoders.hip
+++ b/depth_image_captioning_pub_amd/csrc/encoders.hip
@@ -31,6 +31,10 @@
 void depth_encoder_l1_sparse(int on) { g_l1_sparse = on; }
 static int g_depth_f16x2 = 1;
 void depth_encoder_f16x2(int on) { g_depth_f16x2 = on; }
+static int g_depth_head_fused = 1;
+void depth_encoder_head_fused(int on) { g_depth_head_fused = on; }
+static int g_depth_dyT_fused = 1;
+void depth_encoder_dyT_fused(int on) { g_depth_dyT_fused = on; }
 constexpr int kWg1Split = 128;
 constexpr int kWg2Split = 4;
 constexpr int kWg2SplitBf3 = 5;
@@ -556,10 +560,17 @@
   if (fmt) DIC_TRY(f16_scale_reset(ws.bounds + 2, 2, st));
   unsigned short* const dy3_out[3] = {ws.dy3_pl[0], ws.dy3_pl[1], fmt ? nullptr : ws.dy3_pl[2]};
   unsigned short* const dy2_out[3] = {ws.dy2_pl[0], ws.dy2_pl[1], fmt ? nullptr : ws.dy2_pl[2]};
-  DIC_TRY(adaptive_avgpool_bwd(d_features, B, g.P2h, g.P2w, 2048, pool_out ? pool_out : g.P2h, ws.dy3, st));
-  DIC_TRY(relu_mask_bwd(ws.dy3, ws.x3, g.M3, 2048, ws.bn3, st));
-  DIC_TRY(bn_backward(ws.dy3, ws.x3, g.M3, 2048, w->bn3_w, ws.bn3, gr->bn3_w, gr->bn3_b, ws.bn_ws, st, dy3_out, fmt ? &s_dy3 : nullptr));
-  DIC_TRY(conv_wgrad_bf3(ws.y2p, g.c3, ws.dy3, gr->conv3_w, kWg3SplitBf3, ws.wg_dyT, ws.wg_pT, ws.wg_bf3_ws, st, fmt, s_dy3.slot));
+  unsigned short* const dyT_out[3] = {ws.wg_dyT[0], ws.wg_dyT[1], fmt ? nullptr : ws.wg_dyT[2]};
+  const bool dyT3 = g_depth_head_fused && g_depth_dyT_fused, dyT2 = g_depth_dyT_fused != 0;
+  if (g_depth_head_fused) {
+    DIC_TRY(bn_head_backward(d_features, B, g.P2h, g.P2w, pool_out ? pool_out : g.P2h, ws.x3, 2048, w->bn3_w, ws.bn3, gr->bn3_w, gr->bn3_b,
+                             ws.bn_ws, ws.dy3, st, dy3_out, fmt ? &s_dy3 : nullptr, dyT3 ? dyT_out : nullptr));
+  } else {
+    DIC_TRY(adaptive_avgpool_bwd(d_features, B, g.P2h, g.P2w, 2048, pool_out ? pool_out : g.P2h, ws.dy3, st));
+    DIC_TRY(relu_mask_bwd(ws.dy3, ws.x3, g.M3, 2048, ws.bn3, st));
+    DIC_TRY(bn_backward(ws.dy3, ws.x3, g.M3, 2048, w->bn3_w, ws.bn3, gr->bn3_w, gr->bn3_b, ws.bn_ws, st, dy3_out, fmt ? &s_dy3 : nullptr));
+  }
+  DIC_TRY(conv_wgrad_bf3(ws.y2p, g.c3, ws.dy3, gr->conv3_w, kWg3SplitBf3, ws.wg_dyT, ws.wg_pT, ws.wg_bf3_ws, st, fmt, s_dy3.slot, dyT3));
   DIC_TRY(colsum_rows(ws.dy3, 2048, g.M3, 2048, gr->conv3_b, ws.cs_ws, st));
   {
     const unsigned short* dp[3] = {ws.dy3_pl[0], ws.dy3_pl[1], fmt ? nullptr : ws.dy3_pl[2]};
@@ -567,8 +578,8 @@
     DIC_TRY(conv_dgrad_s1_bf3(dp, g.c3, wp, ws.dy2p, st, ws.tail, kResnetTailSlabs, fmt, fmt ? s_dy3.slot + 1 : nullptr, fmt ? inv_w3 : nullptr));
   }
   DIC_TRY(bn_pool_backward(ws.dy2p, ws.idx2, ws.x2, B, g.H2, g.W2, 512, 3, w->bn2_w, ws.bn2, gr->bn2_w, gr->bn2_b,
-                           ws.bn_ws, ws.dy2, st, dy2_out, fmt ? &s_dy2 : nullptr));
-  DIC_TRY(conv_wgrad_bf3(ws.y1p, g.c2, ws.dy2, ws.dw2o, kWg2SplitBf3, ws.wg_dyT, ws.wg_pT, ws.wg_bf3_ws, st, fmt, s_dy2.slot));
+                           ws.bn_ws, ws.dy2, st, dy2_out, fmt ? &s_dy2 : nullptr, dyT2 ? dyT_out : nullptr));
+  DIC_TRY(conv_wgrad_bf3(ws.y1p, g.c2, ws.dy2, ws.dw2o, kWg2SplitBf3, ws.wg_dyT, ws.wg_pT, ws.wg_bf3_ws, st, fmt, s_dy2.slot, dyT2));
   DIC_TRY(ohwi_to_oihw(ws.dw2o, gr->conv2_w, 512, 128, 3, 3, st));
   DIC_TRY(colsum_rows(ws.dy2, 512, g.M2, 512, gr->conv2_b, ws.cs_ws, st));
   {
@@ -604,15 +615,27 @@
 
 int dic_depth_encoder_inspect(const void* workspace, size_t workspace_bytes, int B, int H, int W, int which, void* out,
                               long long* n_out, void* stream) {
-  DIC_REQUIRE(workspace && B > 0 && which >= 1 && which <= 5, "depth_encoder_inspect: bad arguments");
+  DIC_REQUIRE(workspace && B > 0 && which >= 1 && which <= 9, "depth_encoder_inspect: bad arguments");
   const DepthGeom g = depth_geom(B, H, W);
   bool ov = false;
   DepthWs ws = depth_carve(const_cast<void*>(workspace), workspace_bytes, g, &ov);
   DIC_REQUIRE(!ov, "depth_encoder_inspect: workspace too small");
-  const long long n = which <= 2 ? (long long)B * g.P1h * g.P1w * 128
+  const long long n = which == 9 ? 2 * (long long)conv_wgrad_bf3_plane_elems(g.c2, 0) : which == 8 ? 4 : which == 7 ? g.M2 * 512 : which == 6 ? g.M3 * 2048
+                      : which <= 2 ? (long long)B * g.P1h * g.P1w * 128
                       : which <= 4 ? (long long)B * g.P2h * g.P2w * 512 : g.M3 * 2048;
   if (n_out) *n_out = n;
   if (!out) return DIC_OK;
+  if (which == 9) {
+    const size_t e = conv_wgrad_bf3_plane_elems(g.c2, 0);
+    for (int i = 0; i < 2; ++i)
+      DIC_CHECK_HIP(hipMemcpyAsync((unsigned short*)out + i * e, ws.wg_dyT[i], e * sizeof(unsigned short), hipMemcpyDeviceToDevice, (hipStream_t)stream));
+    return DIC_OK;
+  }
+  if (which >= 6) {
+    const float* src = which == 6 ? ws.dy3 : which == 7 ? ws.dy2 : ws.slots + 4;
+    DIC_CHECK_HIP(hipMemcpyAsync(out, src, (size_t)n * sizeof(float), hipMemcpyDeviceToDevice, (hipStream_t)stream));
+    return DIC_OK;
+  }
   if (which == 5) return relu_mask_export(ws.x3, g.M3, 2048, ws.bn3, (unsigned char*)out, (hipStream_t)stream);
   const void* src = which == 1 ? (const void*)ws.y1p : which == 2 ? (const void*)ws.idx1 : which == 3 ? (const void*)ws.y2p
                                                                                                       : (const void*)ws.idx2;
diff --git a/depth_image_captioning_pub_amd/csrc/gemm_bf3.hip b/depth_image_captioning_pub_amd/csrc/gemm_bf3.hip
--- a/depth_image_captioning_pub_amd/csrc/gemm_bf3.hip
+++ b/depth_image_captioning_pub_amd/csrc/gemm_bf3.hip
@@ -2178,13 +2178,15 @@
 }
 
 int conv_wgrad_bf3(const float* x, const ConvDesc& d, const float* dy, float* dw_ohwi, int splitk,
-                   unsigned short* const dyT[3], unsigned short* const pT[3], float* ws, hipStream_t st, int fmt, const float* dy_slot) {
+                   unsigned short* const dyT[3], unsigned short* const pT[3], float* ws, hipStream_t st, int fmt, const float* dy_slot,
+                   bool dyT_ready) {
   DIC_REQUIRE(!d.in_nchw && d.C % 32 == 0 && d.CO % 32 == 0, "conv_wgrad_bf3: NHWC input, C and CO %% 32");
   DIC_REQUIRE(fmt == 0 || dy_slot, "conv_wgrad_bf3: the f16x2 format needs the scale slot of the gradient");
   const int M = d.M(), Kpad = (M + 31) / 32 * 32;
   const ConvGeom g = d.geom();
-  hipLaunchKernelGGL((transpose_split_kernel<false>), dim3(Kpad / 32, d.CO / 32), dim3(256), 0, st, dy, (long long)d.CO, M,
-                     Kpad, d.CO, g, dyT[0], dyT[1], fmt ? nullptr : dyT[2], 1.0f, fmt ? dy_slot : nullptr);
+  if (!dyT_ready)
+    hipLaunchKernelGGL((transpose_split_kernel<false>), dim3(Kpad / 32, d.CO / 32), dim3(256), 0, st, dy, (long long)d.CO, M,
+                       Kpad, d.CO, g, dyT[0], dyT[1], fmt ? nullptr : dyT[2], 1.0f, fmt ? dy_slot : nullptr);
   hipLaunchKernelGGL((transpose_split_kernel<true>), dim3(Kpad / 32, d.KH * d.KW * (d.C / 32)), dim3(256), 0, st, x,
                      (long long)d.C, M, Kpad, d.C, g, pT[0], pT[1], fmt ? nullptr : pT[2], kF16ActScale, (const float*)nullptr);
   DIC_LAUNCH_CHECK();
diff --git a/depth_image_captioning_pub_amd/csrc/nn_kernels.h b/depth_image_captioning_pub_amd/csrc/nn_kernels.h
--- a/depth_image_captioning_pub_amd/csrc/nn_kernels.h
+++ b/depth_image_captioning_pub_amd/csrc/nn_kernels.h
@@ -49,10 +49,15 @@
                 float* dbeta, float* ws, hipStream_t st,
                 unsigned short* const dx_planes[3] = nullptr   ,
                 F16Scale* f16 = nullptr)                        ;
+int bn_head_backward(const float* dpool, int B, int H, int W, int out, const float* x, int C, const float* gamma, BnBuf bn, float* dgamma,
+                     float* dbeta, float* ws, float* dx, hipStream_t st, unsigned short* const dx_planes[3] = nullptr,
+                     F16Scale* f16 = nullptr,
+                     unsigned short* const dxT_planes[3] = nullptr   );
 int bn_pool_backward(const float* dpool, const unsigned char* idx, const float* x, int B, int H, int W, int C, int k,
                      const float* gamma, BnBuf bn, float* dgamma, float* dbeta, float* ws, float* dy, hipStream_t st,
                      unsigned short* const dy_planes[3] = nullptr   ,
-                     F16Scale* f16 = nullptr)                        ;
+                     F16Scale* f16 = nullptr                         ,
+                     unsigned short* const dyT_planes[3] = nullptr   );
 void bn_backward_ws_layout(float* ws, int C, float** part, float** k2, float** k3);
 int bn_backward_finalize(const float* part, int chunks, int C, double rows, float* dgamma, float* dbeta, float* k2, float* k3, hipStream_t st);
 size_t bn_backward_ws_floats(int C);
diff --git a/depth_image_captioning_pub_amd/csrc/nn_kernels.hip b/depth_image_captioning_pub_amd/csrc/nn_kernels.hip
--- a/depth_image_captioning_pub_amd/csrc/nn_kernels.hip
+++ b/depth_image_captioning_pub_amd/csrc/nn_kernels.hip
@@ -439,6 +439,24 @@
   return DIC_OK;
 }
 
+__device__ __forceinline__ float4 avgpool_grad4(const float* __restrict__ dy, int b, int h, int w, int c4, int C4, int H, int W, int OUT) {
+  float4 acc = make_float4(0.f, 0.f, 0.f, 0.f);
+  const int oi_lo = max(0, (h * OUT) / H - 1), oi_hi = min(OUT - 1, ((h + 1) * OUT + H - 1) / H + 1);
+  const int oj_lo = max(0, (w * OUT) / W - 1), oj_hi = min(OUT - 1, ((w + 1) * OUT + W - 1) / W + 1);
+  for (int oi = oi_lo; oi <= oi_hi; ++oi) {
+    const int h0 = (oi * H) / OUT, h1 = ((oi + 1) * H + OUT - 1) / OUT;
+    if (h < h0 || h >= h1) continue;
+    for (int oj = oj_lo; oj <= oj_hi; ++oj) {
+      const int w0 = (oj * W) / OUT, w1 = ((oj + 1) * W + OUT - 1) / OUT;
+      if (w < w0 || w >= w1) continue;
+      const float inv = 1.0f / (float)((h1 - h0) * (w1 - w0));
+      const float4 g = reinterpret_cast<const float4*>(dy)[(((long long)b * OUT + oi) * OUT + oj) * C4 + c4];
+      acc.x += g.x * inv; acc.y += g.y * inv; acc.z += g.z * inv; acc.w += g.w * inv;
+    }
+  }
+  return acc;
+}
+
 __global__ void __launch_bounds__(256) adaptive_avgpool_bwd_kernel(const float* __restrict__ dy, int B, int H, int W,
                                                                     int C4, int OUT, float* __restrict__ dx) {
   const long long total = (long long)B * H * W * C4;
@@ -449,21 +467,7 @@
     const int w = (int)(r % W); r /= W;
     const int h = (int)(r % H);
     const int b = (int)(r / H);
-    float4 acc = make_float4(0.f, 0.f, 0.f, 0.f);
-    const int oi_lo = max(0, (h * OUT) / H - 1), oi_hi = min(OUT - 1, ((h + 1) * OUT + H - 1) / H + 1);
-    const int oj_lo = max(0, (w * OUT) / W - 1), oj_hi = min(OUT - 1, ((w + 1) * OUT + W - 1) / W + 1);
-    for (int oi = oi_lo; oi <= oi_hi; ++oi) {
-      const int h0 = (oi * H) / OUT, h1 = ((oi + 1) * H + OUT - 1) / OUT;
-      if (h < h0 || h >= h1) continue;
-      for (int oj = oj_lo; oj <= oj_hi; ++oj) {
-        const int w0 = (oj * W) / OUT, w1 = ((oj + 1) * W + OUT - 1) / OUT;
-        if (w < w0 || w >= w1) continue;
-        const float inv = 1.0f / (float)((h1 - h0) * (w1 - w0));
-        const float4 g = reinterpret_cast<const float4*>(dy)[(((long long)b * OUT + oi) * OUT + oj) * C4 + c4];
-        acc.x += g.x * inv; acc.y += g.y * inv; acc.z += g.z * inv; acc.w += g.w * inv;
-      }
-    }
-    reinterpret_cast<float4*>(dx)[i] = acc;
+    reinterpret_cast<float4*>(dx)[i] = avgpool_grad4(dy, b, h, w, c4, C4, H, W, OUT);
   }
 }
 
@@ -516,6 +520,25 @@
 
 __device__ __forceinline__ bool relu_passes(float v, float sc, float sh) { return fmaf(v, sc, sh) > 0.f; }
 
+struct HeadGeom { int H, W, OUT, identity; };
+__device__ __forceinline__ float4 head_grad4(const float* __restrict__ dpool, long long row, int c4, int C4, HeadGeom hg, const float4 v,
+                                             const float4 sc, const float4 sh) {
+  float4 g;
+  if (hg.identity) {
+    const float4 d = reinterpret_cast<const float4*>(dpool)[row * C4 + c4];
+    g = make_float4(0.f + d.x, 0.f + d.y, 0.f + d.z, 0.f + d.w);
+  } else {
+    const int w = (int)(row % hg.W);
+    const long long r = row / hg.W;
+    g = avgpool_grad4(dpool, (int)(r / hg.H), (int)(r % hg.H), w, c4, C4, hg.H, hg.W, hg.OUT);
+  }
+  if (!relu_passes(v.x, sc.x, sh.x)) g.x = 0.f;
+  if (!relu_passes(v.y, sc.y, sh.y)) g.y = 0.f;
+  if (!relu_passes(v.z, sc.z, sh.z)) g.z = 0.f;
+  if (!relu_passes(v.w, sc.w, sh.w)) g.w = 0.f;
+  return g;
+}
+
 __global__ void __launch_bounds__(256) relu_mask_bwd_kernel(float* __restrict__ dy, const float* __restrict__ x,
                                                              long long n4, int C4, BnBuf bn) {
   const long long stride = (long long)gridDim.x * 256;
@@ -597,9 +620,10 @@
 
 constexpr int kBnChunksMax = 512;
 static inline int reduce_chunks(int C) { return std::min(kBnChunksMax, std::max(64, 1024 / std::max(1, C / 64))); }
+template <bool HEAD>
 __global__ void __launch_bounds__(256) bn_bwd_reduce_kernel(const float* __restrict__ dy, const float* __restrict__ x,
                                                              long long rows, int C, BnBuf bn, float* __restrict__ part,
-                                                             float* __restrict__ gmaxp) {
+                                                             float* __restrict__ gmaxp, HeadGeom hg) {
   __shared__ float4 sa[16][16], sb[16][16];
   __shared__ float smax[4];
   float gm = 0.f;
@@ -611,14 +635,20 @@
   if (c < C) {
     const float4 mu = *reinterpret_cast<const float4*>(bn.mean + c);
     const float4 is = *reinterpret_cast<const float4*>(bn.invstd + c);
+    float4 sc = mu, sh = mu;
+    if constexpr (HEAD) {
+      sc = *reinterpret_cast<const float4*>(bn.scale + c);
+      sh = *reinterpret_cast<const float4*>(bn.shift + c);
+    }
     for (long long r = r0 + rl; r < r1; r += 64) {
       float4 g[4], v[4];
 #pragma unroll
       for (int u = 0; u < 4; ++u) {
         const long long rr = r + 16 * u;
         const long long rc = min(rr, r1 - 1);
-        g[u] = *reinterpret_cast<const float4*>(dy + rc * C + c);
         v[u] = *reinterpret_cast<const float4*>(x + rc * C + c);
+        if constexpr (HEAD) g[u] = head_grad4(dy, rc, c >> 2, C >> 2, hg, v[u], sc, sh);
+        else g[u] = *reinterpret_cast<const float4*>(dy + rc * C + c);
         if (rr >= r1) g[u] = make_float4(0.f, 0.f, 0.f, 0.f);
       }
 #pragma unroll
@@ -694,19 +724,25 @@
   }
 }
 
+template <bool HEAD>
 __global__ void __launch_bounds__(256) bn_bwd_apply_kernel(float* __restrict__ dy, const float* __restrict__ x,
                                                             long long n4, int C4, const float* __restrict__ gamma,
                                                             BnBuf bn, const float* __restrict__ k2,
                                                             const float* __restrict__ k3,
                                                             unsigned short* __restrict__ hi,
                                                             unsigned short* __restrict__ mid,
-                                                            unsigned short* __restrict__ lo, const float* __restrict__ f16_slot) {
+                                                            unsigned short* __restrict__ lo, const float* __restrict__ f16_slot,
+                                                            const float* __restrict__ dpool, HeadGeom hg) {
   const long long stride = (long long)gridDim.x * 256;
   const float fs = f16_slot ? f16_slot[0] : 1.f;
   for (long long i = (long long)blockIdx.x * 256 + threadIdx.x; i < n4; i += stride) {
     const int c = (int)(i % C4) * 4;
-    const float4 g = reinterpret_cast<float4*>(dy)[i];
     const float4 v = reinterpret_cast<const float4*>(x)[i];
+    float4 g;
+    if constexpr (HEAD)
+      g = head_grad4(dpool, i / C4, c >> 2, C4, hg, v, *reinterpret_cast<const float4*>(bn.scale + c), *reinterpret_cast<const float4*>(bn.shift + c));
+    else
+      g = reinterpret_cast<float4*>(dy)[i];
     const float4 mu = *reinterpret_cast<const float4*>(bn.mean + c);
     const float4 is = *reinterpret_cast<const float4*>(bn.invstd + c);
     const float4 ga = *reinterpret_cast<const float4*>(gamma + c);
@@ -746,14 +782,14 @@
   float* k3 = k2 + C;
   float* gmaxp = k3 + C;
   const int chunks = reduce_chunks(C);
-  hipLaunchKernelGGL(bn_bwd_reduce_kernel, dim3(C / 64, chunks), dim3(256), 0, st, dy_dx, x, rows, C, bn, part, f16x2 ? gmaxp : nullptr);
+  hipLaunchKernelGGL((bn_bwd_reduce_kernel<false>), dim3(C / 64, chunks), dim3(256), 0, st, dy_dx, x, rows, C, bn, part, f16x2 ? gmaxp : nullptr, HeadGeom{});
   hipLaunchKernelGGL(bn_bwd_finalize_kernel, dim3(ceil_div(C, 32)), dim3(256), 0, st, part, chunks, C, (double)rows,
                      dgamma, dbeta, k2, k3, (const float*)gmaxp, gamma, (const float*)bn.invstd, f16x2 ? f16->bound : nullptr);
   if (f16x2) DIC_TRY(f16_scale_finish(*f16, st));
   const long long n4 = rows * C / 4;
-  hipLaunchKernelGGL(bn_bwd_apply_kernel, dim3(ew_blocks(n4)), dim3(256), 0, st, dy_dx, x, n4, C / 4, gamma, bn, k2, k3,
+  hipLaunchKernelGGL((bn_bwd_apply_kernel<false>), dim3(ew_blocks(n4)), dim3(256), 0, st, dy_dx, x, n4, C / 4, gamma, bn, k2, k3,
                      dx_planes ? dx_planes[0] : nullptr, dx_planes ? dx_planes[1] : nullptr,
-                     dx_planes ? dx_planes[2] : nullptr, f16x2 ? (const float*)f16->slot : nullptr);
+                     dx_planes ? dx_planes[2] : nullptr, f16x2 ? (const float*)f16->slot : nullptr, (const float*)nullptr, HeadGeom{});
   DIC_LAUNCH_CHECK();
   return DIC_OK;
 }
@@ -896,9 +932,104 @@
   if (i < n4) finish(i, reinterpret_cast<const float4*>(x)[i]);
 }
 
+template <bool POOL>
+__global__ void __launch_bounds__(256) bn_bwd_apply_tile_kernel(const float* __restrict__ dpool, const unsigned char* __restrict__ idx,
+                                                                 const float* __restrict__ x, float* __restrict__ dy, long long rows, int C,
+                                                                 HeadGeom hg, PoolGeom pg, const float* __restrict__ gamma, BnBuf bn,
+                                                                 const float* __restrict__ k2, const float* __restrict__ k3,
+                                                                 unsigned short* __restrict__ hi, unsigned short* __restrict__ mid,
+                                                                 unsigned short* __restrict__ lo, const float* __restrict__ f16_slot,
+                                                                 unsigned short* __restrict__ thi, unsigned short* __restrict__ tmid,
+                                                                 unsigned short* __restrict__ tlo, int Kpad) {
+  __shared__ float tile[32][65];
+  const float fs = f16_slot ? f16_slot[0] : 1.f;
+  const int tid = threadIdx.x;
+  const long long m0 = (long long)blockIdx.x * 32;
+  const int c0 = blockIdx.y * 64;
+  {
+    const int c4l = tid & 15, rl = tid >> 4;
+    const int c = c0 + c4l * 4, C4 = C >> 2;
+    const float4 sc = *reinterpret_cast<const float4*>(bn.scale + c);
+    const float4 sh = *reinterpret_cast<const float4*>(bn.shift + c);
+    const float4 mu = *reinterpret_cast<const float4*>(bn.mean + c);
+    const float4 is = *reinterpret_cast<const float4*>(bn.invstd + c);
+    const float4 ga = *reinterpret_cast<const float4*>(gamma + c);
+    const float4 a2 = *reinterpret_cast<const float4*>(k2 + c);
+    const float4 a3 = *reinterpret_cast<const float4*>(k3 + c);
+    float4 v[2];
+#pragma unroll
+    for (int u = 0; u < 2; ++u) v[u] = *reinterpret_cast<const float4*>(x + min(m0 + rl + 16 * u, rows - 1) * C + c);
+#pragma unroll
+    for (int u = 0; u < 2; ++u) {
+      const long long r = m0 + rl + 16 * u;
+      float4 o = make_float4(0.f, 0.f, 0.f, 0.f);
+      if (r < rows) {
+        float4 g;
+        if constexpr (POOL) g = pool_relu_grad4(dpool, idx, v[u], sc, sh, (unsigned)r, c >> 2, C4, pg);
+        else g = head_grad4(dpool, r, c >> 2, C4, hg, v[u], sc, sh);
+        o.x = ga.x * is.x * (g.x - a2.x - (v[u].x - mu.x) * is.x * a3.x);
+        o.y = ga.y * is.y * (g.y - a2.y - (v[u].y - mu.y) * is.y * a3.y);
+        o.z = ga.z * is.z * (g.z - a2.z - (v[u].z - mu.z) * is.z * a3.z);
+        o.w = ga.w * is.w * (g.w - a2.w - (v[u].w - mu.w) * is.w * a3.w);
+        *reinterpret_cast<float4*>(dy + r * C + c) = o;
+        const long long off = plane_offset(r, c, C4 / 8, 1);
+        unsigned short h[4], m[4], l[4];
+        if (!lo) {
+          split2_f16(o.x, fs, h[0], m[0]); split2_f16(o.y, fs, h[1], m[1]); split2_f16(o.z, fs, h[2], m[2]); split2_f16(o.w, fs, h[3], m[3]);
+        } else {
+          split3_bf16(o.x, h[0], m[0], l[0]); split3_bf16(o.y, h[1], m[1], l[1]);
+          split3_bf16(o.z, h[2], m[2], l[2]); split3_bf16(o.w, h[3], m[3], l[3]);
+        }
+        *reinterpret_cast<uint2*>(hi + off) = make_uint2((unsigned)h[0] | ((unsigned)h[1] << 16), (unsigned)h[2] | ((unsigned)h[3] << 16));
+        *reinterpret_cast<uint2*>(mid + off) = make_uint2((unsigned)m[0] | ((unsigned)m[1] << 16), (unsigned)m[2] | ((unsigned)m[3] << 16));
+        if (lo) *reinterpret_cast<uint2*>(lo + off) = make_uint2((unsigned)l[0] | ((unsigned)l[1] << 16), (unsigned)l[2] | ((unsigned)l[3] << 16));
+      }
+      float* t = &tile[rl + 16 * u][c4l * 4];
+      t[0] = o.x; t[1] = o.y; t[2] = o.z; t[3] = o.w;
+    }
+  }
+  __syncthreads();
+  {
+    const int quad = tid & 7, parity = (tid >> 3) & 1, q = tid >> 4;
+#pragma unroll
+    for (int u = 0; u < 2; ++u) {
+      const int cl = 32 * u + 2 * q + parity;
+      unsigned short h[4], mm[4], l[4];
+      if (!lo) {
+#pragma unroll
+        for (int j = 0; j < 4; ++j) split2_f16(tile[quad * 4 + j][cl], fs, h[j], mm[j]);
+      } else {
+#pragma unroll
+        for (int j = 0; j < 4; ++j) split3_bf16(tile[quad * 4 + j][cl], h[j], mm[j], l[j]);
+      }
+      const long long off = plane_offset(c0 + cl, m0 + quad * 4, Kpad / 32, 1);
+      *reinterpret_cast<uint2*>(thi + off) = make_uint2((unsigned)h[0] | ((unsigned)h[1] << 16), (unsigned)h[2] | ((unsigned)h[3] << 16));
+      *reinterpret_cast<uint2*>(tmid + off) = make_uint2((unsigned)mm[0] | ((unsigned)mm[1] << 16), (unsigned)mm[2] | ((unsigned)mm[3] << 16));
+      if (lo) *reinterpret_cast<uint2*>(tlo + off) = make_uint2((unsigned)l[0] | ((unsigned)l[1] << 16), (unsigned)l[2] | ((unsigned)l[3] << 16));
+    }
+  }
+}
+
+static int launch_apply_tile(bool pool, const float* dpool, const unsigned char* idx, const float* x, float* dy, long long rows, int C,
+                             HeadGeom hg, PoolGeom pg, const float* gamma, BnBuf bn, const float* k2, const float* k3,
+                             unsigned short* const planes[3], const float* f16_slot, unsigned short* const dxT[3], hipStream_t st) {
+  DIC_REQUIRE(planes && planes[0] && planes[1] && dxT[0] && dxT[1] && (!planes[2] == !dxT[2]), "bn backward: K-major planes go with row-major planes of the same format");
+  DIC_REQUIRE(C % 64 == 0 && rows >= 1 && rows < (1ll << 31) - 32, "bn backward, K-major planes: C %% 64, rows < 2^31");
+  const int Kpad = (int)((rows + 31) / 32 * 32);
+  const dim3 grid((unsigned)(Kpad / 32), (unsigned)(C / 64));
+  if (pool)
+    hipLaunchKernelGGL((bn_bwd_apply_tile_kernel<true>), grid, dim3(256), 0, st, dpool, idx, x, dy, rows, C, hg, pg, gamma, bn, k2, k3,
+                       planes[0], planes[1], planes[2], f16_slot, dxT[0], dxT[1], dxT[2], Kpad);
+  else
+    hipLaunchKernelGGL((bn_bwd_apply_tile_kernel<false>), grid, dim3(256), 0, st, dpool, idx, x, dy, rows, C, hg, pg, gamma, bn, k2, k3,
+                       planes[0], planes[1], planes[2], f16_slot, dxT[0], dxT[1], dxT[2], Kpad);
+  DIC_LAUNCH_CHECK();
+  return DIC_OK;
+}
+
 int bn_pool_backward(const float* dpool, const unsigned char* idx, const float* x, int B, int H, int W, int C, int k,
                      const float* gamma, BnBuf bn, float* dgamma, float* dbeta, float* ws, float* dy, hipStream_t st,
-                     unsigned short* const dy_planes[3], F16Scale* f16) {
+                     unsigned short* const dy_planes[3], F16Scale* f16, unsigned short* const dyT_planes[3]) {
   DIC_REQUIRE(C % 64 == 0, "bn_pool_backward: C %% 64");
   const bool f16x2 = dy_planes && !dy_planes[2];
   DIC_REQUIRE(!f16x2 || (f16 && f16->bound && f16->slot), "bn_pool_backward: f16x2 planes need a scale slot");
@@ -915,10 +1046,42 @@
   hipLaunchKernelGGL(bn_bwd_finalize_kernel, dim3(ceil_div(C, 32)), dim3(256), 0, st, part, chunks, C, (double)rows,
                      dgamma, dbeta, k2, k3, (const float*)gmaxp, gamma, (const float*)bn.invstd, f16x2 ? f16->bound : nullptr);
   if (f16x2) DIC_TRY(f16_scale_finish(*f16, st));
+  if (dyT_planes)
+    return launch_apply_tile(true, dpool, idx, x, dy, rows, C, HeadGeom{}, pg, gamma, bn, k2, k3, dy_planes, f16x2 ? (const float*)f16->slot : nullptr,
+                             dyT_planes, st);
   const long long n4 = rows * C / 4;
   hipLaunchKernelGGL(bn_pool_bwd_apply_kernel, dim3(ew_blocks(n4)), dim3(256), 0, st, dpool, idx, x, dy, n4, C / 4, pg,
                      gamma, bn, k2, k3, dy_planes ? dy_planes[0] : nullptr, dy_planes ? dy_planes[1] : nullptr,
                      dy_planes ? dy_planes[2] : nullptr, f16x2 ? (const float*)f16->slot : nullptr, make_fastdiv((unsigned)(C / 4)));
+  DIC_LAUNCH_CHECK();
+  return DIC_OK;
+}
+
+int bn_head_backward(const float* dpool, int B, int H, int W, int out, const float* x, int C, const float* gamma, BnBuf bn, float* dgamma,
+                     float* dbeta, float* ws, float* dx, hipStream_t st, unsigned short* const dx_planes[3], F16Scale* f16,
+                     unsigned short* const dxT_planes[3]) {
+  DIC_REQUIRE(C % 4 == 0 && (!dx_planes || C % 64 == 0), "bn_head_backward: C %% 4 (%% 64 with planes)");
+  const bool f16x2 = dx_planes && !dx_planes[2];
+  DIC_REQUIRE(!f16x2 || (f16 && f16->bound && f16->slot), "bn_head_backward: f16x2 planes need a scale slot");
+  const long long rows = (long long)B * H * W;
+  DIC_REQUIRE(rows < (1ll << 31) && (long long)B * out * out < (1ll << 31), "bn_head_backward: index range");
+  const HeadGeom hg{H, W, out, out == H && out == W ? 1 : 0};
+  float* part = ws;
+  float* k2 = ws + (size_t)kBnChunksMax * 2 * C;
+  float* k3 = k2 + C;
+  float* gmaxp = k3 + C;
+  const int chunks = reduce_chunks(C);
+  hipLaunchKernelGGL((bn_bwd_reduce_kernel<true>), dim3(ceil_div(C, 64), chunks), dim3(256), 0, st, dpool, x, rows, C, bn, part, f16x2 ? gmaxp : nullptr, hg);
+  hipLaunchKernelGGL(bn_bwd_finalize_kernel, dim3(ceil_div(C, 32)), dim3(256), 0, st, part, chunks, C, (double)rows,
+                     dgamma, dbeta, k2, k3, (const float*)gmaxp, gamma, (const float*)bn.invstd, f16x2 ? f16->bound : nullptr);
+  if (f16x2) DIC_TRY(f16_scale_finish(*f16, st));
+  if (dxT_planes)
+    return launch_apply_tile(false, dpool, nullptr, x, dx, rows, C, hg, PoolGeom{}, gamma, bn, k2, k3, dx_planes, f16x2 ? (const float*)f16->slot : nullptr,
+                             dxT_planes, st);
+  const long long n4 = rows * C / 4;
+  hipLaunchKernelGGL((bn_bwd_apply_kernel<true>), dim3(ew_blocks(n4)), dim3(256), 0, st, dx, x, n4, C / 4, gamma, bn, k2, k3,
+                     dx_planes ? dx_planes[0] : nullptr, dx_planes ? dx_planes[1] : nullptr,
+                     dx_planes ? dx_planes[2] : nullptr, f16x2 ? (const float*)f16->slot : nullptr, dpool, hg);
   DIC_LAUNCH_CHECK();
   return DIC_OK;
 }
diff --git a/include/dic.h b/include/dic.h
--- a/include/dic.h
+++ b/include/dic.h
@@ -314,6 +314,9 @@
 int dic_debug_bn_backward(float* dy_dx, const float* x, long long rows, int C, const float* gamma, const float* scale, const float* shift,
                           const float* mean, const float* invstd, float* dgamma, float* dbeta, float* ws, size_t ws_floats,
                           uint16_t* const dx_planes[3], uint32_t* f16_bound, float* f16_slot, void* stream);
+int dic_debug_bn_head_backward(const float* dpool, int B, int H, int W, int out, const float* x, int C, const float* gamma, const float* scale,
+                               const float* shift, const float* mean, const float* invstd, float* dgamma, float* dbeta, float* ws,
+                               size_t ws_floats, float* dx, uint16_t* const dx_planes[3], uint32_t* f16_bound, float* f16_slot, void* stream);
 int dic_debug_bn_pool_backward(const float* dpool, const unsigned char* idx, const float* x, int B, int H, int W, int C, int k,
                                const float* gamma, const float* scale, const float* shift, const float* mean, const float* invstd,
                                float* dgamma, float* dbeta, float* ws, size_t ws_floats, float* dy, uint16_t* const dy_planes[3],
```

New measurement: 7526 images/s (median of 6 runs). About the same (+0.9%).
